# chhylp123/BitMapperBS

Hardware: AMD Instinct MI355X
Metric: M 150bp PE reads aligned/s (higher is better)
Workload: dtype u64

## Files before the change

### bitmapperbs_amd/csrc/bmbs_api.hip

```cpp
#include "bmbs_host.h"
#include "bmbs_kernels.hip"



int ensure(Lane* c, DevBuf& b, size_t bytes, bool zero)
{
    if (bytes == 0) bytes = 16;
    if (b.cap >= bytes) return BMBS_OK;
    size_t want = bytes + bytes / 8 + 256;
    if (c->kn.arena && want <= ((size_t)256 << 20)) {
        if (b.cap) want = std::min<size_t>(std::max(want, b.cap + b.cap / 2), (size_t)256 << 20);
        void* p = c->arena.alloc(want);
        if (!p) { c->err = "out of device memory (lane arena)"; return BMBS_ENOMEM; }
        if (b.p && !b.arena) (void)hipFree(b.p);
        b.p = p; b.cap = want; b.arena = true;
    } else {
        if (b.p && !b.arena) (void)hipFree(b.p);
        b.p = nullptr; b.cap = 0; b.arena = false;
        hipError_t e = hipMalloc(&b.p, want);
        if (e != hipSuccess) { c->err = std::string("hipMalloc: ") + hipGetErrorString(e); b.p = nullptr; return BMBS_ENOMEM; }
        b.cap = want;
    }
    if (zero && hipMemsetAsync(b.p, 0, want, c->stream) != hipSuccess) { c->err = "hipMemsetAsync failed"; return BMBS_ESTATE; }
    return BMBS_OK;
// ... 82 lines not shown
    }
    if (rep) for (int c = nc; c < 16; c++) rep[c] = rep[0];
    *n_classes = nc;
}

int map_calculation(const bmbs_params& P, unsigned second_best_diff, unsigned error_threshold, int best_score)
{
    const int unit = std::max(P.gap_open + P.gap_ext, P.mp_max);
    const int worst = -unit * (int)error_threshold;
    const double rank = (double)std::max(best_score - worst, 0) / (double)(-worst);
    const unsigned ediff = second_best_diff > error_threshold ? error_threshold + 1 : second_best_diff;
    if (ediff > error_threshold) {
        static const struct { double at; int q; } alone[] = {{0.8, 42}, {0.7, 40}, {0.6, 24}, {0.5, 23}, {0.4, 8}, {0.3, 3}};
        for (const auto& r : alone) if (rank >= r.at) return r.q;
        return 0;
    }
    const double rerr = (double)(int)ediff / (double)error_threshold;
    const bool perfect = best_score == 0;
    static const struct { double at; int zero; double hi_cut; int hi; double mid_cut; int mid; int lo; } rows[] = {
        {0.9, 39, 0.0, 33, 0.0, 33, 33}, {0.8, 38, 0.0, 27, 0.0, 27, 27}, {0.7, 37, 0.0, 26, 0.0, 26, 26}, {0.6, 36, 0.0, 22, 0.0, 22, 22},
        {0.5, 35, 0.84, 25, 0.68, 16, 5}, {0.4, 34, 0.84, 21, 0.68, 14, 4},
        {0.3, 32, 0.88, 18, 0.67, 15, 3}, {0.2, 31, 0.88, 17, 0.67, 11, 0}, {0.1, 30, 0.88, 12, 0.67, 7, 0},
    };
    for (const auto& r : rows)
        if (rerr >= r.at) return perfect ? r.zero : rank >= r.hi_cut ? r.hi : rank >= r.mid_cut ? r.mid : r.lo;
    return ediff == 0 ? (rank >= 0.67 ? 1 : 0) : (rank >= 0.67 ? 6 : 2);
}

int threshold_k(const bmbs_params& P, int L)
{
    u64 k = (u64)(P.e_f * L);
    if (k >= 31) k = 31;
    return (int)k;
}

int cigar_ops_bound(const bmbs_params& P, int L, int k)
{
    const long goe = (long)P.gap_open + P.gap_ext;
    const long worst = std::max<long>(std::max<long>(P.mp_max, P.np), goe);
    long gaps = (long)L + 2 * k;
    if (goe > 0) gaps = std::min<long>(gaps, (long)k * worst / goe);
    return (int)std::min<long>(2 * gaps + 8, 1 << 20);
}
#define BMBS_MAX_RECORD_OPS 254

int prepare_luts(Lane* c)
{
    if (c->luts_ready) return BMBS_OK;
    int unit = c->prm.gap_open + c->prm.gap_ext;
    if (unit < c->prm.mp_max) unit = c->prm.mp_max;
    c->mapq_unit = unit;
    std::vector<u32> off(64, 0);
    std::vector<u8> lut;
    for (int k = 0; k <= 62; k++) {
        const int range = unit * k;
        off[k] = (u32)lut.size();
        lut.resize(lut.size() + (size_t)(k + 2) * (range + 1));
        u8* t = lut.data() + off[k];
        for (int ed = 0; ed <= k + 1; ed++)
            for (int sd = 0; sd <= range; sd++)
                t[(size_t)ed * (range + 1) + sd] = (u8)map_calculation(c->prm, (unsigned)ed, (unsigned)k, sd - range);
    }
    std::vector<u8> kl(1002);
    for (int L = 0; L <= 1001; L++) kl[L] = (u8)threshold_k(c->prm, L);
    ENS(c, c->mapq_lut, lut.size()); ENS(c, c->mapq_off, off.size() * 4); ENS(c, c->klut, kl.size());
    HIPCHK(c, hipMemcpyAsync(c->mapq_lut.p, lut.data(), lut.size(), hipMemcpyHostToDevice, c->stream));
    HIPCHK(c, hipMemcpyAsync(c->mapq_off.p, off.data(), off.size() * 4, hipMemcpyHostToDevice, c->stream));
    HIPCHK(c, hipMemcpyAsync(c->klut.p, kl.data(), kl.size(), hipMemcpyHostToDevice, c->stream));
    HIPCHK(c, hipStreamSynchronize(c->stream));
    c->luts_ready = true;
    return BMBS_OK;
}

ReadGeom geom(Lane* c, int L, const u16* d_len)
{
    ReadGeom g;
    g.len = d_len; g.klut = c->klut.as<u8>(); g.L = L; g.k = threshold_k(c->prm, L);
    return g;
}

int per_read_workspace(Lane* c, u64 n)
{
    ENS(c, c->verdict, n); ENS(c, c->n_seeds, n); ENS(c, c->multi, n); ENS(c, c->mm_site, n * 2);
    ENS(c, c->exit_site, n * 8); ENS(c, c->seeds, n * BMBS_MAX_SEEDS * sizeof(SeedRec));
    ENS(c, c->n_cand, n * 4); ENS(c, c->cand_off, (n + 1) * 8); ENS(c, c->n_votes, n * 4);
    ENS(c, c->best_site, n * 8); ENS(c, c->best_end, n * 4); ENS(c, c->best_err, n * 4); ENS(c, c->sbd, n * 4);
    ENS(c, c->red_status, n); ENS(c, c->job_flag, n * 4); ENS(c, c->job_off, (n + 1) * 8);
    return BMBS_OK;
}

ReadState read_state(Lane* c)
{
    ReadState s;
    s.verdict = c->verdict.as<u8>(); s.n_seeds = c->n_seeds.as<u8>(); s.multi = c->multi.as<u8>();
    s.mm_site = c->mm_site.as<u16>(); s.exit_site = c->exit_site.as<u64>(); s.seeds = c->seeds.as<SeedRec>();
    s.n_cand = c->n_cand.as<u32>(); s.cand_off = c->cand_off.as<u64>(); s.n_votes = c->n_votes.as<u32>();
    s.best_site = c->best_site.as<u64>(); s.best_end = c->best_end.as<int32_t>(); s.best_err = c->best_err.as<u32>();
    s.sbd = c->sbd.as<u32>(); s.red_status = c->red_status.as<u8>(); s.job_flag = c->job_flag.as<u32>();
    s.job_off = c->job_off.as<u64>();
    return s;
}

inline u64 sw_trace_slots(u64 n_jobs) { const u64 t = (u64)nblk(n_jobs, 64) * 64; return t < (1ull << 20) ? t : (1ull << 20); }

inline size_t sw_window_lds(const ReadGeom& gm, int jobs_per_lane) { return (size_t)jobs_per_lane * ((gm.L + 2 * gm.k + 62) / 32 + 1) * 64 * 8; }

template <int KB>
void launch_sw(Lane* c, const char* d_seq, const char* d_qual, const char* d_qual2, const ReadGeom& gm, int stride, u64 n_jobs,
               const Jobs& jobs, u32 rev_from, u32* d_cigar_pool, int max_ops, const PackedRows& prw)
{
    const u64 slots = sw_trace_slots(n_jobs);
    const size_t lds = sw_window_lds(gm, 1);
    auto kern = gm.len ? k_align_sw<KB, false> : gm.k == KB ? k_align_sw<KB, true, true> : k_align_sw<KB, true, false>;
    for (u64 base = 0; base < n_jobs; base += slots)
        hipLaunchKernelGGL(kern, dim3((unsigned)(slots / 64)), dim3(64), lds, c->stream, c->ix, c->sp, c->pen_lut.as<int>(), d_seq,
                           d_qual, d_qual2, gm, stride, c->totals.as<u64>() + 2, c->sw_job.as<u32>(), jobs, rev_from, c->trace.as<u64>(),
                           slots, base, d_cigar_pool, max_ops, c->a_start.as<int>(), c->a_end.as<int>(), c->a_nm.as<u32>(),
                           c->a_score.as<int>(), c->a_nops.as<int>(), prw);
}

template <int KB>
void launch_sw2(Lane* c, const char* d_seq, const char* d_qual, const char* d_qual2, const ReadGeom& gm, int stride, u64 n_jobs,
                const Jobs& jobs, u32 rev_from, u32* d_cigar_pool, int max_ops, const PackedRows& prw)
{
    const u64 slots = sw_trace_slots((n_jobs + 1) / 2);
    auto kern = !prw.base ? k_align_sw2<KB, false, false> : gm.k == KB ? k_align_sw2<KB, true, true> : k_align_sw2<KB, false, true>;
    for (u64 base = 0; base < n_jobs; base += 2 * slots)
        hipLaunchKernelGGL(kern, dim3((unsigned)(slots / 64)), dim3(64), sw_window_lds(gm, 2), c->stream, c->ix, c->sp, c->pen_lut.as<int>(), d_seq,
                           d_qual, d_qual2, gm, stride, c->totals.as<u64>() + 2, c->sw_job.as<u32>(), jobs, rev_from, c->trace.as<u64>(),
                           slots, base, d_cigar_pool, max_ops, c->a_start.as<int>(), c->a_end.as<int>(), c->a_nm.as<u32>(),
                           c->a_score.as<int>(), c->a_nops.as<int>(), prw);
}

template <class F>
void with_band_bound(int k, F&& f)
{
    if (k <= 2) f(std::integral_constant<int, 2>());
    else if (k <= 4) f(std::integral_constant<int, 4>());
    else if (k <= 6) f(std::integral_constant<int, 6>());
    else if (k <= 8) f(std::integral_constant<int, 8>());
    else if (k <= 10) f(std::integral_constant<int, 10>());
    else if (k <= 12) f(std::integral_constant<int, 12>());
    else if (k <= 16) f(std::integral_constant<int, 16>());
    else if (k <= 20) f(std::integral_constant<int, 20>());
    else if (k <= 24) f(std::integral_constant<int, 24>());
    else f(std::integral_constant<int, 31>());
}

int run_align(Lane* c, const char* d_seq, const char* d_qual, const char* d_qual2, const ReadGeom& gm, int stride, u64 n_jobs, const Jobs& jobs,
              u32 rev_from, u32* d_cigar_pool, int max_ops, const PackedRows& pr, const u64* n_jobs_dev, u64 sw_bound)
{
    if (sw_bound > n_jobs) sw_bound = n_jobs;
    const int L = gm.L, k = gm.k;
    const u64 nj = n_jobs ? n_jobs : 1;
    const u64 nwk = (u64)((2 * k + 1 + 15) / 16);
    ENS(c, c->a_start, nj * 4); ENS(c, c->a_end, nj * 4); ENS(c, c->a_nm, nj * 4); ENS(c, c->a_score, nj * 4); ENS(c, c->a_nops, nj * 4);
    ENS(c, c->need_sw, nj * 4); ENS(c, c->sw_off, (nj + 1) * 8); ENS(c, c->sw_job, nj * 4);
    if (!n_jobs) return BMBS_OK;
    const int swm = c->kn.sw_form;
    const bool wave_form = swm == 3;
    int maxpen = std::max(std::max(c->prm.mp_max, c->prm.np), c->prm.gap_open + c->prm.gap_ext);
    const bool packed = !wave_form && swm != 1 && (k >= 5 || swm == 2) && !gm.len && c->prm.gap_ext < 256 && (L + 64) * maxpen < 12000 &&
                        c->prm.mp_min >= 0 && c->prm.gap_ext >= 0 && c->prm.gap_open >= 0 && c->prm.np >= 0;
    const bool reg_form = !wave_form;
    if (reg_form) {
        const u64 nwords = packed ? (u64)((2 * k + 1 + 7) / 8) : nwk;
        const u64 slots = packed ? sw_trace_slots((sw_bound + 1) / 2) : sw_trace_slots(sw_bound);
        ENS(c, c->trace, slots * (u64)L * nwords * 8);
    }
    unsigned long long* cnt = c->counters.as<unsigned long long>();
    prof_begin(c, "k_align_ungapped");
    if (pr.base)
        hipLaunchKernelGGL(k_align_ungapped_p, dim3(nblk(n_jobs, 256)), dim3(256), 0, c->stream, c->ix, c->sp, c->pen_lut.as<int>(), d_seq, pr,
                           d_qual, d_qual2, gm, stride, n_jobs, n_jobs_dev, jobs, rev_from, c->a_start.as<int>(), c->a_end.as<int>(), c->a_nm.as<u32>(),
                           c->a_score.as<int>(), c->a_nops.as<int>(), c->need_sw.as<u32>(), cnt);
    else
        hipLaunchKernelGGL(k_align_ungapped, dim3(nblk(n_jobs, 256)), dim3(256), 0, c->stream, c->ix, c->sp, c->pen_lut.as<int>(), d_seq,
                           d_qual, d_qual2, gm, stride, n_jobs, n_jobs_dev, jobs, rev_from, c->a_start.as<int>(), c->a_end.as<int>(), c->a_nm.as<u32>(),
                           c->a_score.as<int>(), c->a_nops.as<int>(), c->need_sw.as<u32>(), cnt);
    prof_end(c);
    prof_begin(c, "scan_sw");
    int rc = scan_u32(c, c->need_sw.as<u32>(), n_jobs, c->sw_off.as<u64>(), 2, c->sw_job.as<u32>(), 0, n_jobs_dev);
    if (rc) return rc;
    prof_end(c);
    if (n_jobs_dev && reg_form && sw_bound < n_jobs)
        hipLaunchKernelGGL(k_guard_count, dim3(1), dim3(1), 0, c->stream, c->totals.as<u64>() + 2, sw_bound, c->flags.as<u32>(), BMBS_FLAG_SW);
    prof_begin(c, "k_align_sw");
    if (!reg_form) {
        const size_t words = (size_t)sww_lds_words(L, k);
#define SWW_LAUNCH(LANES)                                                                                                             \
        hipLaunchKernelGGL((k_align_sw_wave<LANES>), dim3(nblk(n_jobs, 64 / LANES)), dim3(64), words * 4 * (64 / LANES), c->stream, c->ix, \
                           c->sp, c->pen_lut.as<int>(), d_seq, d_qual, d_qual2, gm, stride, c->totals.as<u64>() + 2, c->sw_job.as<u32>(),   \
                           jobs, rev_from, d_cigar_pool, max_ops, c->a_start.as<int>(), c->a_end.as<int>(), c->a_nm.as<u32>(),          \
                           c->a_score.as<int>(), c->a_nops.as<int>(), pr)
        if (k <= 7) SWW_LAUNCH(16);
        else if (k <= 15) SWW_LAUNCH(32);
        else SWW_LAUNCH(64);
#undef SWW_LAUNCH
        prof_end(c);
        return BMBS_OK;
    }
    with_band_bound(k, [&](auto kb) {
        if (packed) launch_sw2<decltype(kb)::value>(c, d_seq, d_qual, d_qual2, gm, stride, sw_bound, jobs, rev_from, d_cigar_pool, max_ops, pr);
        else launch_sw<decltype(kb)::value>(c, d_seq, d_qual, d_qual2, gm, stride, sw_bound, jobs, rev_from, d_cigar_pool, max_ops, pr);
    });
    prof_end(c);
    return BMBS_OK;
}

SeedCarry seed_carry(Lane* c)
{
    SeedCarry sc;
    sc.sp0 = c->sd_sp0.as<u64>(); sc.hits0 = c->sd_hits0.as<u32>(); sc.ml0 = c->sd_ml0.as<u16>(); sc.tm = c->sd_tm.as<u16>();
    sc.seed_id = c->sd_seed_id.as<u8>(); sc.clen = c->sd_clen.as<u32>(); sc.first_ml = c->sd_first_ml.as<u16>();
    sc.flag_c = c->sd_flag_c.as<u32>(); sc.flag_d = c->sd_flag_d.as<u32>(); sc.off_c = c->sd_off_c.as<u64>(); sc.off_d = c->sd_off_d.as<u64>();
    sc.list_c = c->sd_list_c.as<u32>(); sc.list_d = c->sd_list_d.as<u32>();
    return sc;
}

bool use_packed_rows(const Lane* c) { return !c->kn.rows_ascii; }
PackedRows packed_rows(const Lane* c, const ReadGeom& gm)
{
    if (!use_packed_rows(c)) return PackedRows{nullptr, nullptr, 0, 0};
    return PackedRows{c->prow.as<u64>(), c->prow_dirty.as<u8>(), pack_words(gm.L), pack_base_words(gm.L)};
}

bool occ3_build(Occ3Shared& o, u64 margin)
{
    const u64 rows = o.rows, nb = rows / 96 + 2, need = 27 * nb * 16;
    size_t free_b = 0, total_b = 0;
    (void)hipMemGetInfo(&free_b, &total_b);
    if (free_b <= need + margin) return false;
    const u64 n_chunks = (nb + OCC3_CHUNK - 1) / OCC3_CHUNK;
    void *t3 = nullptr, *c3 = nullptr, *sums = nullptr;
    hipStream_t st = nullptr;
    bool ok = hipMalloc(&t3, need) == hipSuccess && hipMalloc(&c3, 64 * 8) == hipSuccess && hipMalloc(&sums, 27 * n_chunks * 8 + 64) == hipSuccess &&
              hipStreamCreate(&st) == hipSuccess;
    if (ok) {
        u32* flag = reinterpret_cast<u32*>(c3) + 2 * 60;
        (void)hipMemsetAsync(c3, 0, 64 * 8, st);
        hipLaunchKernelGGL(k_occ3_planes, dim3(8192), dim3(256), 0, st, o.base, rows, nb, reinterpret_cast<uint4*>(t3));
        hipLaunchKernelGGL(k_occ3_chunk_sums, dim3(nblk(27 * n_chunks, 256)), dim3(256), 0, st, reinterpret_cast<uint4*>(t3), nb, n_chunks, reinterpret_cast<u64*>(sums));
        hipLaunchKernelGGL(k_occ3_chunk_scan, dim3(1), dim3(64), 0, st, reinterpret_cast<u64*>(sums), n_chunks, flag);
        hipLaunchKernelGGL(k_occ3_apply, dim3(nblk(27 * n_chunks, 256)), dim3(256), 0, st, reinterpret_cast<uint4*>(t3), nb, n_chunks, reinterpret_cast<u64*>(sums));
        hipLaunchKernelGGL(k_occ3_c3, dim3(1), dim3(64), 0, st, o.base, reinterpret_cast<u64*>(c3));
        DevIndex probe = o.base;
        probe.occ3 = reinterpret_cast<const uint4*>(t3); probe.c3 = reinterpret_cast<const u64*>(c3); probe.nb3 = nb;
        const u64 n_check = 1u << 20;
        hipLaunchKernelGGL(k_occ3_check, dim3(nblk(n_check, 256)), dim3(256), 0, st, probe, rows, n_check, flag + 1);
        u32 h[2] = {1, 1};
        ok = hipMemcpyAsync(h, flag, 8, hipMemcpyDeviceToHost, st) == hipSuccess && hipStreamSynchronize(st) == hipSuccess && h[0] == 0 && h[1] == 0;
        if (!ok && getenv("BMBS_VERBOSE")) fprintf(stderr, "[bmbs] trigram table not used: count overflow %u, differences from three single steps %u\n", h[0], h[1]);
    }
    if (st) (void)hipStreamDestroy(st);
    if (sums) (void)hipFree(sums);
    if (ok) { o.occ3 = t3; o.c3 = c3; o.nb3 = nb; }
    else { if (t3) (void)hipFree(t3); if (c3) (void)hipFree(c3); }
    return true;
}
void occ3_want(Lane* c, bool behind_a_call)
{
    if (c->ix.occ3 || !c->o3 || c->kn.kgram < 1 || !use_packed_rows(c)) return;
    const bool wants = c->kn.kgram >= 2 || c->lr_chain >= 3.0;
    std::lock_guard<std::mutex> l(c->o3->mu);
    if (!c->o3->occ3 && wants && !c->o3->tried) {
        (void)hipSetDevice(c->dev);
        const bool attempted = occ3_build(*c->o3, behind_a_call ? (8ull << 30) : (40ull << 30));
        if (attempted || ++c->o3->skipped >= 8) c->o3->tried = true;
    }
    if (c->o3->occ3) { c->ix.occ3 = reinterpret_cast<const uint4*>(c->o3->occ3); c->ix.c3 = reinterpret_cast<const u64*>(c->o3->c3); c->ix.nb3 = c->o3->nb3; }
}

int launch_seeding(Lane* c, const char* d_seq, const ReadGeom& gm, int stride, u64 n, int pe_mode, bool prepacked)
{
    ENS(c, c->sd_sp0, n * 8); ENS(c, c->sd_hits0, n * 4); ENS(c, c->sd_ml0, n * 2); ENS(c, c->sd_tm, n * 2); ENS(c, c->sd_seed_id, n);
    ENS(c, c->sd_clen, n * 4); ENS(c, c->sd_first_ml, n * 2); ENS(c, c->sd_flag_c, n * 4); ENS(c, c->sd_flag_d, n * 4);
    ENS(c, c->sd_off_c, (n + 1) * 8); ENS(c, c->sd_off_d, (n + 1) * 8); ENS(c, c->sd_list_c, n * 4); ENS(c, c->sd_list_d, n * 4);
    SeedCarry sc = seed_carry(c);
    ReadState st = read_state(c);
    unsigned long long* cnt = c->counters.as<unsigned long long>();
    const unsigned chunks = nblk(n, SEED_CHUNK);
    const unsigned chunks_min = nblk(n, SEED_CHUNK_MIN);
    const int target_waves = c->kn.seed_waves;
    const bool packed = use_packed_rows(c);
    if (packed && !prepacked) {
        const int pwords = pack_words(gm.L), W = pack_base_words(gm.L);
        { int rz_ = ensure(c, c->prow, n * (u64)pwords * 8 + 64, true); if (rz_) return rz_; } ENS(c, c->prow_dirty, n + 64);
        HIPCHK(c, hipMemsetAsync(c->prow_dirty.p, 0, n + 64, c->stream));
        prof_begin(c, "k_pack_rows");
        hipLaunchKernelGGL(k_pack_rows, dim3(nblk(n * (u64)(stride / 16), 256)), dim3(256), 0, c->stream, d_seq, gm, stride, (long)n,
                           c->prow.as<u64>(), pwords, W, c->prow_dirty.as<u32>());
        prof_end(c);
    }
    const PackedRows pr = packed_rows(c, gm);
    prof_begin(c, "k_seed_first");
    occ3_want(c, false);
    const bool kg = c->ix.occ3 && packed && (c->kn.kgram >= 2 || (c->kn.kgram == 1 && c->lr_chain >= 3.0));
    const int stage = c->kn.seed_stage;
    if (packed && kg && stage) hipLaunchKernelGGL((k_seed_first<true, true, true>), dim3(chunks), dim3(64), 0, c->stream, c->ix, d_seq, pr, gm, stride, (long)n, sc, cnt);
    else if (packed && kg) hipLaunchKernelGGL((k_seed_first<true, true>), dim3(chunks), dim3(64), 0, c->stream, c->ix, d_seq, pr, gm, stride, (long)n, sc, cnt);
    else if (packed && stage) hipLaunchKernelGGL((k_seed_first<true, false, true>), dim3(chunks), dim3(64), 0, c->stream, c->ix, d_seq, pr, gm, stride, (long)n, sc, cnt);
    else if (packed) hipLaunchKernelGGL(k_seed_first<true>, dim3(chunks), dim3(64), 0, c->stream, c->ix, d_seq, pr, gm, stride, (long)n, sc, cnt);
    else hipLaunchKernelGGL(k_seed_first<false>, dim3(chunks), dim3(64), 0, c->stream, c->ix, d_seq, pr, gm, stride, (long)n, sc, cnt);
    prof_end(c);
    prof_begin(c, "k_seed_decide");
    const bool lds_ok = (size_t)64 * (stride + 8) <= 48 * 1024;
    if (packed)
        hipLaunchKernelGGL(k_seed_decide_p, dim3(nblk(n, 64)), dim3(64), (size_t)64 * (pr.pwords + 1) * 8, c->stream, c->ix, d_seq, pr, gm, stride,
                           (long)n, c->prm.seed_len, pe_mode, (stage && !(pe_mode && c->prm.sensitive)) ? 1 : 0, st, sc, cnt);
    else if (lds_ok)
        hipLaunchKernelGGL((k_seed_decide<true, true>), dim3(nblk(n, 64)), dim3(64), (size_t)64 * (stride + 8), c->stream, c->ix, d_seq, gm,
                           stride, (long)n, c->prm.seed_len, pe_mode, st, sc, cnt);
    else
        hipLaunchKernelGGL((k_seed_decide<false, true>), dim3(nblk(n, 256)), dim3(256), 0, c->stream, c->ix, d_seq, gm, stride, (long)n,
                           c->prm.seed_len, pe_mode, st, sc, cnt);
    prof_end(c);
    prof_begin(c, "list_second");
    int rc = scan_u32(c, sc.flag_c, n, sc.off_c, 3, sc.list_c);
    if (rc) return rc;
    prof_end(c);
    prof_begin(c, "k_seed_second");
    if (packed && kg) hipLaunchKernelGGL((k_seed_second<true, true>), dim3(chunks_min), dim3(64), 0, c->stream, c->ix, d_seq, pr, gm, stride, c->totals.as<u64>() + 3, target_waves, pe_mode, st, sc, cnt);
    else if (packed) hipLaunchKernelGGL(k_seed_second<true>, dim3(chunks_min), dim3(64), 0, c->stream, c->ix, d_seq, pr, gm, stride, c->totals.as<u64>() + 3, target_waves, pe_mode, st, sc, cnt);
    else hipLaunchKernelGGL(k_seed_second<false>, dim3(chunks_min), dim3(64), 0, c->stream, c->ix, d_seq, pr, gm, stride, c->totals.as<u64>() + 3, target_waves, pe_mode, st, sc, cnt);
    prof_end(c);
    prof_begin(c, "list_extra");
    rc = scan_u32(c, sc.flag_d, n, sc.off_d, 4, sc.list_d);
    if (rc) return rc;
    prof_end(c);
    prof_begin(c, "k_seed_extra");
    {
        const size_t lds = 64 * (size_t)(stride + 16);
        const bool wide_ix = c->ix.sa64 != nullptr;
        const int rows_in_lds = lds <= 48 * 1024 && !wide_ix;
        const size_t plds = (size_t)64 * (pr.pwords + 1) * 8;
        if (packed && plds <= 16 * 1024 && kg)
            hipLaunchKernelGGL((k_seed_extra<false, true, true, true>), dim3(chunks_min), dim3(64), plds, c->stream, c->ix, d_seq, pr, gm, stride, c->totals.as<u64>() + 4,
                               target_waves, c->prm.seed_len, pe_mode, st, sc, cnt);
        else if (packed && plds <= 16 * 1024)
            hipLaunchKernelGGL((k_seed_extra<false, true, true>), dim3(chunks_min), dim3(64), plds, c->stream, c->ix, d_seq, pr, gm, stride, c->totals.as<u64>() + 4,
                               target_waves, c->prm.seed_len, pe_mode, st, sc, cnt);
        else if (packed)
            hipLaunchKernelGGL((k_seed_extra<false, true>), dim3(chunks_min), dim3(64), 0, c->stream, c->ix, d_seq, pr, gm, stride, c->totals.as<u64>() + 4,
                               target_waves, c->prm.seed_len, pe_mode, st, sc, cnt);
        else if (rows_in_lds)
            hipLaunchKernelGGL((k_seed_extra<true, false>), dim3(chunks_min), dim3(64), lds, c->stream, c->ix, d_seq, pr, gm, stride, c->totals.as<u64>() + 4,
                               target_waves, c->prm.seed_len, pe_mode, st, sc, cnt);
        else
            hipLaunchKernelGGL((k_seed_extra<false, false>), dim3(chunks_min), dim3(64), 0, c->stream, c->ix, d_seq, pr, gm, stride, c->totals.as<u64>() + 4,
                               target_waves, c->prm.seed_len, pe_mode, st, sc, cnt);
    }
    prof_end(c);
    return BMBS_OK;
}

int cand_total(Lane* c, const ReadState& st, u64 n, bool exact, u64* tot_out)
{
    if (exact) {
        u64 tot = 0;
        HIPCHK(c, hipMemcpyAsync(&tot, c->totals.as<u64>(), 8, hipMemcpyDeviceToHost, c->stream));
        HIPCHK(c, hipStreamSynchronize(c->stream));
        *tot_out = tot;
        return BMBS_OK;
    }
    const u64 cap = cap_from(c->lr_cand, n, n, c->kn.cap_scale);
    hipLaunchKernelGGL(k_guard_cand, dim3(nblk(n, 256)), dim3(256), 0, c->stream, c->totals.as<u64>(), cap, c->flags.as<u32>(), (long)n, st.verdict,
                       st.n_cand, st.cand_off);
    hipLaunchKernelGGL(k_guard_done, dim3(1), dim3(1), 0, c->stream, c->totals.as<u64>(), c->flags.as<u32>(), BMBS_FLAG_CAND);
    *tot_out = cap;
    return BMBS_OK;
}

int run_seed_stages(Lane* c, const char* d_seq, const ReadGeom& gm, int stride, u64 n, u64* total_cand, int pe_mode, bool exact, bool prepacked)
{
    ReadState st = read_state(c);
    int rc = launch_seeding(c, d_seq, gm, stride, n, pe_mode, prepacked);
    if (rc) return rc;
    prof_begin(c, "scan_cand");
    rc = scan_u32(c, st.n_cand, n, st.cand_off, 0);
    if (rc) return rc;
    prof_end(c);
    u64 tot = 0;
    rc = cand_total(c, st, n, exact, &tot);
    if (rc) return rc;
    *total_cand = tot;
    const u64 t1 = exact ? std::max<u64>(tot, cap_from((double)tot / (double)n, n, n)) : tot;
    ENS(c, c->cand, t1 * 8); ENS(c, c->votes, t1 * sizeof(bmbs_vote)); ENS(c, c->slot_read, t1 * 4);
    ENS(c, c->ferr, t1 * 4); ENS(c, c->fend, t1 * 4);
    ENS(c, c->long_flag, n * 4); ENS(c, c->long_off, (n + 1) * 8); ENS(c, c->long_list, n * 4); ENS(c, c->vote_list, n * 4);
    prof_begin(c, "k_vote_fused");
    HIPCHK(c, hipMemsetAsync(c->long_flag.p, 0, n * 4, c->stream));
    HIPCHK(c, hipMemsetAsync(st.n_votes, 0, n * 4, c->stream));
// ... 43 lines not shown
    if (n && stride == ds) { HIPCHK(c, hipMemcpyAsync(dst.p, src, n * (u64)ds, hipMemcpyHostToDevice, st)); return BMBS_OK; }
    HIPCHK(c, hipMemsetAsync(dst.p, 0, n * (u64)ds + 64, st));
    if (n) HIPCHK(c, hipMemcpy2DAsync(dst.p, ds, src, stride, L, n, hipMemcpyHostToDevice, st));
    return BMBS_OK;
}


extern "C" void bmbs_default_params(bmbs_params* p)
{
    p->e_f = 0.08; p->mp_max = 6; p->mp_min = 2; p->np = 1; p->gap_open = 5; p->gap_ext = 3; p->q_base = 33;
    p->seed_len = 30; p->min_ins = 0; p->max_ins = 500; p->sensitive = 0; p->ambiguous_out = 0;
}

void lane_destroy(Lane* c);

Lane* lane_create(int device_id, const bmbs_params& prm, const Knobs& kn, bool first)
{
    Lane* c = new Lane();
    c->dev = device_id;
    c->prm = prm; c->kn = kn;
    c->sp.mp_max = c->prm.mp_max; c->sp.mp_min = c->prm.mp_min; c->sp.np = c->prm.np;
    c->sp.gap_open = c->prm.gap_open; c->sp.gap_ext = c->prm.gap_ext; c->sp.q_base = c->prm.q_base;
    c->sp.seed_len = c->prm.seed_len;
    if (hipStreamCreate(&c->stream) != hipSuccess) { delete c; return nullptr; }
    (void)hipEventCreateWithFlags(&c->ev_up, hipEventDisableTiming);
    (void)hipEventCreateWithFlags(&c->ev_k, hipEventDisableTiming);
    int lut[256];
    for (int q = 0; q < 256; q++) lut[q] = mismatch_penalty(c->prm, q);
    {
        uint8_t class_of[256], rep[16]; int32_t penalty_of[16], nc = 0;
        qual_class_table(c->prm, class_of, penalty_of, &nc, rep);
        for (int k = 0; k < 8; k++) { c->qrep_lo |= (u64)rep[k] << (8 * k); c->qrep_hi |= (u64)rep[8 + k] << (8 * k); }
    }
    const size_t shard_bytes = BMBS_SHARDS * BMBS_SHARD_WORDS * 8;
    if (ensure(c, c->pen_lut, sizeof(lut)) || ensure(c, c->stats, shard_bytes) || ensure(c, c->call_stats, shard_bytes) || ensure(c, c->counters, shard_bytes) ||
        ensure(c, c->totals, 32 * 8) || ensure(c, c->flags, BMBS_FLAG_WORDS * 4) || ensure(c, c->tx_info, 64) ||
        hipHostMalloc((void**)&c->h_info, 128, hipHostMallocPortable) != hipSuccess ||
        hipHostMalloc((void**)&c->h_tot, 8 * 20 * 8, hipHostMallocPortable) != hipSuccess) { lane_destroy(c); return nullptr; }
    memset(c->h_tot, 0, 8 * 20 * 8);
    (void)hipMemcpy(c->pen_lut.p, lut, sizeof(lut), hipMemcpyHostToDevice);
    (void)hipMemset(c->stats.p, 0, shard_bytes);
    (void)hipMemset(c->call_stats.p, 0, shard_bytes);
    (void)hipMemset(c->counters.p, 0, shard_bytes);
    textpath_device_init(c);
    (void)hipMemset(c->totals.p, 0, 32 * 8);
    (void)hipMemset(c->flags.p, 0, BMBS_FLAG_WORDS * 4);
    if (first)
    if (const char* wl = getenv("BMBS_WAVELOG")) {
        const unsigned cap = 1u << 21;
        if (*wl && !ensure(c, c->wavelog_buf, (u64)cap * 32) && !ensure(c, c->wavelog_count, 64)) {
            (void)hipMemset(c->wavelog_count.p, 0, 64);
            WaveLogDev d = {c->wavelog_buf.as<unsigned long long>(), c->wavelog_count.as<unsigned int>(), cap};
            if (hipMemcpyToSymbol(HIP_SYMBOL(g_wavelog), &d, sizeof(d)) == hipSuccess) c->wavelog_path = wl;
        }
    }
    return c;
}

void lane_copy_streams(std::vector<Lane*>& lanes)
{
    for (Lane* c : lanes) (void)hipStreamCreateWithFlags(&c->up_stream, hipStreamNonBlocking);
    for (Lane* c : lanes) (void)hipStreamCreateWithFlags(&c->down_stream, hipStreamNonBlocking);
}
__attribute__((constructor)) static void bmbs_env_init() { setenv("GPU_MAX_HW_QUEUES", "8", 0); }

void lane_destroy(Lane* c)
{
    if (!c) return;
    (void)hipSetDevice(c->dev);
    if (c->stream) (void)hipStreamSynchronize(c->stream);
    if (!c->wavelog_path.empty()) {
        (void)hipDeviceSynchronize();
        unsigned cnt = 0;
        (void)hipMemcpy(&cnt, c->wavelog_count.p, 4, hipMemcpyDeviceToHost);
        if (cnt > (1u << 21)) cnt = 1u << 21;
        std::vector<unsigned long long> h((size_t)cnt * 4);
        if (cnt) (void)hipMemcpy(h.data(), c->wavelog_buf.p, (size_t)cnt * 32, hipMemcpyDeviceToHost);
        if (FILE* f = fopen(c->wavelog_path.c_str(), "wb")) { fwrite(h.data(), 32, cnt, f); fclose(f); }
        WaveLogDev d = {nullptr, nullptr, 0};
        (void)hipMemcpyToSymbol(HIP_SYMBOL(g_wavelog), &d, sizeof(d));
        release(c->wavelog_buf); release(c->wavelog_count);
    }
    DevBuf* all[] = {&c->occ, &c->hash, &c->sa, &c->gen2, &c->gen2p, &c->chrom_start, &c->t20, &c->pen_lut, &c->mapq_lut, &c->verdict,
                     &c->n_seeds, &c->multi, &c->mm_site, &c->exit_site, &c->seeds, &c->n_cand, &c->cand_off,
                     &c->n_votes, &c->best_site, &c->best_end, &c->best_err, &c->sbd, &c->red_status, &c->job_flag,
                     &c->job_off, &c->scan_tmp, &c->scan_ticket, &c->totals, &c->cand, &c->votes, &c->slot_read, &c->vote_off, &c->votes_dense, &c->dense_read, &c->ferr, &c->fend,
                     &c->job_read, &c->job_site, &c->job_end, &c->job_err, &c->need_sw, &c->sw_off, &c->sw_job, &c->trace, &c->a_start, &c->a_end, &c->a_nm, &c->a_score, &c->a_nops,
                     &c->in_seq, &c->in_qual, &c->out_res, &c->cig_pool, &c->in_a, &c->in_b, &c->in_c, &c->in_d,
                     &c->stats, &c->call_stats, &c->flags, &c->counters, &c->pe_seq, &c->pe_B, &c->pe_occ, &c->pe_len, &c->pe_cur,
                     &c->sd_sp0, &c->sd_hits0, &c->sd_ml0, &c->sd_tm, &c->sd_seed_id, &c->sd_clen, &c->sd_first_ml, &c->sd_flag_c, &c->sd_flag_d,
                     &c->sd_off_c, &c->sd_off_d, &c->sd_list_c, &c->sd_list_d, &c->pe_vround, &c->pe_dead, &c->pe_both, &c->pe_npair, &c->pe_sbd, &c->in_seq2, &c->in_qual2,
                     &c->pe_first, &c->pe_full, &c->pe_R, &c->pe_roff, &c->pe_rflag, &c->pe_rscan, &c->pe_rlist, &c->pe_rcnt, &c->pe_ritem_off, &c->pe_rcand, &c->long_flag, &c->long_off, &c->long_list, &c->vote_list,
                     &c->mapq_off, &c->klut, &c->in_len, &c->fq_text1, &c->fq_text2, &c->fq_idx, &c->pk_in1, &c->pk_in2, &c->pq_in1, &c->pq_in2, &c->pk_ascii, &c->prow, &c->prow_dirty, &c->pe_mid_flag, &c->pe_mid_list};
    for (DevBuf* b : all) release(*b);
    for (auto& set : c->profset) for (auto& p : set) { (void)hipEventDestroy(p.a); (void)hipEventDestroy(p.b); }
    c->arena.free_all();
    if (c->h_tot) (void)hipHostFree(c->h_tot);
    if (c->h_info) (void)hipHostFree(c->h_info);
    { DevBuf* tx[] = {&c->tx_tilecnt, &c->tx_tileoff, &c->tx_nl[0], &c->tx_nl[1], &c->tx_rec[0], &c->tx_rec[1], &c->tx_info, &c->sam_len, &c->sam_off, &c->sam_out, &c->chrom_chars, &c->chrom_off, &c->big_list,
                     &c->bam_raw, &c->bam_slots, &c->bam_slot_len, &c->bam_off, &c->stats_snap, &c->z_comp, &c->z_off, &c->z_text, &c->z_err, &c->z_nl, &c->z_comp2, &c->z_off2, &c->z_err2,
                     &c->bs_key, &c->bs_key2, &c->bs_idx, &c->bs_idx2, &c->bs_slen, &c->bs_soff, &c->bs_tmp, &c->bs_in, &c->bs_len, &c->bs_off, &c->bs_sorted, &c->bai_a, &c->bai_b, &c->bai_out,
                     &c->dp_in, &c->dp_len, &c->dp_off, &c->dp_sig, &c->dp_key, &c->dp_key2, &c->dp_idx, &c->dp_idx2, &c->dp_dup, &c->dp_tmpl,
                     &c->mt_in, &c->mt_len, &c->mt_off, &c->mt_clip, &c->mt_cnt, &c->mt_eoff, &c->mt_ev, &c->mt_work, &c->mt_acc, &c->mt_site, &c->mt_cl2};
      for (DevBuf* b : tx) release(*b); }
    if (c->ev_up) (void)hipEventDestroy(c->ev_up);
    if (c->ev_k) (void)hipEventDestroy(c->ev_k);
    if (c->ev_qx_a) (void)hipEventDestroy(c->ev_qx_a);
    if (c->ev_qx_b) (void)hipEventDestroy(c->ev_qx_b);
    if (c->up_stream) (void)hipStreamDestroy(c->up_stream);
    if (c->down_stream) (void)hipStreamDestroy(c->down_stream);
    if (c->stream) (void)hipStreamDestroy(c->stream);
    delete c;
}


extern "C" bmbs_ctx* bmbs_create(int device_id, const bmbs_params* params)
{
    int ndev = 0;
    if (hipGetDeviceCount(&ndev) != hipSuccess || ndev <= 0 || device_id < 0 || device_id >= ndev) return nullptr;
    if (hipSetDevice(device_id) != hipSuccess) return nullptr;
    bmbs_ctx* X = new bmbs_ctx();
    X->dev = device_id;
    if (params) X->prm = *params; else bmbs_default_params(&X->prm);
    X->kn.read();
    for (int i = 0; i < X->kn.host_lanes; i++) {
        Lane* c = lane_create(device_id, X->prm, X->kn, i == 0);
        if (!c) { bmbs_destroy(X); return nullptr; }
        X->lanes.push_back(c);
    }
    lane_copy_streams(X->lanes);
    return X;
}

extern "C" void bmbs_destroy(bmbs_ctx* X)
{
#ifdef VOTE_PROF
    {
        unsigned long long h[4][8];
        if (hipMemcpyFromSymbol(h, HIP_SYMBOL(g_vote_prof), sizeof h) == hipSuccess)
            for (int q = 0; q < 4; q++)
                fprintf(stderr, "[vote_prof] class %d: lists %llu candidates %llu sites %llu | Mcycles: locate+sort %.1f run-ends %.1f vote-order %.1f write %.1f | one-lane fallbacks %llu\n",
                        q, h[q][0], h[q][1], h[q][2], h[q][3] / 1e6, h[q][4] / 1e6, h[q][5] / 1e6, h[q][6] / 1e6, h[q][7]);
    }
#endif
    if (!X) return;
    (void)hipSetDevice(X->dev);
    for (size_t i = X->lanes.size(); i-- > 0;) lane_destroy(X->lanes[i]);
    delete X;
}

extern "C" int32_t bmbs_max_cigar_ops(const bmbs_params* params, int32_t L)
{
    if (L <= 0 || L > BMBS_MAX_READ) return -1;
    bmbs_params P;
    if (params) P = *params; else bmbs_default_params(&P);
    return cigar_ops_bound(P, L, threshold_k(P, L));
}

extern "C" int64_t bmbs_outcome_index(uint64_t bases, uint32_t not_acgt, int32_t len, int32_t bits, int32_t* depth)
{
    if (bits != 32 && bits != 33) return -2;
    static const std::vector<u16> tab = [] { std::vector<u16> t(256); for (int v = 0; v < 256; v++) t[v] = th_tab_entry(v); return t; }();
    int D = 0;
    u64 idx = 0;
    const bool ok = th_slot(bases, not_acgt, len, bits, tab.data(), idx, D);
    if (depth) *depth = D;
    return ok ? (int64_t)idx : -1;
}

extern "C" const char* bmbs_last_error(const bmbs_ctx* X) { return X ? X->err.c_str() : "no context (no HIP device?)"; }

static int lane_index_attach(Lane* c, const bmbs_index_view* v)
{
// ... 185 lines not shown
        if ((u64)P.cigar_cap < n_jobs * (u64)max_ops) { c->err = "cigar pool too small (it takes bmbs_max_cigar_ops() slots per read)"; return BMBS_ENOMEM; }
    } else {
        n_jobs_dev = c->totals.as<u64>() + 1;
        sw_bound = cap_from(c->lr_sw, reads, c->kn.cap_scale < 1.0 ? 64 : 16384, c->kn.cap_scale);
        if ((u64)P.cigar_cap < reads * (u64)max_ops) {
            hipLaunchKernelGGL(k_guard_jobs, dim3(nblk(reads, 256)), dim3(256), 0, c->stream, n_jobs_dev, (u64)max_ops, (u64)P.cigar_cap, c->flags.as<u32>(), (long)reads, st.job_flag);
            hipLaunchKernelGGL(k_guard_done, dim3(1), dim3(1), 0, c->stream, c->totals.as<u64>() + 1, c->flags.as<u32>(), BMBS_FLAG_CIGAR);
        }
    }
    c->last_n_jobs = n_jobs;
    const u64 nj = n_jobs ? n_jobs : 1;
    ENS(c, c->job_read, nj * 4); ENS(c, c->job_site, nj * 8); ENS(c, c->job_end, nj * 4); ENS(c, c->job_err, nj * 4);
    if (n_jobs) {
        prof_begin(c, "k_job_list");
        hipLaunchKernelGGL(k_job_list, dim3(nblk(reads, 256)), dim3(256), 0, c->stream, (long)reads, st, c->job_read.as<u32>(),
                           c->job_site.as<u64>(), c->job_end.as<int>(), c->job_err.as<u32>());
        prof_end(c);
    }
    const Jobs jobs = {c->job_read.as<u32>(), c->job_site.as<u64>(), c->job_end.as<int>(), c->job_err.as<u32>()};
    return run_align(c, seq, qual1, qual2, gm, P.stride, n_jobs, jobs, rev_from, reinterpret_cast<u32*>(P.d_cigar_pool), max_ops, packed_rows(c, gm),
                     n_jobs_dev, sw_bound);
}

int se_filter_reduce(Lane* c, const ReadGeom& gm, const ReadState& st, const char* d_seq, int stride, u64 n, u64 tot, bool exact)
{
    ENS(c, c->vote_off, (n + 1) * 8);
    {
        const u64 t1 = exact ? std::max<u64>(tot, cap_from((double)tot / (double)n, n, n)) : (tot ? tot : 1);
        ENS(c, c->votes_dense, t1 * sizeof(bmbs_vote)); ENS(c, c->dense_read, t1 * 4);
    }
    prof_begin(c, "vote_compact");
    int rc = scan_u32(c, st.n_votes, n, c->vote_off.as<u64>(), 5);
    if (rc) return rc;
    if (tot)
        hipLaunchKernelGGL(k_vote_compact, dim3(nblk(tot, 256)), dim3(256), 0, c->stream, tot, exact ? (const u64*)nullptr : c->totals.as<u64>(), st,
                           c->vote_off.as<u64>(), c->slot_read.as<u32>(), c->votes.as<bmbs_vote>(), c->votes_dense.as<bmbs_vote>(), c->dense_read.as<u32>());
    prof_end(c);
    if (tot) {
        prof_begin(c, "k_filter");
        hipLaunchKernelGGL(k_filter, dim3(nblk(tot, 256)), dim3(256), 0, c->stream, c->ix, d_seq, packed_rows(c, gm), gm, stride, c->totals.as<u64>() + 5,
                           c->dense_read.as<u32>(), c->votes_dense.as<bmbs_vote>(), c->ferr.as<u32>(), c->fend.as<int>(), c->counters.as<unsigned long long>());
        prof_end(c);
    }
    prof_begin(c, "k_reduce");
    HIPCHK(c, hipMemsetAsync(st.job_flag, 0, n * 4, c->stream));
    HIPCHK(c, hipMemsetAsync(st.red_status, 0, n, c->stream));
    hipLaunchKernelGGL(k_reduce, dim3(nblk(n, 256)), dim3(256), 0, c->stream, (long)n, c->prm.ambiguous_out, st, c->vote_off.as<u64>(),
                       c->votes_dense.as<bmbs_vote>(), c->ferr.as<u32>(), c->fend.as<int>(), c->totals.as<u64>() + 10, c->vote_list.as<u32>());
    prof_end(c);
    return BMBS_OK;
}

int map_se_dev(Lane* c, const Pending& P)
{
    ReadGeom gm = {};
    int max_ops = 0;
    int rc = call_open(c, P, (u64)P.n, &gm, &max_ops);
    if (rc || P.n == 0) return rc;
    const u64 n = (u64)P.n;
    const char* d_seq = reinterpret_cast<const char*>(P.a[0]);
    const char* d_qual = reinterpret_cast<const char*>(P.a[1]);
    if (P.packed_hw) {
        ENS(c, c->pk_ascii, n * (u64)P.stride + 64);
        { int rz_ = ensure(c, c->prow, n * (u64)pack_words(gm.L) * 8 + 64, true); if (rz_) return rz_; } ENS(c, c->prow_dirty, n + 64);
        HIPCHK(c, hipMemsetAsync(c->prow_dirty.p, 0, n + 64, c->stream));
        prof_begin(c, "k_rows_from_packed");
        rows_from_packed(c, reinterpret_cast<const u64*>(P.a[0]), P.packed_hw, gm, 0, n, false, c->pk_ascii.as<char>(), P.stride);
        prof_end(c);
        d_seq = c->pk_ascii.as<char>();
    }
    const ReadState st = read_state(c);
    u64 tot = 0;
    rc = run_seed_stages(c, d_seq, gm, P.stride, n, &tot, 0, P.exact, P.packed_hw > 0);
    if (rc) return rc;
    c->last_total_cand = tot;
    rc = se_filter_reduce(c, gm, st, d_seq, P.stride, n, tot, P.exact);
    if (rc) return rc;
    rc = align_jobs(c, P, gm, st, d_seq, d_qual, nullptr, n, 0xffffffffu, max_ops);
    if (rc) return rc;
    prof_begin(c, "k_finalize");
    hipLaunchKernelGGL(k_finalize, dim3(nblk(n, 256)), dim3(256), 0, c->stream, c->ix, c->sp, c->pen_lut.as<int>(),
                       c->mapq_lut.as<u8>(), c->mapq_off.as<u32>(), c->mapq_unit, d_seq, d_qual, gm, P.stride, (long)n, st, c->a_start.as<int>(),
                       c->a_end.as<int>(), c->a_nm.as<u32>(), c->a_score.as<int>(), c->a_nops.as<int>(), max_ops, P.cigar_base,
                       c->prm.ambiguous_out, c->sd_sp0.as<u64>(), c->sd_hits0.as<u32>(),
                       reinterpret_cast<bmbs_result_dev*>(P.d_results), c->call_stats.as<unsigned long long>());
    prof_end(c);
    return call_end(c, P.slot);
}

struct PeCall {
    Lane* c; ReadGeom gm; PeIns pi; ReadState st; PeState ps; PeCand *A, *B; char* seq_all; u64 n, n2; int stride; bool exact; u64 tot;
    bool prepacked;
    int rows(const Pending& P);
    int seed();
    int votes();
    int verify_round(int round, u64 cap, const char* name_f, const char* name_c);
    int verify_fast();
    int verify_sensitive();
};

int PeCall::rows(const Pending& P)
{
    prepacked = false;
    if (P.packed_hw) {
        { int rz_ = ensure(c, c->prow, n2 * (u64)pack_words(gm.L) * 8 + 64, true); if (rz_) return rz_; } ENS(c, c->prow_dirty, n2 + 64);
        HIPCHK(c, hipMemsetAsync(c->prow_dirty.p, 0, n2 + 64, c->stream));
        prof_begin(c, "k_rows_from_packed");
        rows_from_packed(c, reinterpret_cast<const u64*>(P.a[0]), P.packed_hw, gm, 0, n, false, seq_all, stride);
        rows_from_packed(c, reinterpret_cast<const u64*>(P.a[2]), P.packed_hw, gm, n, n, true, seq_all, stride);
        prof_end(c);
        prepacked = true;
    } else if (!P.prepared) {
        u64* prow = nullptr; u32* pdirty = nullptr;
        const int pwords = pack_words(gm.L), W = pack_base_words(gm.L);
        if (use_packed_rows(c)) {
            { int rz_ = ensure(c, c->prow, n2 * (u64)pwords * 8 + 64, true); if (rz_) return rz_; } ENS(c, c->prow_dirty, n2 + 64);
            HIPCHK(c, hipMemsetAsync(c->prow_dirty.p, 0, n2 + 64, c->stream));
            prow = c->prow.as<u64>(); pdirty = c->prow_dirty.as<u32>(); prepacked = true;
        }
        const int sparse = prow != nullptr;
        const char* seq1 = reinterpret_cast<const char*>(P.a[0]);
        const char* seq2 = reinterpret_cast<const char*>(P.a[2]);
        prof_begin(c, "k_pe_prepare");
        const int ppr = stride / 16;
        if (sparse && ppr <= 256) {
            const int rpb = 256 / ppr;
            hipLaunchKernelGGL(k_pe_prepare_p, dim3(std::min<u64>(nblk(n, rpb), 2048)), dim3(256), (size_t)rpb * (ppr + 1) * 16, c->stream,
                               seq1, seq2, gm, stride, (long)n, seq_all, prow, pwords, W, pdirty);
        } else
        hipLaunchKernelGGL(k_pe_prepare, dim3(nblk(n * (stride / 16), 256)), dim3(256), 0, c->stream, seq1, seq2, gm, stride, (long)n, seq_all,
                           prow, pwords, W, pdirty, sparse);
        prof_end(c);
    }
    return BMBS_OK;
}

int PeCall::seed()
{
    ps.occ = c->pe_occ.as<int>(); ps.len = c->pe_len.as<u32>(); ps.cur = c->pe_cur.as<u8>(); ps.vround = c->pe_vround.as<u8>();
    ps.dead = c->pe_dead.as<u8>(); ps.both = c->pe_both.as<u8>(); ps.npair = c->pe_npair.as<int>(); ps.sbd = c->pe_sbd.as<u32>();
    if (c->prm.sensitive) {
        ENS(c, c->pe_first, n); ENS(c, c->pe_full, n2); ENS(c, c->pe_roff, n2 * 8); ENS(c, c->pe_rflag, n * 4); ENS(c, c->pe_rscan, (n + 1) * 8);
        ENS(c, c->pe_rlist, n * 4); ENS(c, c->pe_rcnt, n * 4); ENS(c, c->pe_ritem_off, (n + 1) * 8);
    }
    ps.first = c->pe_first.as<u8>(); ps.full = c->pe_full.as<u8>(); ps.R = c->pe_R.as<PeCand>(); ps.roff = c->pe_roff.as<u64>();
    c->last_reseeded = 0; c->last_reseed_cand = 0;
    int rc = launch_seeding(c, seq_all, gm, stride, n2, 1, prepacked);
    if (rc) return rc;
    prof_begin(c, "scan_cand");
    rc = scan_u32(c, st.n_cand, n2, st.cand_off, 0);
    if (rc) return rc;
    prof_end(c);
    rc = cand_total(c, st, n2, exact, &tot);
    if (rc) return rc;
    c->last_total_cand = tot;
    const u64 t1 = exact ? std::max<u64>(tot, cap_from((double)tot / (double)n2, n2, n2)) : (tot ? tot : 1);
    ENS(c, c->cand, t1 * 8); ENS(c, c->votes, t1 * sizeof(PeCand)); ENS(c, c->pe_B, t1 * sizeof(PeCand)); ENS(c, c->slot_read, t1 * 4);
    ENS(c, c->dense_read, t1 * 4); ENS(c, c->ferr, t1 * 4);
    A = c->votes.as<PeCand>();
    B = c->pe_B.as<PeCand>();
    return BMBS_OK;
}

int PeCall::votes()
{
    unsigned long long* cnt = c->counters.as<unsigned long long>();
    ENS(c, c->long_flag, n2 * 4); ENS(c, c->long_off, (n2 + 1) * 8); ENS(c, c->long_list, n2 * 4);
// ... 1033 lines not shown
```

### bitmapperbs_amd/csrc/bmbs_dev.h

```cpp
#ifndef BMBS_DEV_H
#define BMBS_DEV_H
#include <stdint.h>
#include <hip/hip_runtime.h>

typedef uint64_t u64; typedef uint32_t u32; typedef uint16_t u16; typedef uint8_t u8;

struct DevIndex {
    const uint4* occ;
    const u64*   hash;
    const u32*   sa;
    const u64*   sa64;
    int          sup_shift;
    u64          supT[4], supA[4];
    const u64*   gen2;
    const u64*   gen2p;
    const u64*   t20;
    int          t_e;
    int          t_b;
    const uint4* occ3;
    const u64*   c3;
    u64          nb3;
    const u64*   chrom_start;
    u64 G;
    u64 total;
    u64 shapline;
    u64 C[3];
    int n_chrom;
};

struct SeedRec { u64 sp; u32 hits; u16 len; u16 off; };
#define BMBS_MAX_SEEDS 28

struct ReadState {
    u8*   verdict;
    u8*   n_seeds;
    u8*   multi;
    u16*  mm_site;
    u64*  exit_site;
    SeedRec* seeds;
    u32*  n_cand;
    u64*  cand_off;
    u32*  n_votes;
    u64*  best_site;
    int32_t* best_end;
    u32*  best_err;
    u32*  sbd;
    u8*   red_status;
    u32*  job_flag;
    u64*  job_off;
};

struct ReadGeom {
    const u16* len; const u8* klut; int L; int k;
    __device__ __forceinline__ int rl(long r) const { return len ? (int)len[r] : L; }
    __device__ __forceinline__ int rk(int Lr) const { return len ? (int)klut[Lr] : k; }
};

struct ScoreParams {
    int mp_max, mp_min, np, gap_open, gap_ext, q_base;
    int seed_len;
};
struct bmbs_result_dev {
    u64 pos; u32 cigar_off; int32_t chrom; u16 flag; u16 nm; int16_t score; u8 status; u8 mapq; u8 n_cigar; u8 path; u16 n_cand; u32 tlen;
};

#define BMBS_SHARDS 64
#define BMBS_SHARD_WORDS 32
#endif
```

### bitmapperbs_amd/csrc/bmbs_host.h

```cpp
#ifndef BMBS_HOST_H
#define BMBS_HOST_H
#include "../../include/bmbs.h"
#include "bmbs_dev.h"
#include <algorithm>
#include <atomic>
#include <cmath>
#include <cstdio>
#include <cstring>
#include <ctime>
#include <sys/syscall.h>
#include <unistd.h>
#include <deque>
#include <memory>
#include <mutex>
#include <string>
#include <thread>
#include <vector>


struct DevBuf {
    void* p = nullptr; size_t cap = 0;
    bool arena = false;
    template <class T> T* as() const { return reinterpret_cast<T*>(p); }
};
// ... 33 lines not shown
    long split_min = 250000;
    int up_turns = 1;
    int scan_chain = 0;
    int prefilter = 1;
    int pef_long = 1;
    int vote_dense = 1;
    int kgram = 1;
    int seed_stage = 1;
    double cap_scale = 1.0;
    static const bool copy_streams = true, copy_lock = true, arena = true;
    void read()
    {
        auto is = [](const char* e, const char* v) { return e && !strcmp(e, v); };
        const char* e = getenv("BMBS_SW");
        sw_form = is(e, "reg") ? 1 : is(e, "reg2") ? 2 : is(e, "wave") ? 3 : 0;
        rows_ascii = is(getenv("BMBS_LEGACY"), "1");
        if ((e = getenv("BMBS_SEED_WAVES"))) seed_waves = atoi(e);
        exact = is(getenv("BMBS_EXACT"), "1");
        if ((e = getenv("BMBS_LANES"))) lanes = atoi(e);
        if (lanes < 1) lanes = 1;
        if (lanes > 8) lanes = 8;
        if ((e = getenv("BMBS_HOST_LANES"))) host_lanes = atoi(e);
        if (host_lanes < lanes) host_lanes = lanes;
        if (host_lanes > 8) host_lanes = 8;
        if ((e = getenv("BMBS_KGRAM"))) kgram = atoi(e);
        if ((e = getenv("BMBS_CHUNK"))) chunk = atol(e);
        if ((e = getenv("BMBS_SPLIT_MIN"))) split_min = atol(e);
        if (split_min < 1) split_min = 1;
        if ((e = getenv("BMBS_CAP_SCALE"))) cap_scale = atof(e);
        if ((e = getenv("BMBS_PEF_LONG"))) pef_long = atoi(e);
        if ((e = getenv("BMBS_PREFILTER"))) prefilter = atoi(e);
        if ((e = getenv("BMBS_VOTE_DENSE"))) vote_dense = atoi(e);
        if ((e = getenv("BMBS_UP_TURNS"))) up_turns = atoi(e);
        if ((e = getenv("BMBS_SCAN_CHAIN"))) scan_chain = atoi(e);
        if ((e = getenv("BMBS_SEED_STAGE"))) seed_stage = atoi(e) == 0 ? 0 : 1;
    }
};

struct Pending {
    bool pe = false, exact = false;
    int slot = 0;
    uint64_t a[4] = {0, 0, 0, 0};
    const u16* d_len = nullptr;
    int32_t L = 0, stride = 0;
    int64_t n = 0;
    uint64_t d_results = 0, d_cigar_pool = 0;
    int64_t cigar_cap = 0;
    u32 cigar_base = 0;
    bool prepared = false;
    int packed_hw = 0;
    bool staged = false;
};

struct Occ3Shared {
    std::mutex mu;
    bool tried = false;
    int skipped = 0;
    int dev = 0;
    DevIndex base;
    u64 rows = 0;
    void* occ3 = nullptr; void* c3 = nullptr; u64 nb3 = 0;
    ~Occ3Shared() { if (occ3 || c3) { (void)hipSetDevice(dev); if (occ3) (void)hipFree(occ3); if (c3) (void)hipFree(c3); } }
};

struct Lane {
    int dev = 0;
    hipStream_t stream = nullptr;
    hipStream_t up_stream = nullptr, down_stream = nullptr;
    hipEvent_t ev_up = nullptr, ev_k = nullptr;
    bmbs_params prm;
    ScoreParams sp;
    Knobs kn;
    Arena arena;
    std::string err;
    bool attached = false;
    DevIndex ix;
    u64 rows = 0;
    DevBuf occ, hash, sa, gen2, gen2p, chrom_start, t20;
    std::shared_ptr<Occ3Shared> o3;
    DevBuf pen_lut, mapq_lut;
    bool luts_ready = false;
    int mapq_unit = 0;
    DevBuf mapq_off, klut;
    DevBuf verdict, n_seeds, multi, mm_site, exit_site, seeds, n_cand, cand_off, n_votes, best_site,
        best_end, best_err, sbd, red_status, job_flag, job_off, scan_tmp, totals;
    DevBuf scan_ticket;
    u32 scan_ticket_base = 0, scan_epoch = 0;
    DevBuf vote_list;
    DevBuf cand, votes, slot_read, vote_off, votes_dense, dense_read, ferr, fend, job_read, job_site, job_end, job_err, need_sw, sw_off, sw_job, trace,
        a_start, a_end, a_nm, a_score, a_nops;
    DevBuf in_seq, in_qual, out_res, cig_pool, in_a, in_b, in_c, in_d, in_len;
    DevBuf pe_mid_flag, pe_mid_list;
    DevBuf big_list;
    DevBuf wavelog_buf, wavelog_count; std::string wavelog_path;
    DevBuf prow, prow_dirty;
    double link_up_s = 0, link_down_s = 0, text_call_s = 0; u64 text_calls = 0;
    DevBuf pk_in1, pk_in2, pk_ascii;
    DevBuf pq_in1, pq_in2;
    u64 qrep_lo = 0, qrep_hi = 0;
    hipEvent_t ev_qx_a = nullptr, ev_qx_b = nullptr;
    bool qx_timed = false;
    DevBuf fq_text1, fq_text2, fq_idx;
    DevBuf tx_tilecnt, tx_tileoff, tx_nl[2], tx_rec[2], tx_info, sam_len, sam_off, sam_out, chrom_chars, chrom_off;
    DevBuf bam_raw, bam_slots, bam_slot_len, bam_off, stats_snap;
    DevBuf bs_key, bs_key2, bs_idx, bs_idx2, bs_slen, bs_soff, bs_tmp, bs_in, bs_len, bs_off, bs_sorted;
    int64_t bs_n = -1;
    DevBuf bai_a, bai_b, bai_out;
    int64_t bai_n = -1;
    u64 bai_bytes = 0, bai_z = 0, bai_cnt[4] = {0, 0, 0, 0}, bai_at[3] = {0, 0, 0};
    u32 bai_ref_max = 0;
    bool bai_done = false;
    DevBuf dp_in, dp_len, dp_off, dp_sig, dp_key, dp_key2, dp_idx, dp_idx2, dp_dup, dp_tmpl;
    int64_t dup_n2 = -1;
    bool dup_pe = false, dup_done = false;
    DevBuf mt_in, mt_len, mt_off, mt_clip, mt_cnt, mt_eoff, mt_ev, mt_work, mt_acc, mt_site, mt_cl2;
    std::vector<std::pair<u64, u64>> mt_slice;
    int64_t ms_n = -1, mt_sites = -1;
    u64 ms_bytes = 0;
    DevBuf z_comp, z_off, z_text, z_err, z_nl, z_comp2, z_off2, z_err2;
    struct OpenText { bool valid = false, pe = false; u64 bytes1 = 0, bytes2 = 0; int64_t n = 0; } open_text;
    u32* h_info = nullptr;
    int n_refs = 0, max_ref_len = 0;
    DevBuf sd_sp0, sd_hits0, sd_ml0, sd_tm, sd_seed_id, sd_clen, sd_first_ml, sd_flag_c, sd_flag_d, sd_off_c, sd_off_d, sd_list_c, sd_list_d;
    DevBuf pe_seq, pe_B, pe_occ, pe_len, pe_cur, pe_vround, pe_dead, pe_both, pe_npair, pe_sbd, in_seq2, in_qual2;
    DevBuf pe_first, pe_full, pe_R, pe_roff, pe_rflag, pe_rscan, pe_rlist, pe_rcnt, pe_ritem_off, pe_rcand;
    u64 last_reseeded = 0, last_reseed_cand = 0;
    DevBuf stats, call_stats, flags, counters, long_flag, long_off, long_list;
    std::vector<Prof> profset[8];
    int prof_used[8] = {0, 0, 0, 0, 0, 0, 0, 0};
    int cur_slot = 0;
    struct ProfSum { const char* name; double ms; };
    std::vector<ProfSum> last, acc;
    u64 acc_calls = 0;
    u64 last_total_cand = 0, last_n_jobs = 0;
    int last_max_ops = 0;
    double lr_chain = 0;
    u64 h_counters[8] = {0, 0, 0, 0, 0, 0, 0, 0};
    double lr_cand = 0, lr_sw = 0, lr_rcand = 0, lr_long = 0;
    u64* h_tot = nullptr;
    std::deque<Pending> inflight;
    int next_slot = 0;
    u64 n_retries = 0;
};


struct bmbs_ctx {
    int dev = 0;
    bmbs_params prm;
    Knobs kn;
    std::string err;
    std::vector<Lane*> lanes;
    int used_lanes = 1;
    int next_lane = 0;
};

#define HIPCHK(c, call)                                                                                   \
    do {                                                                                                  \
        hipError_t e_ = (call);                                                                           \
        if (e_ != hipSuccess) {                                                                           \
            (c)->err = std::string(#call) + ": " + hipGetErrorString(e_);                                 \
            return BMBS_ENODEV;                                                                           \
        }                                                                                                 \
    } while (0)
#define ENS(c, buf, bytes) do { int rc_ = ensure((c), (buf), (bytes)); if (rc_) return rc_; } while (0)

int ensure(Lane* c, DevBuf& b, size_t bytes, bool zero = false);
void release(DevBuf& b);
inline unsigned nblk(u64 n, unsigned bs) { return (unsigned)((n + bs - 1) / bs); }
void prof_begin(Lane* c, const char* name);
void prof_end(Lane* c);
int scan_u32(Lane* c, const u32* in, u64 n, u64* out, int slot, u32* list = nullptr, int nz = 0, const u64* n_dev = nullptr);
int threshold_k(const bmbs_params& P, int L);
int cigar_ops_bound(const bmbs_params& P, int L, int k);
int lane_settle(Lane* c);
int lane_enqueue(Lane* c, Pending P, bool staged);
int settle_all(bmbs_ctx* X);
inline Lane* lane0(bmbs_ctx* X) { return X && !X->lanes.empty() ? X->lanes[0] : nullptr; }
inline int fin(bmbs_ctx* X, Lane* c, int rc) { if (rc && X && c) X->err = c->err; return rc; }
#define ON_LANE0(call) Lane* c = lane0(X); if (!c) return BMBS_EINVAL; { const int rs_ = settle_all(X); if (rs_) return rs_; } X->used_lanes = 1; return fin(X, c, call)
extern std::mutex g_h2d_mu[16], g_d2h_mu[16];
void textpath_device_init(Lane* c);
#endif
```

### bitmapperbs_amd/csrc/k_finalize.hip

```cpp
DEVI u16 sat16(u32 v) { return v > 0xffffu ? (u16)0xffffu : (u16)v; }

__global__ void __launch_bounds__(256)
k_finalize(DevIndex ix, ScoreParams sp, const int* __restrict__ pen_lut, const u8* __restrict__ mapq_lut,
           const u32* __restrict__ mapq_off, int unit, const char* __restrict__ seq, const char* __restrict__ qual, ReadGeom gm,
           int stride, long n, ReadState st, const int* __restrict__ a_start, const int* __restrict__ a_end,
           const u32* __restrict__ a_nm, const int* __restrict__ a_score, const int* __restrict__ a_nops,
           int max_ops, u32 cigar_base, int ambiguous_out, const u64* __restrict__ sp0, const u32* __restrict__ hits0,
           bmbs_result_dev* __restrict__ res, unsigned long long* __restrict__ stats)
{
    __shared__ unsigned long long sh[5];
    __shared__ u64 s_cs[BMBS_CS_LDS];
    if (threadIdx.x < 5) sh[threadIdx.x] = 0;
    const u64* cs = chrom_table(ix, s_cs);
    __syncthreads();
    const long r = (long)blockIdx.x * blockDim.x + threadIdx.x;
    u32 s0 = 0, s1 = 0, s2 = 0, s3 = 0, s4 = 0;
    if (r < n) {
        bmbs_result_dev o;
        o.pos = 0; o.cigar_off = 0; o.chrom = -1; o.status = 0; o.mapq = 0; o.flag = 0; o.nm = 0; o.score = 0;
        o.n_cigar = 0; o.path = 0; o.n_cand = sat16(st.n_cand[r]); o.tlen = 0;
        const int verdict = st.verdict[r];
        const int L = gm.rl(r), k = gm.rk(L);
        const int range = unit * k;
        mapq_lut += mapq_off[k];
        bool have = false, amb = false;
        u64 site = 0; long long start_site = 0, end_site = 0;
        u32 nm = 0; int score = 0; u32 sbd = 0; int mapq = 0;
        if (verdict == 1) { have = true; site = st.exit_site[r]; start_site = 0; end_site = L - 1; nm = 0; score = 0; mapq = 42; o.path = 1; }
        else if (verdict == 2) {
            have = true; site = st.exit_site[r]; start_site = 0; end_site = L - 1; nm = 1; o.path = 2;
            const int mv = st.mm_site[r], ms = mv & 0x7fff;
            score = (mv & 0x8000) ? -sp.np : -pen_lut[(unsigned char)qual[(size_t)r * stride + ms]];
            sbd = 0xffffffffu;
        } else if (verdict == 4) {
            o.status = 2; o.path = 4;
            if (ambiguous_out) {
                const u64 sp_ = sp0[r];
                u32 nh = hits0[r]; if (nh > 1000u) nh = 1000u;
                o.status = 3;
                for (u32 i = 0; i < nh; i++) {
                    const u64 s_ = ix.total - sa_at(ix, sp_ + i) - (u64)L;
                    u64 loc = s_; int flag;
                    if (loc >= ix.G) { loc = ix.G * 2 - (loc + (u64)(L - 1)) - 1; flag = 16; } else flag = 0;
                    int c = 0;
                    c = chrom_of(cs, ix.n_chrom, loc);
                    if (c >= ix.n_chrom) continue;
                    const u64 pos = loc + 1 - cs[c];
                    if (pos + (u64)(L - 1) > cs[c + 1] - cs[c]) continue;
                    o.pos = pos; o.chrom = c; o.flag = (u16)flag; o.mapq = 1; o.status = 2;
                    break;
                }
            }
        }
        else if (verdict == 3) {
            o.path = 3;
            const int rs = st.red_status[r];
            if (rs == 1 || (rs == 2 && ambiguous_out)) {
                amb = rs == 2;
                have = true; site = st.best_site[r]; sbd = st.sbd[r];
                if (st.job_flag[r]) {
                    const u64 jb = st.job_off[r];
                    start_site = a_start[jb]; end_site = a_end[jb]; nm = a_nm[jb]; score = a_score[jb];
                    const int no = a_nops[jb];
                    o.cigar_off = cigar_base + (u32)(jb * (u64)max_ops);
                    o.n_cigar = no < 0 ? 255 : (u8)no;
                } else { end_site = st.best_end[r]; start_site = end_site - L + 1; nm = 0; score = 0; }
            } else if (rs == 2) o.status = 2;
        }
        if (have) {
            if (verdict != 1) {
                int sd = score + range; if (sd < 0) sd = 0; if (sd > range) sd = range;
                const u32 ed = sbd > (u32)k ? (u32)k + 1 : sbd;
                mapq = mapq_lut[(size_t)ed * (range + 1) + sd];
            }
            u64 loc = site; int flag;
            if (loc >= ix.G) { loc = loc + (u64)end_site; loc = ix.G * 2 - loc - 1; flag = 16; }
            else { loc = loc + (u64)start_site; flag = 0; }
            int c = 0;
            c = chrom_of(cs, ix.n_chrom, loc);
            bool ok = c < ix.n_chrom;
            u64 pos = 0;
            if (ok) {
                pos = loc + 1 - cs[c];
                const u64 clen = cs[c + 1] - cs[c];
                if (pos + (u64)end_site - (u64)start_site > clen) ok = false;
            }
            o.pos = pos; o.chrom = c < ix.n_chrom ? c : -1; o.flag = (u16)flag; o.mapq = (u8)mapq;
            o.nm = (u16)nm; o.score = (int16_t)score;
            o.status = ok ? (amb ? 2 : 1) : 3;
        }
        res[r] = o;
        s0 = 1;
        if (o.status == 1) { s1 = 1; s3 = (u32)L; s4 = (u32)nm; }
        else if (o.status == 2) s2 = 1;
    }
    wave_stats_add(sh, s0, s1, s2, s3, s4);
    __syncthreads();
    if (threadIdx.x < 5 && sh[threadIdx.x]) atomicAdd(&SHARD(stats)[threadIdx.x], sh[threadIdx.x]);
}
```

### bitmapperbs_amd/csrc/k_pe_fast.hip

```cpp
struct PeCand { u64 site; u32 err; int32_t end; };

struct PeIns { int min_ins, max_ins; };
DEVI void pe_bounds(const ReadGeom& gm, const PeIns& pi, long p, long n, long long& maxd, long long& mind, int& large_k)
{
    const int L1 = gm.rl(p), L2 = gm.rl(p + n);
    const int k1 = gm.rk(L1), k2 = gm.rk(L2);
    large_k = k1 > k2 ? k1 : k2;
    maxd = (long long)pi.max_ins + 2LL * large_k;
    mind = (long long)pi.min_ins - 2LL * large_k - (L1 > L2 ? L1 : L2);
}

struct PeState {
    int*  occ;
    u32*  len;
    u8*   cur;
    u8*   vround;
    u8*   dead;
    u8*   both;
    int*  npair;
    u32*  sbd;
    u8*   first;
    u8*   full;
    PeCand* R;
    u64*  roff;
// ... 86 lines not shown
            const size_t i16 = (size_t)r * ppr + piece;
            const int L1 = gm.rl(r);
            L2 = gm.rl(n + r);
            u32 b1, m1, b2, m2;
            pack_piece(v1, L1 - piece * 16, b1, m1);
            pack_piece(v2, L2 - piece * 16, b2, m2);
            lb[rl * (ppr + 1) + piece] = b2; lm[rl * (ppr + 1) + piece] = m2;
            if (piece == 0) { lb[rl * (ppr + 1) + ppr] = 0; lm[rl * (ppr + 1) + ppr] = 0; }
            if (piece * 16 < ((L1 + 63) & ~63)) {
                u64* row = prow + (size_t)r * pwords;
                if (piece * 16 < ((L1 + 31) & ~31)) reinterpret_cast<u32*>(row)[piece] = b1;
                reinterpret_cast<u16*>(row + W)[piece] = (u16)m1;
                if (m1) { atomicOr(&dirty32[r >> 2], 1u << (8 * (int)(r & 3))); reinterpret_cast<uint4*>(seq_all)[i16] = v1; }
            }
        }
        __syncthreads();
        if (on && piece * 16 < ((L2 + 63) & ~63)) {
            const int j0 = piece * 16, lo = L2 - 16 - j0;
            const u32* fb = lb + rl * (ppr + 1); const u32* fm = lm + rl * (ppr + 1);
            u32 win, bad, inr;
            if (lo >= 0) {
                const int idx = lo >> 4, sh = lo & 15;
                win = sh ? (fb[idx] >> (2 * sh)) | (fb[idx + 1] << (32 - 2 * sh)) : fb[idx];
                bad = ((fm[idx] | (fm[idx + 1] << 16)) >> sh) & 0xffffu;
                inr = 0xffffu;
            } else if (lo > -16) {
                win = fb[0] << (2 * -lo);
                bad = (fm[0] << -lo) & 0xffffu;
                inr = (0xffffu << -lo) & 0xffffu;
            } else { win = 0; bad = 0; inr = 0; }
            u32 x = inr & ~bad;
            x = (x | (x << 8)) & 0x00ff00ffu; x = (x | (x << 4)) & 0x0f0f0f0fu; x = (x | (x << 2)) & 0x33333333u; x = (x | (x << 1)) & 0x55555555u;
            win ^= x | (x << 1);
            u32 rv = __brev(win);
            rv = ((rv >> 1) & 0x55555555u) | ((rv & 0x55555555u) << 1);
            const u32 om = __brev(bad & inr) >> 16;
            const long row_id = n + r;
            u64* row = prow + (size_t)row_id * pwords;
            if (j0 < ((L2 + 31) & ~31)) reinterpret_cast<u32*>(row)[piece] = rv;
            reinterpret_cast<u16*>(row + W)[piece] = (u16)om;
            if (om) {
                atomicOr(&dirty32[row_id >> 2], 1u << (8 * (int)(row_id & 3)));
                const char* src = s2raw + r * stride;
                unsigned char o[16];
#pragma unroll
                for (int t = 0; t < 16; t++) {
                    const int j = j0 + t;
                    char c = 0;
                    if (j < L2) { const char a = src[L2 - 1 - j]; c = a == 'A' ? 'T' : a == 'T' ? 'A' : a == 'C' ? 'G' : a == 'G' ? 'C' : a; }
                    o[t] = (unsigned char)c;
                }
                uint4 v;
                v.x = o[0] | (o[1] << 8) | (o[2] << 16) | ((u32)o[3] << 24);
                v.y = o[4] | (o[5] << 8) | (o[6] << 16) | ((u32)o[7] << 24);
                v.z = o[8] | (o[9] << 8) | (o[10] << 16) | ((u32)o[11] << 24);
                v.w = o[12] | (o[13] << 8) | (o[14] << 16) | ((u32)o[15] << 24);
                reinterpret_cast<uint4*>(seq_all + total)[(size_t)r * ppr + piece] = v;
            }
        }
        r = rn; on = onn; v1 = n1; v2 = n2;
    }
}


DEVI bool vote_pe_light(long r, const ReadGeom& gm, const ReadState& st, const PeState& ps, PeCand* __restrict__ A, u32* __restrict__ long_flag)
{
    const int v = st.verdict[r];
    ps.cur[r] = 0; ps.vround[r] = 0;
    if (v == 3 || v == 4) return true;
    long_flag[r] = 0;
    if (v == 1 || v == 2) {
        const u64 off = st.cand_off[r];
        A[off].site = st.exit_site[r]; A[off].err = v == 1 ? 0u : 1u; A[off].end = gm.rl(r) - 1;
        ps.occ[r] = 1; ps.len[r] = 1;
    } else { ps.occ[r] = 0; ps.len[r] = 0; }
    return false;
}
DEVI void vote_pe_heavy(const DevIndex& ix, long r, const ReadGeom& gm, const ReadState& st, const PeState& ps, PeCand* __restrict__ A,
                        u32* __restrict__ long_flag, u32* __restrict__ mid_flag)
{
    const int L = gm.rl(r), k = gm.rk(L);
    const int v = st.verdict[r];
    const long nc = (long)st.n_cand[r];
    const SeedRec* my = st.seeds + (size_t)r * BMBS_MAX_SEEDS;
    const int ns = st.n_seeds[r];
    PeCand* o = A + st.cand_off[r];
    if (nc <= VOTE_REG) {
        u64 c[VOTE_REG];
        int sidx = 0; u32 h = 0;
        u64 sp = 0, adj = 0; u32 hits = 0;
        if (ns > 0) { sp = my[0].sp; adj = (u64)my[0].len + (u64)my[0].off; hits = my[0].hits; }
#pragma unroll
        for (int j = 0; j < VOTE_REG; j++) {
            c[j] = ~0ull;
            if (j < nc) {
                while (h == hits && sidx + 1 < ns) { sidx++; h = 0; sp = my[sidx].sp; adj = (u64)my[sidx].len + (u64)my[sidx].off; hits = my[sidx].hits; }
                c[j] = ix.total - ((sp >> 63) ? (sp & ~(1ull << 63)) : sa_at(ix, sp + h)) - adj;
                h++;
            }
        }
#define CE(a, b) { const u64 x_ = c[a], y_ = c[b]; c[a] = x_ < y_ ? x_ : y_; c[b] = x_ < y_ ? y_ : x_; }
        CE(0,1) CE(2,3) CE(4,5) CE(6,7) CE(8,9) CE(10,11) CE(12,13) CE(14,15)
        CE(0,2) CE(1,3) CE(4,6) CE(5,7) CE(8,10) CE(9,11) CE(12,14) CE(13,15)
        CE(1,2) CE(5,6) CE(9,10) CE(13,14)
        CE(0,4) CE(1,5) CE(2,6) CE(3,7) CE(8,12) CE(9,13) CE(10,14) CE(11,15)
        CE(2,4) CE(3,5) CE(10,12) CE(11,13)
        CE(1,2) CE(3,4) CE(5,6) CE(9,10) CE(11,12) CE(13,14)
        CE(0,8) CE(1,9) CE(2,10) CE(3,11) CE(4,12) CE(5,13) CE(6,14) CE(7,15)
        CE(4,8) CE(5,9) CE(6,10) CE(7,11)
        CE(2,4) CE(3,5) CE(6,8) CE(7,9) CE(10,12) CE(11,13)
        CE(1,2) CE(3,4) CE(5,6) CE(7,8) CE(9,10) CE(11,12) CE(13,14)
#undef CE
        int nv = 0;
#pragma unroll
        for (int i = 0; i < VOTE_REG; i++) {
            if (i < nc) {
                if (v == 4) { o[i].site = c[i]; o[i].err = 0; o[i].end = L - 1; }
                else if (i + 1 >= nc || (i + 1 < VOTE_REG && c[i + 1] != c[i])) {
                    o[nv].site = c[i] < (u64)k ? 0 : c[i] - (u64)k; o[nv].err = 0; o[nv].end = 0; nv++;
                }
            }
        }
        if (v == 4) { ps.occ[r] = (int)nc; ps.len[r] = (u32)nc; }
        else { ps.occ[r] = -1; ps.len[r] = (u32)nv; }
        long_flag[r] = 0;
        return;
    }
    if (mid_flag && nc <= VOTE_MID) { mid_flag[r] = 1; long_flag[r] = 0; return; }
    long_flag[r] = 1;
}

__global__ void __launch_bounds__(64)
k_vote_pe_fused(DevIndex ix, long n2, ReadGeom gm, ReadState st, PeState ps, PeCand* __restrict__ A, u32* __restrict__ long_flag,
                u32* __restrict__ mid_flag)
{
    const long r = (long)blockIdx.x * blockDim.x + threadIdx.x;
    if (r >= n2) return;
    if (vote_pe_light(r, gm, st, ps, A, long_flag)) vote_pe_heavy(ix, r, gm, st, ps, A, long_flag, mid_flag);
}

#define VOTE_DENSE_BLOCK 256
__global__ void __launch_bounds__(VOTE_DENSE_BLOCK)
k_vote_pe_dense(DevIndex ix, long n2, ReadGeom gm, ReadState st, PeState ps, PeCand* __restrict__ A, u32* __restrict__ long_flag,
                u32* __restrict__ mid_flag)
{
    constexpr int BLOCK = VOTE_DENSE_BLOCK, NW = BLOCK / 64;
    __shared__ u16 sh_idx[BLOCK];
    __shared__ int sh_tot[NW];
    const int tid = (int)threadIdx.x, lane = tid & 63, w = tid >> 6;
    const long row0 = (long)blockIdx.x * BLOCK;
    const long r = row0 + tid;
    const bool heavy = r < n2 && vote_pe_light(r, gm, st, ps, A, long_flag);
    const unsigned long long m = __ballot(heavy);
    if (heavy) sh_idx[w * 64 + __popcll(m & ((1ull << lane) - 1))] = (u16)tid;
    if (lane == 0) sh_tot[w] = __popcll(m);
    __syncthreads();
    int base = 0, src = -1;
#pragma unroll
    for (int q = 0; q < NW; q++) {
        const int t = sh_tot[q];
        if (src < 0 && tid < base + t) src = q * 64 + tid - base;
        base += t;
    }
    if (src < 0) return;
    vote_pe_heavy(ix, row0 + sh_idx[src], gm, st, ps, A, long_flag, mid_flag);
}

__global__ void __launch_bounds__(64)
k_vote_pe_mid(DevIndex ix, ReadGeom gm, ReadState st, PeState ps, const u64* __restrict__ count_ptr, const u32* __restrict__ list,
              PeCand* __restrict__ A, unsigned long long* __restrict__ counters)
{
    const long it = (long)blockIdx.x * blockDim.x + threadIdx.x;
    const bool act = it < (long)*count_ptr;
    const long r = act ? (long)list[it] : 0;
    const long nc = act ? (long)st.n_cand[r] : 0;
    wave_count_add(counters, CNT_CAND_MID, (u32)nc);
    if (!act) return;
    const int L = gm.rl(r), k = gm.rk(L);
    const int v = st.verdict[r];
    const SeedRec* my = st.seeds + (size_t)r * BMBS_MAX_SEEDS;
    const int ns = st.n_seeds[r];
    PeCand* o = A + st.cand_off[r];
    u64 c[VOTE_MID];
    {
        int sidx = 0; u32 h = 0;
        u64 sp = 0, adj = 0; u32 hits = 0;
        if (ns > 0) { sp = my[0].sp; adj = (u64)my[0].len + (u64)my[0].off; hits = my[0].hits; }
#pragma unroll
        for (int j = 0; j < VOTE_MID; j++) {
            c[j] = ~0ull;
            if (j < nc) {
                while (h == hits && sidx + 1 < ns) { sidx++; h = 0; sp = my[sidx].sp; adj = (u64)my[sidx].len + (u64)my[sidx].off; hits = my[sidx].hits; }
                c[j] = ix.total - ((sp >> 63) ? (sp & ~(1ull << 63)) : sa_at(ix, sp + h)) - adj;
                h++;
            }
        }
    }
#pragma unroll
    for (int size = 2; size <= VOTE_MID; size <<= 1) {
#pragma unroll
        for (int stride = size >> 1; stride > 0; stride >>= 1) {
#pragma unroll
            for (int t = 0; t < VOTE_MID / 2; t++) {
                const int i = 2 * t - (t & (stride - 1)), j = i + stride;
                const bool asc = (i & size) == 0;
                const u64 x_ = c[i], y_ = c[j];
                const bool sw = asc ? x_ > y_ : x_ < y_;
                c[i] = sw ? y_ : x_; c[j] = sw ? x_ : y_;
            }
        }
    }
    if (v == 4) {
#pragma unroll
        for (int i = 0; i < VOTE_MID; i++) if (i < nc) { PeCand e; e.site = c[i]; e.err = 0; e.end = L - 1; o[i] = e; }
        ps.occ[r] = (int)nc; ps.len[r] = (u32)nc;
    } else {
        int nv = 0;
#pragma unroll
        for (int i = 0; i < VOTE_MID; i++) {
            if (i < nc && (i + 1 >= nc || (i + 1 < VOTE_MID && c[i + 1] != c[i]))) {
                PeCand e; e.site = c[i] < (u64)k ? 0 : c[i] - (u64)k; e.err = 0; e.end = 0;
                o[nv++] = e;
            }
        }
        ps.occ[r] = -1; ps.len[r] = (u32)nv;
    }
}

DEVI long pe_lower_bound_u64(const u64* v, long n, u64 key)
{
    long lo = 0, hi = n;
    while (lo < hi) { const long mid = (lo + hi) >> 1; if (v[mid] < key) lo = mid + 1; else hi = mid; }
    return lo;
}
#define PREF_STAGE 256
template <int EMAX>
DEVI int pe_prefilter(u64* keys, int cnt, int k, const PeCand* mate, long nm, u64 maxd, u64* sh_mate, int* sh_w)
{
    const int T = (int)blockDim.x, tid = (int)threadIdx.x, lane = tid & 63, w = tid >> 6;
    const int E = (cnt + T - 1) / T;
    for (int i = tid; i < (int)nm; i += T) sh_mate[i] = mate[i].site;
    __syncthreads();
    u64 mine[EMAX];
    u32 keep = 0;
    bool wrapped = false;
    int kept = 0;
#pragma unroll
    for (int e = 0; e < EMAX; e++) {
        const int idx = tid * E + e;
        if (e < E && idx < cnt) {
            const u64 c = keys[idx];
            mine[e] = c;
            wrapped |= (c >> 63) != 0;
            const u64 x = c < (u64)k ? 0 : c - (u64)k;
            const u64 lo = x > maxd ? x - maxd : 0;
            const long j = pe_lower_bound_u64(sh_mate, nm, lo);
            const bool ok = j < nm && (sh_mate[j] <= x || sh_mate[j] - x <= maxd);
            if (ok) { keep |= 1u << e; kept++; }
        }
    }
    if (__syncthreads_or(wrapped ? 1 : 0)) return -1;
    int incl = kept;
    for (int o = 1; o < 64; o <<= 1) { const int v = __shfl_up(incl, o, 64); if (lane >= o) incl += v; }
    if (lane == 63) sh_w[w] = incl;
    __syncthreads();
    int base = incl - kept, total = 0;
    for (int q = 0; q < (T + 63) / 64; q++) { const int x = sh_w[q]; if (q < w) base += x; total += x; }
#pragma unroll
    for (int e = 0; e < EMAX; e++) if (keep & (1u << e)) keys[base++] = mine[e];
    __syncthreads();
    return total;
}

template <int CAP, int BLOCK, int LO>
__global__ void __launch_bounds__(BLOCK)
k_vote_pe_long(DevIndex ix, ReadGeom gm, ReadState st, PeState ps, const u64* __restrict__ count_ptr, const u32* __restrict__ list,
               PeCand* __restrict__ A, u32* __restrict__ big_list, unsigned long long* __restrict__ big_count, u64* __restrict__ cand,
               unsigned long long* __restrict__ counters, long n_pairs, PeIns pi, int prefilter, const u32* __restrict__ long_flag)
{
    __shared__ u64 keys[CAP];
    __shared__ u16 endpos[CAP];
    __shared__ u32 sh_pref[BMBS_MAX_SEEDS + 1];
    __shared__ int sh_w[2 * (BLOCK / 64) + 1];
    __shared__ u64 sh_mate[PREF_STAGE];
    constexpr int EMAX = (CAP + BLOCK - 1) / BLOCK;
    auto in_class = [](long nc) { return nc > LO && (CAP == VL_CAP || nc <= CAP); };
    auto listed = [&](long x) { return long_flag[x] != 0; };
    const long total_items = (long)*count_ptr;
    for (long item = blockIdx.x; item < total_items; item += gridDim.x) {
        const long r0 = list[item];
        const long nc0 = (long)st.n_cand[r0];
        if (big_list && nc0 > CAP) { if (threadIdx.x == 0) big_list[atomicAdd(big_count, 1ull)] = (u32)r0; continue; }
        if (!in_class(nc0)) continue;
        const long m0 = r0 < n_pairs ? r0 + n_pairs : r0 - n_pairs;
        const bool mate_here = prefilter && listed(m0) && in_class((long)st.n_cand[m0]);
        if (mate_here) {
            const long ncm = (long)st.n_cand[m0];
            if (ncm < nc0 || (ncm == nc0 && m0 < r0)) continue;
        }
        for (int turn = 0; turn < (mate_here ? 2 : 1); turn++) {
            const long r = turn ? m0 : r0;
            const long m = turn ? r0 : m0;
            const long nc = (long)st.n_cand[r];
            if (counters && threadIdx.x == 0) {
                atomicAdd(&SHARD(counters)[CAP == VM_CAP ? CNT_CAND_LONG : CNT_CAND_BIG], (unsigned long long)nc);
                atomicAdd(&SHARD(counters)[CNT_LISTS_LONG], 1ull);
            }
            const int L = gm.rl(r), k = gm.rk(L);
            const int v = st.verdict[r];
            PeCand* o = A + st.cand_off[r];
            if (nc > CAP) {
                u64* c = cand + st.cand_off[r];
                vl_sort_huge<CAP, BLOCK>(ix, st.seeds + (size_t)r * BMBS_MAX_SEEDS, st.n_seeds[r], nc, keys, sh_pref, reinterpret_cast<u64*>(o), c);
                if (v == 4) {
                    for (long i = threadIdx.x; i < nc; i += BLOCK) { PeCand e; e.site = c[i]; e.err = 0; e.end = L - 1; o[i] = e; }
                    if (threadIdx.x == 0) { ps.occ[r] = (int)nc; ps.len[r] = (u32)nc; }
                } else {
                    int running = 0;
                    for (long base = 0; base < nc; base += BLOCK) {
                        const long i = base + (long)threadIdx.x;
                        bool keep = false;
                        u64 key = 0;
                        if (i < nc) { key = c[i]; keep = i == nc - 1 || c[i + 1] != key; }
                        int tot;
                        const int pre = vl_prefix(keep, sh_w, tot);
                        if (keep) { PeCand e; e.site = key < (u64)k ? 0 : key - (u64)k; e.err = 0; e.end = 0; o[running + pre] = e; }
                        running += tot;
                    }
                    if (threadIdx.x == 0) { ps.occ[r] = -1; ps.len[r] = (u32)running; }
                }
                if (mate_here && turn == 0) __threadfence();
                __syncthreads();
                continue;
            }
            vl_locate_range(ix, st.seeds + (size_t)r * BMBS_MAX_SEEDS, st.n_seeds[r], 0, (int)nc, keys, sh_pref, true);
            int cnt = (int)nc;
            if (prefilter && v == 3) {
                const bool earlier = !listed(m) || (long)st.n_cand[m] <= LO;
                const bool mate_final = (turn == 1 || earlier) && ps.len[m] <= PREF_STAGE;
                long long maxd, mind; int large_k;
                pe_bounds(gm, pi, r < n_pairs ? r : r - n_pairs, n_pairs, maxd, mind, large_k);
                if (mate_final && mind <= 0 && maxd >= 0) {
                    const int occm = ps.occ[m];
                    const long nm = occm == 0 ? 0 : (long)ps.len[m];
                    const PeCand* ml = A + st.cand_off[m];
                    if (nm == 0) cnt = 0;
                    else if (!(ml[nm - 1].site >> 63)) {
                        const int kept = pe_prefilter<EMAX>(keys, cnt, k, ml, nm, (u64)maxd, sh_mate, sh_w);
                        if (kept >= 0) cnt = kept;
                    }
                    if (cnt < (int)nc && counters && threadIdx.x == 0) atomicAdd(&SHARD(counters)[CNT_PREFILTER_DROP], (unsigned long long)(nc - cnt));
                }
            }
            if (cnt == 0) {
                if (threadIdx.x == 0) { ps.occ[r] = -1; ps.len[r] = 0; }
                __syncthreads();
                continue;
            }
            vl_sort_keys<EMAX>(keys, cnt);
            if (v == 4) {
                for (long i = threadIdx.x; i < cnt; i += BLOCK) { PeCand e; e.site = keys[i]; e.err = 0; e.end = L - 1; o[i] = e; }
                if (threadIdx.x == 0) { ps.occ[r] = (int)cnt; ps.len[r] = (u32)cnt; }
            } else {
                const int nv = vl_run_ends(keys, cnt, endpos, sh_w);
                for (int e2 = threadIdx.x; e2 < nv; e2 += BLOCK) {
                    const u64 site = keys[endpos[e2]];
                    PeCand e; e.site = site < (u64)k ? 0 : site - (u64)k; e.err = 0; e.end = 0;
                    o[e2] = e;
                }
                if (threadIdx.x == 0) { ps.occ[r] = -1; ps.len[r] = (u32)nv; }
            }
            if (mate_here && turn == 0) __threadfence();
            __syncthreads();
        }
    }
}

DEVI PeCand* pe_list(const PeState& ps, const ReadState& st, PeCand* A, PeCand* B, long r)
{
    const int cur = ps.cur[r];
    return cur == 2 ? ps.R + ps.roff[r] : (cur ? B : A) + st.cand_off[r];
}

DEVI void pe_filter_decide(const PeState& ps, long p, long r1, long r2, int occ1, int occ2, long la, long lb)
{
    ps.cur[r1] = 1; ps.cur[r2] = 1;
    ps.len[r1] = (u32)la; ps.len[r2] = (u32)lb;
    if (la == 0 || lb == 0) { ps.dead[p] = 1; return; }
    if (occ1 == -1 && occ2 == -1) {
        ps.both[p] = 1;
        if (la <= lb) { ps.vround[r1] = 1; ps.vround[r2] = 2; } else { ps.vround[r2] = 1; ps.vround[r1] = 2; }
    } else if (occ1 != -1) {
        if (la < occ1) ps.occ[r1] = (int)la;
        ps.vround[r2] = 1;
    } else {
        if (lb < occ2) ps.occ[r2] = (int)lb;
        ps.vround[r1] = 1;
    }
}
DEVI void pe_filter_serial(const PeCand* a, long na, const PeCand* b, long nb, long long maxd, long long mind, PeCand* ra, PeCand* rb, long& la_out, long& lb_out)
{
    long la = 0, lb = 0, first = 0;
    for (long i = 0; i < na; i++) {
        for (long j = first; j < nb; j++) {
            bool hit = false;
            if (a[i].site > b[j].site) {
                const long long d = (long long)(a[i].site - b[j].site);
                if (d > maxd) first = j + 1;
                else if (d >= mind) hit = true;
            } else {
                const long long d = (long long)(b[j].site - a[i].site);
                if (d > maxd) break;
                if (d >= mind) hit = true;
            }
            if (hit) {
                if (la == 0 || a[i].site > ra[la - 1].site) ra[la++] = a[i];
                if (lb == 0 || b[j].site > rb[lb - 1].site) rb[lb++] = b[j];
            }
// ... 236 lines not shown
```

### bitmapperbs_amd/csrc/k_pe_sensitive.hip

```cpp

DEVI bool pes_suit(const PeCand* mate, int mate_occ, int& next_start, u64 site, long long maxd, long long mind)
{
    for (int i = next_start; i < mate_occ; i++) {
        const u64 ms = mate[i].site;
        if (ms > site) {
            const long long d = (long long)(ms - site);
            if (d > maxd) return false;
            if (d >= mind) return true;
        } else {
            const long long d = (long long)(site - ms);
            if (d > maxd) next_start = i + 1;
            else if (d >= mind) return true;
        }
    }
    return false;
}

__global__ void __launch_bounds__(256)
k_pes_order(long n, ReadState st, SeedCarry sc, PeState ps)
{
    const long p = (long)blockIdx.x * blockDim.x + threadIdx.x;
    if (p >= n) return;
    ps.dead[p] = 0; ps.both[p] = 0; ps.npair[p] = 0; ps.sbd[p] = 0;
    u32 c[2];
    for (int m = 0; m < 2; m++) {
        const long r = p + m * n;
        const int v = st.verdict[r], ns = st.n_seeds[r];
        const SeedRec* my = st.seeds + (size_t)r * BMBS_MAX_SEEDS;
        c[m] = (v == 1 || v == 4) ? 0u : (ns >= 1 && my[0].off == 0 ? my[0].hits : 0u);
        ps.full[r] = (u8)((sc.flag_c[r] && !sc.flag_d[r]) ? 1 : ns);
        ps.roff[r] = 0;
    }
    const int f = c[0] <= c[1] ? 0 : 1;
    ps.first[p] = (u8)f;
    const long rF = p + (long)f * n;
    const int vF = st.verdict[rF];
    if (vF == 0) ps.dead[p] = 1;
    else if (vF == 3) ps.vround[rF] = 1;
}

DEVI bool pes_suit_any(const PeCand* a, int na, u64 s, long long maxd, long long mind)
{
    if (na == 0 || maxd < 0) return false;
    const u64 mn = mind > 0 ? (u64)mind : 0;
    if (mn > (u64)maxd) return false;
    long j = pe_lower_bound(a, na, s + mn);
    if (j < na && a[j].site - s <= (u64)maxd) return true;
    if (s < mn) return false;
    j = pe_lower_bound(a, na, s > (u64)maxd ? s - (u64)maxd : 0);
    return j < na && a[j].site <= s - mn;
}
__global__ void __launch_bounds__(64)
k_pes_second(long n, ReadGeom gm, PeIns pi, ReadState st, PeState ps, PeCand* __restrict__ A, PeCand* __restrict__ B)
{
    const long p = (long)blockIdx.x * blockDim.x + threadIdx.x;
    const int lane = threadIdx.x & 63;
    bool act = p < n && !ps.dead[p];
    long long maxd = 0, mind = 0; int large_k;
    long rF = 0, rS = 0;
    int occF = 0;
    if (act) {
        pe_bounds(gm, pi, p, n, maxd, mind, large_k);
        const int f = ps.first[p];
        rF = p + (long)f * n; rS = p + (long)(1 - f) * n;
        occF = ps.occ[rF];
        if (occF == 0) { ps.dead[p] = 1; act = false; }
        else if (st.verdict[rS] != 3) act = false;
    }
    const long nb = act ? (long)ps.len[rS] : 0;
    const bool coop = act && nb + occF > 64;
    if (act && !coop) {
        const PeCand* a = pe_list(ps, st, A, B, rF);
        PeCand* b = pe_list(ps, st, A, B, rS);
        long kept = 0;
        int next_start = 0;
        for (long j = 0; j < nb; j++) {
            const PeCand cj = b[j];
            if (pes_suit(a, occF, next_start, cj.site, maxd, mind)) b[kept++] = cj;
        }
        ps.len[rS] = (u32)kept;
        ps.vround[rS] = 2;
    }
    unsigned long long todo = __ballot(coop);
    while (todo) {
        const int src = __ffsll((long long)todo) - 1;
        todo &= todo - 1;
        const long pp = (long)__shfl((long long)p, src, 64);
        long long mxd, mnd; int lk;
        pe_bounds(gm, pi, pp, n, mxd, mnd, lk);
        const int f = ps.first[pp];
        const long rF2 = pp + (long)f * n, rS2 = pp + (long)(1 - f) * n;
        const int na = ps.occ[rF2];
        const long nb2 = (long)ps.len[rS2];
        const PeCand* a = pe_list(ps, st, A, B, rF2);
        PeCand* b = pe_list(ps, st, A, B, rS2);
        if ((a[na - 1].site >> 63) || (nb2 && (b[nb2 - 1].site >> 63))) {
            if (lane == src) {
                long kept = 0;
                int next_start = 0;
                for (long j = 0; j < nb2; j++) {
                    const PeCand cj = b[j];
                    if (pes_suit(a, na, next_start, cj.site, mxd, mnd)) b[kept++] = cj;
                }
                ps.len[rS2] = (u32)kept; ps.vround[rS2] = 2;
            }
            continue;
        }
        long kept = 0;
        for (long base = 0; base < nb2; base += 64) {
            const long j = base + lane;
            PeCand cj; cj.site = 0; cj.err = 0; cj.end = 0;
            bool keep = false;
            if (j < nb2) { cj = b[j]; keep = pes_suit_any(a, na, cj.site, mxd, mnd); }
            const unsigned long long kb = __ballot(keep);
            if (keep) b[kept + __popcll(kb & ((1ull << lane) - 1))] = cj;
            kept += __popcll(kb);
        }
        if (lane == src) { ps.len[rS2] = (u32)kept; ps.vround[rS2] = 2; }
    }
}

__global__ void __launch_bounds__(256)
k_pes_reseed_flag(long n, PeState ps, u32* __restrict__ flag)
{
    const long p = (long)blockIdx.x * blockDim.x + threadIdx.x;
    if (p >= n) return;
    const long rS = p + (long)(1 - ps.first[p]) * n;
    flag[p] = (!ps.dead[p] && ps.occ[rS] == 0) ? 1u : 0u;
}

template <bool PACKED, bool KG = false>
__global__ void __launch_bounds__(64)
k_pes_reseed(DevIndex ix, const char* __restrict__ seq, PackedRows pr, ReadGeom gm, int stride, long n, const u64* __restrict__ count_ptr,
             const u32* __restrict__ plist, ReadState st, PeState ps, u32* __restrict__ rcnt, unsigned long long* __restrict__ counters)
{
    __shared__ u64 s_c3[KG ? 27 : 1];
    th_tab_fill(ix);
    const u64* c3 = KG ? kgram_c3(ix, s_c3) : nullptr;
    const long it = (long)blockIdx.x * blockDim.x + threadIdx.x;
    LaneCounters lc = {0, 0, 0, 0, 0};
    if (it < (long)*count_ptr) {
        const long p = plist[it];
        const long r = p + (long)(1 - ps.first[p]) * n;
        const char* rd = seq + (size_t)r * stride;
        const u64* prow = PACKED ? pr.base + (size_t)r * pr.pwords : nullptr;
        const bool dirty = PACKED ? pr.dirty[r] != 0 : false;
        const int L = gm.rl(r);
        SeedRec* my = st.seeds + (size_t)r * BMBS_MAX_SEEDS;
        const int full = ps.full[r];
        int rs[3], rl[3], rn = 0;
        int s0 = 0, s1 = 0;
        if (full >= 1) s0 = my[0].off;
        if (full >= 2) {
            s1 = my[1].off;
            rn = 2;
            rs[0] = s0; rl[0] = s1 - s0;
            rs[1] = (int)my[full - 2].off + (int)my[full - 2].len; rl[1] = L - rs[1];
        } else if (full == 1) {
            rn = 2;
            rs[0] = s0; rl[0] = L / 2;
            rs[1] = rs[0] + rl[0]; rl[1] = L - rs[1];
        }
        const int last = full >= 1 ? (int)my[full - 1].off + (int)my[full - 1].len : 0;
        if (last < L) { rs[rn] = last; rl[rn] = L - last; rn++; }
        const int max_seed = L / 10 == 0 ? 25 : (L / 10 - 1 > 25 ? 25 : L / 10 - 1);
        const u64 max_hits = 1000, avail = 20;
        int ns = 0, seed_id = 0;
        u64 ncand = 0;
        typename std::conditional<PACKED, SearchP, Search>::type S; SeedHit h;
        while (seed_id < rn) {
            const int tm = rs[seed_id], ml = rl[seed_id];
            if constexpr (PACKED) {
                if (search_begin_p<true>(ix, prow, pr.W, dirty, tm + ml, tm, S, h, lc.n_hash))
                    while (!search_step_p<true, KG>(ix, tm + ml, S, h, lc.n_ext, c3, &lc.n_jump)) {}
            } else {
                if (search_begin<true>(ix, rd, tm + ml, tm, S, h, lc.n_hash))
                    while (!search_step<true>(ix, rd, tm + ml, S, h, lc.n_ext)) {}
            }
            if (h.hits == 1) seed_record(my, ns, ncand, h.sp, 1, (u64)ml, (u64)tm);
            else if ((u64)ml >= avail && h.hits <= max_hits) { if (h.hits != 0) seed_record(my, ns, ncand, h.sp, h.hits, (u64)ml, (u64)tm); }
            else if (L - tm == ml) break;
            seed_id++;
        }
        int tm = full > 1 ? (s0 + s1) / 2 : 4;
        while (seed_id < max_seed && tm < L) {
            if constexpr (PACKED) {
                if (search_begin_p<false>(ix, prow, pr.W, dirty, L, tm, S, h, lc.n_hash))
                    while (!search_step_p<false, KG>(ix, L, S, h, lc.n_ext, c3, &lc.n_jump)) {}
            } else {
                if (search_begin<false>(ix, rd, L, tm, S, h, lc.n_hash))
                    while (!search_step<false>(ix, rd, L, S, h, lc.n_ext)) {}
            }
            if (h.hits == 1) seed_record(my, ns, ncand, h.sp, 1, h.ml, (u64)tm);
            else if (h.ml >= avail && h.hits <= max_hits) { if (h.hits != 0) seed_record(my, ns, ncand, h.sp, h.hits, h.ml, (u64)tm); }
            else if ((u64)(L - tm) == h.ml) break;
            tm += 8;
            seed_id++;
        }
        st.n_seeds[r] = (u8)ns;
        rcnt[it] = (u32)ncand;
    }
    flush_counters(counters, lc, 2);
}

#define PESV_LONG 32
__global__ void __launch_bounds__(64)
k_pes_vote(DevIndex ix, long n, ReadGeom gm, PeIns pi, const u64* __restrict__ count_ptr, const u32* __restrict__ plist,
           const u64* __restrict__ roff, ReadState st, PeState ps, u64* __restrict__ rcand, PeCand* __restrict__ A, PeCand* __restrict__ B,
           u32* __restrict__ long_flag, unsigned long long* __restrict__ counters)
{
    const long it = (long)blockIdx.x * blockDim.x + threadIdx.x;
    const bool act_ = it < (long)*count_ptr;
    wave_count_add(counters, CNT_CAND_RESEED, act_ ? (u32)(roff[it + 1] - roff[it]) : 0u);
    if (!act_) return;
    if (long_flag) long_flag[it] = 0;
    const long p = plist[it];
    const int f = ps.first[p];
    const long rF = p + (long)f * n, r = p + (long)(1 - f) * n;
    const int k = gm.rk(gm.rl(r));
    long long maxd, mind; int large_k;
    pe_bounds(gm, pi, p, n, maxd, mind, large_k);
    const u64 o0 = roff[it], o1 = roff[it + 1];
    ps.roff[r] = o0;
    const long nc = (long)(o1 - o0);
    if (nc == 0) { ps.len[r] = 0; ps.vround[r] = 0; return; }
    if (long_flag && nc > PESV_LONG) { long_flag[it] = 1; return; }
    const SeedRec* my = st.seeds + (size_t)r * BMBS_MAX_SEEDS;
    const int ns = st.n_seeds[r];
    u64* c = rcand + o0;
    long o = 0;
    for (int s = 0; s < ns; s++) {
        const u64 sp = my[s].sp, adj = (u64)my[s].len + (u64)my[s].off;
        for (u32 j = 0; j < my[s].hits; j++) c[o++] = ix.total - ((sp >> 63) ? (sp & ~(1ull << 63)) : sa_at(ix, sp + j)) - adj;
    }
    sort_u64_asc(c, nc);
    const PeCand* a = pe_list(ps, st, A, B, rF);
    const int occF = ps.occ[rF];
    PeCand* out = ps.R + o0;
    long nv = 0;
    int next_start = 0;
    u64 pre = c[0];
    for (long i = 1; i <= nc; i++) {
        if (i < nc && c[i] == pre) continue;
        const u64 site = (i < nc) ? (pre < (u64)k ? 0 : pre - (u64)k) : (pre >= (u64)k ? pre - (u64)k : 0);
        if (pes_suit(a, occF, next_start, site, maxd, mind)) { out[nv].site = site; out[nv].err = 0; out[nv].end = 0; nv++; }
        if (i < nc) pre = c[i];
    }
    ps.cur[r] = 2; ps.len[r] = (u32)nv; ps.vround[r] = 3;
}

template <int CAP, int BLOCK, int LO>
__global__ void __launch_bounds__(BLOCK)
k_pes_vote_long(DevIndex ix, long n, ReadGeom gm, PeIns pi, const u64* __restrict__ count_ptr, const u32* __restrict__ items,
                const u32* __restrict__ plist, const u64* __restrict__ roff, ReadState st, PeState ps, u64* __restrict__ rcand,
                PeCand* __restrict__ A, PeCand* __restrict__ B)
{
    __shared__ u64 keys[CAP];
    __shared__ u16 endpos[CAP];
    __shared__ u32 sh_pref[BMBS_MAX_SEEDS + 1];
    __shared__ int sh_w[2 * (BLOCK / 64) + 1];
    const long total = (long)*count_ptr;
    for (long item = blockIdx.x; item < total; item += gridDim.x) {
        const long it = items[item];
        const u64 o0 = roff[it], o1 = roff[it + 1];
        const long nc = (long)(o1 - o0);
        if (nc <= LO || (CAP != VL_CAP && nc > CAP)) continue;
        const long p = plist[it];
        const int f = ps.first[p];
        const long rF = p + (long)f * n, r = p + (long)(1 - f) * n;
        const int k = gm.rk(gm.rl(r));
        long long maxd, mind; int large_k;
        pe_bounds(gm, pi, p, n, maxd, mind, large_k);
        const SeedRec* my = st.seeds + (size_t)r * BMBS_MAX_SEEDS;
        const int ns = st.n_seeds[r];
        const PeCand* a = pe_list(ps, st, A, B, rF);
        const int occF = ps.occ[rF];
        PeCand* out = ps.R + o0;
        if (nc > CAP) {
            u64* c = rcand + o0;
            vl_sort_huge<CAP, BLOCK>(ix, my, ns, nc, keys, sh_pref, reinterpret_cast<u64*>(out), c);
            if ((occF > 0 && (a[occF - 1].site >> 63)) || (c[nc - 1] >> 63)) {
                if (threadIdx.x == 0) {
                    long nv = 0;
                    int next_start = 0;
                    u64 pre = c[0];
                    for (long i = 1; i <= nc; i++) {
                        if (i < nc && c[i] == pre) continue;
                        const u64 site = pre < (u64)k ? 0 : pre - (u64)k;
                        if (pes_suit(a, occF, next_start, site, maxd, mind)) { out[nv].site = site; out[nv].err = 0; out[nv].end = 0; nv++; }
                        if (i < nc) pre = c[i];
                    }
                    ps.cur[r] = 2; ps.len[r] = (u32)nv; ps.vround[r] = 3;
                }
                __syncthreads();
                continue;
            }
            int running = 0;
            for (long base = 0; base < nc; base += BLOCK) {
                const long i = base + (long)threadIdx.x;
                bool keep = false;
                u64 site = 0;
                if (i < nc) {
                    const u64 key = c[i];
                    if (i == nc - 1 || c[i + 1] != key) { site = key < (u64)k ? 0 : key - (u64)k; keep = pes_suit_any(a, occF, site, maxd, mind); }
                }
                int tot;
                const int pre = vl_prefix(keep, sh_w, tot);
                if (keep) { PeCand c2; c2.site = site; c2.err = 0; c2.end = 0; out[running + pre] = c2; }
                running += tot;
            }
            if (threadIdx.x == 0) { ps.cur[r] = 2; ps.len[r] = (u32)running; ps.vround[r] = 3; }
            __syncthreads();
            continue;
        }
        bool serial = occF > 0 && (a[occF - 1].site >> 63);
        if (!serial) {
            vl_locate_sort<(CAP + BLOCK - 1) / BLOCK>(ix, my, ns, (int)nc, keys, sh_pref);
            serial = (keys[nc - 1] >> 63) != 0;
        }
        if (serial) {
            if (threadIdx.x == 0) {
                u64* c = rcand + o0;
                long o = 0;
                for (int s2 = 0; s2 < ns; s2++) {
                    const u64 sp = my[s2].sp, adj = (u64)my[s2].len + (u64)my[s2].off;
                    for (u32 j = 0; j < my[s2].hits; j++) c[o++] = ix.total - ((sp >> 63) ? (sp & ~(1ull << 63)) : sa_at(ix, sp + j)) - adj;
                }
                sort_u64_asc(c, nc);
                long nv = 0;
                int next_start = 0;
                u64 pre = c[0];
                for (long i = 1; i <= nc; i++) {
                    if (i < nc && c[i] == pre) continue;
                    const u64 site = pre < (u64)k ? 0 : pre - (u64)k;
                    if (pes_suit(a, occF, next_start, site, maxd, mind)) { out[nv].site = site; out[nv].err = 0; out[nv].end = 0; nv++; }
                    if (i < nc) pre = c[i];
                }
                ps.cur[r] = 2; ps.len[r] = (u32)nv; ps.vround[r] = 3;
            }
            __syncthreads();
            continue;
        }
        const int nd = vl_run_ends(keys, (int)nc, endpos, sh_w);
        int running = 0;
        for (int base = 0; base < nd; base += BLOCK) {
            const int e = base + (int)threadIdx.x;
            bool keep = false;
            u64 site = 0;
            if (e < nd) {
                const u64 key = keys[endpos[e]];
                site = key < (u64)k ? 0 : key - (u64)k;
                keep = pes_suit_any(a, occF, site, maxd, mind);
            }
            int tot;
            const int pre = vl_prefix(keep, sh_w, tot);
            if (keep) { PeCand c2; c2.site = site; c2.err = 0; c2.end = 0; out[running + pre] = c2; }
// ... 232 lines not shown
```

### bitmapperbs_amd/csrc/k_seed.hip

```cpp
struct SeedHit { u64 hits, sp, ml; };

struct Search { u64 top, bot, ptop, pbot; int s, steps, tm; ReadCur cur; };

DEVI void swar_code3(u64 w, u64& digits, u64& bad)
{
    const u64 K01 = 0x0101010101010101ull;
    digits = 0x0202020202020202ull - ((w >> 1) & K01) - ((w >> 2) & K01);
    const u64 isT = (w >> 2) & ~(w >> 1) & K01;
    bad = w ^ (0x4141414141414141ull | (w & 0x0606060606060606ull)) ^ (isT | (isT << 4));
}
DEVI u32 base3_of4(u32 x) { return (x * 0x0103091Bu) >> 24; }

template <bool FIXED, class SearchT>
DEVI int th_outcome(u64 v, int D, int len, SearchT& S, SeedHit& out, u32& n_hash)
{
    const int tag = (int)(v >> 60);
    if (tag == 14) return 0;
    n_hash++;
    const u64 row = v & ((1ull << 36) - 1), hits = (v >> 36) & ((1ull << 20) - 1);
    const int s = (int)(v >> 56) & 15, E = D - 16;
    if (tag == 15) return 1;
    if (FIXED) {
        if (tag == 2) return 1;
        if (tag != 0) { S.top = row | (1ull << 63); S.bot = S.top + 1; S.s = tag == 3 ? E : s; return 3; }
// ... 210 lines not shown
            if (!FIXED) { out.ml = 16 + S.s; out.sp = ptop; out.hits = pbot - ptop; } else { out.hits = 0; out.sp = 0; }
            return true;
        }
    }
    const u64 lt = ptop - (ptop > ix.shapline ? 1 : 0), lb = pbot - (pbot > ix.shapline ? 1 : 0);
    const u32 it = jump ? (u32)(ptop >> 5) / 3u : (u32)(lt >> 5), ib = jump ? (u32)(pbot >> 5) / 3u : (u32)(lb >> 5);
    const u32 rt = jump ? (u32)(ptop - (u64)it * 96) : (u32)lt & 31u, rb = jump ? (u32)(pbot - (u64)ib * 96) : (u32)lb & 31u;
    const uint4* base = jump ? ix.occ3 + (u64)g * ix.nb3 : ix.occ;
    const uint4 ht = base[it];
    uint4 hb = ht;
    if (ib != it) hb = base[ib];
    if (jump) {
        const u64 c3g = c3[g];
        const u64 t2 = c3g + occ3_in_block(ht, rt), b2 = c3g + occ3_in_block(hb, rb);
        if (b2 > t2 && b2 - t2 >= 2) {
            S.top = t2; S.bot = b2; S.s += 3; n_ext += 3;
            if (n_jump) (*n_jump)++;
            S.cur.buf >>= 6; S.cur.have -= 3; S.cur.pos += 3;
            if (S.s == S.steps) { out.ml = (u64)len; out.sp = S.top; out.hits = S.bot - S.top; return true; }
            return false;
        }
        S.kg = -(1 << 20);
        return false;
    }
    {
        const u32 mt = rt ? (~0u << (32 - rt)) : 0u, mb = rb ? (~0u << (32 - rb)) : 0u;
        u64 tT = (u64)ht.x + __popc(ht.z & mt), tA = (u64)ht.y + __popc(ht.w & mt);
        u64 bT = (u64)hb.x + __popc(hb.z & mb), bA = (u64)hb.y + __popc(hb.w & mb);
        if (ix.sup_shift) { super_add(ix, lt, tT, tA); super_add(ix, lb, bT, bA); }
        const u64 ct = d == 1 ? tT : (d == 2 ? tA : lt - tT - tA);
        const u64 cb = d == 1 ? bT : (d == 2 ? bA : lb - bT - bA);
        S.top = ix.C[d] + ct; S.bot = ix.C[d] + cb;
    }
    n_ext++;
    if (S.bot <= S.top) {
        if (!FIXED) { out.ml = 16 + S.s; out.sp = ptop; out.hits = pbot - ptop; } else { out.hits = 0; out.sp = S.top; }
        return true;
    }
    if (KG) S.kg = 2 * (S.bot - S.top) > before ? S.kg + 1 : (S.kg < 0 ? S.kg : 0);
    S.s++;
    if (S.s == S.steps) { out.ml = (u64)len; out.sp = S.top; out.hits = S.bot - S.top; return true; }
    return false;
}

DEVI bool rest_matches_3l(const DevIndex& ix, const u64* row, int W, bool dirty, int L, int tm, int start, u64 site)
{
    for (int q = start & ~31; q < L; q += 32) {
        const u64 rb = row[q >> 5];
        const u64 d = site + (u64)(q - tm);
        u64 mm;
        if (d + 32 <= ix.total) mm = mism_3l(rb, gen_bases32(ix, d));
        else {
            mm = 0;
            for (int j = 0; j < 32; j++) {
                const u64 dj = d + (u64)j;
                const int rc = (int)((rb >> (2 * j)) & 3);
                bool eq = false;
                if (dj < ix.total) { const int g = gbase(ix, dj); eq = (rc == g) || ((rc & 1) && (g & 1)); }
                if (!eq) mm |= 1ull << (2 * j);
            }
        }
        if (dirty) mm |= spread32((u32)((row[W + (q >> 6)] >> (q & 63)) & 0xffffffffull));
        if (mm & field_range(start - q, L - q)) return false;
    }
    return true;
}

DEVI int seed_offset_unmatch(int L, int pre, const char* rd, int step)
{
    if (L - pre < 18 || L - pre < step) return L;
    const int ret = pre + step;
    for (int i = 0; i < step; i++, pre++) if (rd[pre] == 'N') return pre + 1;
    return ret;
}
DEVI int seed_offset_unmatch_p(int L, int pre, const char* rd, int step, const u64* mask)
{
    if (L - pre < 18 || L - pre < step) return L;
    const int ret = pre + step;
    for (int i = 0; i < step; i++, pre++) if (((mask[pre >> 6] >> (pre & 63)) & 1) && rd[pre] == 'N') return pre + 1;
    return ret;
}

struct SeedCarry {
    u64* sp0; u32* hits0; u16* ml0;
    u16* tm; u8* seed_id; u32* clen; u16* first_ml;
    u32* flag_c; u32* flag_d;
    u64* off_c; u64* off_d;
    u32* list_c; u32* list_d;
};

DEVI void seed_record(SeedRec* my, int& ns, u64& ncand, u64 sp, u64 hits, u64 len, u64 off)
{
    my[ns].sp = sp; my[ns].hits = (u32)hits; my[ns].len = (u16)len; my[ns].off = (u16)off; ns++;
    ncand += hits;
}

DEVI void seed_finish(const ReadState& st, long r, int verdict, int ns, u64 ncand, int pe_mode)
{
    st.verdict[r] = (u8)verdict;
    st.n_seeds[r] = (u8)ns;
    st.n_cand[r] = verdict == 3 ? (u32)ncand : (pe_mode ? (verdict == 4 ? (u32)ncand : (verdict == 1 || verdict == 2) ? 1u : 0u) : 0u);
}

#define SEED_BATCH 16
#define SEED_CHUNK 256
#define SEED_CHUNK_MIN 64
DEVI long seed_chunk(long total, int target_waves)
{
    long c = (total + target_waves - 1) / target_waves;
    return c < SEED_CHUNK_MIN ? SEED_CHUNK_MIN : (c > SEED_CHUNK ? SEED_CHUNK : c);
}

struct LaneCounters { u32 n_hash, n_ext, n_sa, n_ung, n_jump; };
DEVI void flush_counters(unsigned long long* counters, const LaneCounters& c, int kid)
{
    u32 a = c.n_hash, b = c.n_ext, d = c.n_sa, e = c.n_ung, j = c.n_jump;
    for (int o = 32; o > 0; o >>= 1) { a += __shfl_down(a, o); b += __shfl_down(b, o); d += __shfl_down(d, o); e += __shfl_down(e, o); j += __shfl_down(j, o); }
    if ((threadIdx.x & 63) == 0 && counters) {
        counters = SHARD(counters);
        if (j) atomicAdd(&counters[8], (unsigned long long)j);
        unsigned long long* k = counters + 16 + 4 * kid;
        if (a) { atomicAdd(&counters[0], (unsigned long long)a); atomicAdd(&k[0], (unsigned long long)a); }
        if (b) { atomicAdd(&counters[1], (unsigned long long)b); atomicAdd(&k[1], (unsigned long long)b); }
        if (d) { atomicAdd(&counters[2], (unsigned long long)d); atomicAdd(&k[2], (unsigned long long)d); }
        if (e) { atomicAdd(&counters[5], (unsigned long long)e); atomicAdd(&k[3], (unsigned long long)e); }
    }
}

DEVI void wave_stats_add(unsigned long long* sh, u32 v0, u32 v1, u32 v2, u32 v3, u32 v4)
{
    for (int o = 32; o > 0; o >>= 1) { v0 += __shfl_down(v0, o); v1 += __shfl_down(v1, o); v2 += __shfl_down(v2, o); v3 += __shfl_down(v3, o); v4 += __shfl_down(v4, o); }
    if ((threadIdx.x & 63) == 0) {
        if (v0) atomicAdd(&sh[0], (unsigned long long)v0);
        if (v1) atomicAdd(&sh[1], (unsigned long long)v1);
        if (v2) atomicAdd(&sh[2], (unsigned long long)v2);
        if (v3) atomicAdd(&sh[3], (unsigned long long)v3);
        if (v4) atomicAdd(&sh[4], (unsigned long long)v4);
    }
}

template <bool PACKED, bool KG = false, bool STAGE = false>
__global__ void __launch_bounds__(64)
k_seed_first(DevIndex ix, const char* __restrict__ seq, PackedRows pr, ReadGeom gm, int stride, long n, SeedCarry sc,
             unsigned long long* __restrict__ counters)
{
    __shared__ u64 s_c3[KG ? 27 : 1];
    __shared__ u64 s_sp0[STAGE ? SEED_CHUNK : 1];
    __shared__ u32 s_hits0[STAGE ? SEED_CHUNK : 1];
    __shared__ u16 s_ml0[STAGE ? SEED_CHUNK : 1];
    th_tab_fill(ix);
    const u64* c3 = KG ? kgram_c3(ix, s_c3) : nullptr;
    const WaveLogT wl_t = wavelog_begin();
    int L = gm.L;
    const long chunk_begin = (long)blockIdx.x * SEED_CHUNK;
    const long chunk_end = chunk_begin + SEED_CHUNK < n ? chunk_begin + SEED_CHUNK : n;
    long next = chunk_begin;
    LaneCounters lc = {0, 0, 0, 0, 0};
    bool active = false;
    long r = 0;
    const char* rd = seq;
    typename std::conditional<PACKED, SearchP, Search>::type S; SeedHit h;
    bool pending = true, have = false;
    for (;;) {
        const unsigned long long pm = __ballot(pending);
        if (__popcll(pm) >= SEED_BATCH || !__any(active)) {
            if (pm == 0) break;
            const int rank = __popcll(pm & ((1ull << (threadIdx.x & 63)) - 1));
            const long it = next + rank;
            next += __popcll(pm);
            if (pending) {
                if (have) {
                    if (STAGE) { const int q = (int)(r - chunk_begin); s_sp0[q] = h.sp; s_hits0[q] = (u32)h.hits; s_ml0[q] = (u16)h.ml; }
                    else { sc.sp0[r] = h.sp; sc.hits0[r] = (u32)h.hits; sc.ml0[r] = (u16)h.ml; }
                    have = false;
                }
                if (it < chunk_end) {
                    r = it; have = true; L = gm.rl(r);
                    bool go;
                    if constexpr (PACKED) go = search_begin_p<false>(ix, pr.base + (size_t)r * pr.pwords, pr.W, pr.dirty[r] != 0, L, 0, S, h, lc.n_hash);
                    else { rd = seq + (size_t)r * stride; go = search_begin<false>(ix, rd, L, 0, S, h, lc.n_hash); }
                    if (go) { active = true; pending = false; }
                } else pending = false;
            }
            if (!__any(active) && !__any(pending)) break;
            continue;
        }
#ifdef BMBS_UTIL
        if ((threadIdx.x & 63) == 0) atomicAdd(&counters[8], 1ull);
        if (active) atomicAdd(&counters[9], 1ull);
#endif
        if (active) {
            bool fin;
            if constexpr (PACKED) fin = search_step_p<false, KG>(ix, L, S, h, lc.n_ext, c3, &lc.n_jump); else fin = search_step<false>(ix, rd, L, S, h, lc.n_ext);
            if (fin) { active = false; pending = true; }
        }
    }
    if (STAGE) {
        __syncthreads();
        const int cnt = (int)(chunk_end - chunk_begin);
        for (int q = threadIdx.x & 63; q < cnt; q += 64) { sc.sp0[chunk_begin + q] = s_sp0[q]; sc.hits0[chunk_begin + q] = s_hits0[q]; sc.ml0[chunk_begin + q] = s_ml0[q]; }
    }
    flush_counters(counters, lc, 0);
    wavelog_end(wl_t, 3);
}

template <bool USE_LDS, bool VEC8>
__global__ void
k_seed_decide(DevIndex ix, const char* __restrict__ seq, ReadGeom gm, int stride, long n, int seed_len, int pe_mode, ReadState st,
              SeedCarry sc, unsigned long long* __restrict__ counters)
{
    __shared__ unsigned int shc[2];
    if (threadIdx.x < 2) shc[threadIdx.x] = 0;
    __syncthreads();
    const long r = (long)blockIdx.x * blockDim.x + threadIdx.x;
    u32 n_sa = 0, n_ung = 0;
    extern __shared__ __align__(16) char lds_rows[];
    const int lstride = stride + 8;
    if (USE_LDS) {
        const long row0 = (long)blockIdx.x * blockDim.x;
        const long rows = n - row0 < (long)blockDim.x ? n - row0 : (long)blockDim.x;
        const int per_row = stride / 16;
        const int total16 = (int)rows * per_row;
        const uint4* src = reinterpret_cast<const uint4*>(seq + (size_t)row0 * stride);
        const int dq = (int)blockDim.x / per_row, dr = (int)blockDim.x - dq * per_row;
        int rr = (int)threadIdx.x / per_row, cc = (int)threadIdx.x - rr * per_row;
        for (int q = threadIdx.x; q < total16; q += blockDim.x) {
            const uint4 v = src[q];
            u64* dst = reinterpret_cast<u64*>(lds_rows + rr * lstride + cc * 16);
            dst[0] = ((u64)v.y << 32) | v.x;
            dst[1] = ((u64)v.w << 32) | v.z;
            rr += dq; cc += dr;
            if (cc >= per_row) { cc -= per_row; rr++; }
        }
    }
    __syncthreads();
    if (r < n) {
        const char* rd = USE_LDS ? lds_rows + (size_t)threadIdx.x * lstride : seq + (size_t)r * stride;
        const int L = gm.rl(r);
        int firstC = L;
        for (int i = 0; i < L; i += 8) {
            const u64 x = *reinterpret_cast<const u64*>(rd + i) ^ 0x4343434343434343ull;
            const u64 z = (x - 0x0101010101010101ull) & ~x & 0x8080808080808080ull;
            if (z) { const int j = i + (__ffsll((long long)z) - 1) / 8; if (j < L) firstC = j; break; }
        }
        SeedRec* my = st.seeds + (size_t)r * BMBS_MAX_SEEDS;
        int ns = 0;
        u64 ncand = 0, clen = 0;
        const int max_seed = L / 10 == 0 ? 25 : (L / 10 - 1 > 25 ? 25 : L / 10 - 1);
        int verdict = 0, multi = 0, get_error = -1, tm = 0, seed_id = 0;
        u64 mm_site = 0, c0 = 0, first_ml = 0;
        const u64 max_hits = 1000;
        bool done = false;
        u32 fc = 0, fd = 0;
        if (seed_id < max_seed && tm < L) {
            const u64 hits = sc.hits0[r], sp = sc.sp0[r];
            u64 ml = sc.ml0[r];
            first_ml = ml;
            if (hits == 1) {
                u64 p;
                if (sp >> 63) p = sp & ~(1ull << 63);
                else { p = sa_at(ix, sp); n_sa++; }
                const u64 loc = ix.total - p - ml;
                seed_record(my, ns, ncand, sp, 1, ml, 0);
                c0 = loc; clen = 1;
                int error = 0;
                if (ml > (u64)firstC) ml = (u64)firstC;
                if (ml != (u64)L) {
                    const int need = L - (int)ml;
                    const u64 start = loc + ml;
                    n_ung++;
                    if (VEC8) {
                        if (!window_valid(ix, start, (u64)need, loc < ix.G)) {
                            error = need >= 2 ? 2 : 1;
                        } else {
                            const int ml0 = (int)ml;
                            const uint4* g4 = reinterpret_cast<const uint4*>(ix.gen2);
                            u64 gidx = (loc + (u64)(ml0 & ~15)) >> 6;
                            uint4 cb = g4[gidx], nb = g4[gidx + 1];
                            for (int p = ml0 & ~15; p < L && error < 2; p += 16) {
                                const u64 r0 = *reinterpret_cast<const u64*>(rd + p), r1 = *reinterpret_cast<const u64*>(rd + p + 8);
                                const u64 d = loc + (u64)p;
                                if ((d >> 6) != gidx) { gidx = d >> 6; cb = nb; nb = g4[gidx + 1]; }
                                const int o = (int)(d & 63) * 2;
                                const u64 c0 = ((u64)cb.y << 32) | cb.x, c1 = ((u64)cb.w << 32) | cb.z, n0 = ((u64)nb.y << 32) | nb.x;
                                const u64 lo64 = o < 64 ? c0 : c1, hi64 = o < 64 ? c1 : n0;
                                const int sh = o & 63;
                                u64 w = lo64 >> sh;
                                if (sh > 32) w |= hi64 << (64 - sh);
                                const u32 w32 = (u32)w;
                                u64 m0 = mism8(r0, w32 & 0xffffu), m1 = mism8(r1, w32 >> 16);
                                if (p < ml0) {
                                    const int lo = ml0 - p;
                                    if (lo >= 8) { m0 = 0; m1 &= ~((1ull << (8 * (lo - 8))) - 1); } else m0 &= ~((1ull << (8 * lo)) - 1);
                                }
                                if (p + 16 > L) {
                                    const int hi = L - p;
                                    if (hi <= 8) { m1 = 0; if (hi < 8) m0 &= (1ull << (8 * hi)) - 1; } else m1 &= (1ull << (8 * (hi - 8))) - 1;
                                }
                                if (m0 | m1) {
                                    const int cnt = __popcll(m0) + __popcll(m1);
                                    if (error == 0) {
                                        ml = (u64)(m0 ? p + (__ffsll((long long)m0) - 1) / 8 : p + 8 + (__ffsll((long long)m1) - 1) / 8);
                                        error = cnt >= 2 ? 2 : 1;
                                    } else error = 2;
                                }
                            }
                        }
                    } else {
                        WinReader wr; wr.init(ix, start, window_valid(ix, start, (u64)need, loc < ix.G));
                        int read_i = (int)ml;
                        ReadCur rc; rc.seek(rd, read_i, L);
                        for (int i = 0; i < need; i++) {
                            const char a = rc.next();
                            const int b = wr.next();
                            if (!(code4(a) == b || (a == 'T' && b == 1))) { error++; if (error == 1) ml = (u64)read_i; else break; }
                            read_i++;
                        }
                    }
                }
                get_error = error;
                if (error == 0) { verdict = 1; st.exit_site[r] = loc; done = true; }
            }
            if (!done) {
                mm_site = ml;
                if (!pe_mode) {
                    if (ml == (u64)L && hits > 1) {
                        multi = 1;
                        if (firstC == L) { verdict = 4; done = true; }
                    }
                } else if (ml == (u64)L && hits > 1 && hits <= 10000) {
                    multi = 1;
                    if (firstC == L) { seed_record(my, ns, ncand, sp, hits, ml, 0); verdict = 4; done = true; }
                }
            }
            if (!done) {
                if (hits == 1) {  }
                else if (ml >= (u64)seed_len && hits <= max_hits) { if (hits != 0) { seed_record(my, ns, ncand, sp, hits, ml, (u64)tm); clen += hits; } }
                if (ml == 0) tm = seed_offset_unmatch(L, tm, rd, 8); else tm = tm + (int)(ml / 2);
                seed_id++;
            }
        }
        st.multi[r] = (u8)multi;
        st.mm_site[r] = (u16)(mm_site | ((mm_site < (u64)L && rd[mm_site] == 'N') ? 0x8000u : 0u));
        if (done) seed_finish(st, r, verdict, ns, ncand, pe_mode);
        else {
            st.exit_site[r] = c0;
            st.n_seeds[r] = (u8)ns; st.n_cand[r] = (u32)ncand;
            sc.tm[r] = (u16)tm; sc.seed_id[r] = (u8)seed_id; sc.clen[r] = (u32)clen; sc.first_ml[r] = (u16)first_ml;
            if (get_error == 1 && L - (int)first_ml >= 17) fc = 1; else fd = 1;
        }
        sc.flag_c[r] = fc; sc.flag_d[r] = fd;
    }
    if (counters) {
        atomicAdd(&shc[0], n_sa); atomicAdd(&shc[1], n_ung);
        __syncthreads();
        if (threadIdx.x == 0) { unsigned long long* cs = SHARD(counters); atomicAdd(&cs[2], (unsigned long long)shc[0]); atomicAdd(&cs[5], (unsigned long long)shc[1]); }
    }
}

__global__ void __launch_bounds__(64)
k_seed_decide_p(DevIndex ix, const char* __restrict__ seq, PackedRows pr, ReadGeom gm, int stride, long n, int seed_len, int pe_mode,
                int skip_v1, ReadState st, SeedCarry sc, unsigned long long* __restrict__ counters)
{
    __shared__ unsigned int shc[2];
    if (threadIdx.x < 2) shc[threadIdx.x] = 0;
    extern __shared__ __align__(16) char lds_prows[];
    const int lw = pr.pwords + 1;
    u64* lrows = reinterpret_cast<u64*>(lds_prows);
    const long row0 = (long)blockIdx.x * blockDim.x;
    const long rows = n - row0 < (long)blockDim.x ? n - row0 : (long)blockDim.x;
    {
        const u64* src = pr.base + (size_t)row0 * pr.pwords;
        const int total = (int)rows * pr.pwords;
        for (int q = threadIdx.x; q < total; q += blockDim.x) { const int rr = q / pr.pwords, cc = q - rr * pr.pwords; lrows[rr * lw + cc] = src[q]; }
    }
    __syncthreads();
    const long r = row0 + threadIdx.x;
    u32 n_sa = 0, n_ung = 0;
    if (r < n) {
        const u64* row = lrows + (size_t)threadIdx.x * lw;
        const int W = pr.W;
        const bool dirty = pr.dirty[r] != 0;
        const int L = gm.rl(r);
        int firstC = L;
        for (int w = 0; w * 32 < L; w++) {
            const u64 x = row[w];
            const u64 z = x & ~(x >> 1) & PK_EVEN;
            if (z) { const int j = w * 32 + (__ffsll((long long)z) - 1) / 2; if (j < L) firstC = j; break; }
        }
        SeedRec* my = st.seeds + (size_t)r * BMBS_MAX_SEEDS;
        int ns = 0;
        u64 ncand = 0, clen = 0;
        const int max_seed = L / 10 == 0 ? 25 : (L / 10 - 1 > 25 ? 25 : L / 10 - 1);
        int verdict = 0, multi = 0, get_error = -1, tm = 0, seed_id = 0;
        u64 mm_site = 0, c0 = 0, first_ml = 0;
        const u64 max_hits = 1000;
        bool done = false;
        u32 fc = 0, fd = 0;
        if (seed_id < max_seed && tm < L) {
            const u64 hits = sc.hits0[r], sp = sc.sp0[r];
            u64 ml = sc.ml0[r];
            first_ml = ml;
            if (hits == 1) {
                u64 p;
                if (sp >> 63) p = sp & ~(1ull << 63);
                else { p = sa_at(ix, sp); n_sa++; }
                const u64 loc = ix.total - p - ml;
                if (!skip_v1) seed_record(my, ns, ncand, sp, 1, ml, 0);
                c0 = loc; clen = 1;
                int error = 0;
                if (ml > (u64)firstC) ml = (u64)firstC;
                if (ml != (u64)L) {
                    const int need = L - (int)ml;
                    n_ung++;
                    if (!window_valid(ix, loc + ml, (u64)need, loc < ix.G)) {
                        error = need >= 2 ? 2 : 1;
                    } else {
                        const int ml0 = (int)ml;
                        GenStream gs; gs.init(ix, loc + (u64)(ml0 & ~31));
                        for (int q = ml0 & ~31; q < L && error < 2; q += 32) {
                            u64 mm = mism_bs(row[q >> 5], gs.next32());
                            if (dirty) mm |= spread32((u32)((row[W + (q >> 6)] >> (q & 63)) & 0xffffffffull));
                            mm &= field_range(ml0 - q, L - q);
                            if (mm) {
                                const int cnt = __popcll(mm);
                                if (error == 0) { ml = (u64)(q + (__ffsll((long long)mm) - 1) / 2); error = cnt >= 2 ? 2 : 1; }
                                else error = 2;
                            }
                        }
                    }
                }
                get_error = error;
                if (error == 0) { verdict = 1; st.exit_site[r] = loc; done = true; }
                if (skip_v1) { if (error == 0) { ns = 1; ncand = 1; } else seed_record(my, ns, ncand, sp, 1, first_ml, 0); }
            }
            if (!done) {
                mm_site = ml;
                if (!pe_mode) {
                    if (ml == (u64)L && hits > 1) {
                        multi = 1;
                        if (firstC == L) { verdict = 4; done = true; }
                    }
                } else if (ml == (u64)L && hits > 1 && hits <= 10000) {
                    multi = 1;
                    if (firstC == L) { seed_record(my, ns, ncand, sp, hits, ml, 0); verdict = 4; done = true; }
                }
            }
            if (!done) {
                if (hits == 1) {  }
                else if (ml >= (u64)seed_len && hits <= max_hits) { if (hits != 0) { seed_record(my, ns, ncand, sp, hits, ml, (u64)tm); clen += hits; } }
                if (ml == 0) {
                    if (!dirty) tm = (L - tm < 18) ? L : tm + 8;
                    else tm = seed_offset_unmatch_p(L, tm, seq + (size_t)r * stride, 8, row + W);
                } else tm = tm + (int)(ml / 2);
                seed_id++;
            }
        }
        st.multi[r] = (u8)multi;
        bool isN = false;
        if (dirty && mm_site < (u64)L && ((row[W + (mm_site >> 6)] >> (mm_site & 63)) & 1)) isN = seq[(size_t)r * stride + mm_site] == 'N';
        st.mm_site[r] = (u16)(mm_site | (isN ? 0x8000u : 0u));
        if (done) seed_finish(st, r, verdict, ns, ncand, pe_mode);
        else {
            st.exit_site[r] = c0;
            st.n_seeds[r] = (u8)ns; st.n_cand[r] = (u32)ncand;
            sc.tm[r] = (u16)tm; sc.seed_id[r] = (u8)seed_id; sc.clen[r] = (u32)clen; sc.first_ml[r] = (u16)first_ml;
            if (get_error == 1 && L - (int)first_ml >= 17) fc = 1; else fd = 1;
        }
        sc.flag_c[r] = fc; sc.flag_d[r] = fd;
    }
    if (counters) {
        atomicAdd(&shc[0], n_sa); atomicAdd(&shc[1], n_ung);
        __syncthreads();
        if (threadIdx.x == 0) { unsigned long long* cs = SHARD(counters); atomicAdd(&cs[2], (unsigned long long)shc[0]); atomicAdd(&cs[5], (unsigned long long)shc[1]); }
    }
}

template <bool PACKED, bool KG = false>
__global__ void __launch_bounds__(64)
k_seed_second(DevIndex ix, const char* __restrict__ seq, PackedRows pr, ReadGeom gm, int stride, const u64* __restrict__ count_ptr, int target_waves,
              int pe_mode, ReadState st, SeedCarry sc, unsigned long long* __restrict__ counters)
{
    int L = gm.L;
    const long total = (long)*count_ptr;
    const long chunk = seed_chunk(total, target_waves);
    const long chunk_begin = (long)blockIdx.x * chunk;
    if (chunk_begin >= total) return;
    __shared__ u64 s_c3[KG ? 27 : 1];
    th_tab_fill(ix);
    const u64* c3 = KG ? kgram_c3(ix, s_c3) : nullptr;
    const WaveLogT wl_t = wavelog_begin();
    const long chunk_end = chunk_begin + chunk < total ? chunk_begin + chunk : total;
    long next = chunk_begin;
    LaneCounters lc = {0, 0, 0, 0, 0};
    bool active = false;
    long r = 0;
    const char* rd = seq;
    const u64* prow = nullptr;
    bool dirty = false;
    typename std::conditional<PACKED, SearchP, Search>::type S; SeedHit h;
    const u64 max_hits = 1000;
    bool verify = false;
    auto finish = [&]() {
        SeedRec* my = st.seeds + (size_t)r * BMBS_MAX_SEEDS;
        int ns = st.n_seeds[r];
        u64 ncand = st.n_cand[r], clen = sc.clen[r];
        const u64 first_ml = sc.first_ml[r];
        const u64 second_len = (u64)L - first_ml;
        const u64 c0 = st.exit_site[r];
        u64 c1 = 0;
        int extra = 1;
        if (verify) {
            verify = false;
            u64 p;
            if (S.top >> 63) p = S.top & ~(1ull << 63);
            else { p = sa_at(ix, S.top); lc.n_sa++; }
            const int done_chars = 16 + S.s;
            const int tm = S.tm;
            const u64 site = ix.total - p - (u64)done_chars;
            bool ok = true;
            const int start = tm + done_chars;
            if constexpr (PACKED) ok = rest_matches_3l(ix, prow, pr.W, dirty, L, tm, start, site);
            else {
            Win32Cur wc; wc.init(ix, site + (u64)((start & ~15) - tm));
            for (int q = start & ~15; q < L && ok; q += 16) {
                const uint4 v = *reinterpret_cast<const uint4*>(rd + q);
                const u64 rw[2] = {((u64)v.y << 32) | v.x, ((u64)v.w << 32) | v.z};
                const u64 d = site + (u64)(q - tm);
                u64 m[2];
                if (d + 16 <= ix.total) {
                    const u32 w32 = wc.at(d);
                    m[0] = mism8_3letter(rw[0], w32 & 0xffffu); m[1] = mism8_3letter(rw[1], w32 >> 16);
                } else {
                    for (int hf = 0; hf < 2; hf++) {
                        m[hf] = 0;
                        for (int j = 0; j < 8; j++) {
                            const u64 dj = d + (u64)(8 * hf + j);
                            const char a = (char)((rw[hf] >> (8 * j)) & 0xff);
                            const bool eq = dj < ix.total && code3(a) <= 2 && code3(a) == code3("ACGT"[gbase(ix, dj)]);
                            if (!eq) m[hf] |= 0x80ull << (8 * j);
                        }
                    }
                }
                if (q < start) {
                    const int lo = start - q;
                    if (lo >= 8) { m[0] = 0; m[1] &= ~((1ull << (8 * (lo - 8))) - 1); } else m[0] &= ~((1ull << (8 * lo)) - 1);
                }
                if (q + 16 > L) {
                    const int hi = L - q;
                    if (hi <= 8) { m[1] = 0; if (hi < 8) m[0] &= (1ull << (8 * hi)) - 1; } else m[1] &= (1ull << (8 * (hi - 8))) - 1;
                }
                if (m[0] | m[1]) ok = false;
            }
            }
            if (ok) { h.hits = 1; h.sp = (p - (u64)(S.steps - S.s)) | (1ull << 63); }
            else { h.hits = 0; h.sp = 0; }
        }
        if (h.hits == 1) {
            u64 p;
            if (h.sp >> 63) p = h.sp & ~(1ull << 63);
            else { p = sa_at(ix, h.sp); lc.n_sa++; }
            c1 = ix.total - p - second_len - first_ml;
            seed_record(my, ns, ncand, h.sp, 1, second_len, first_ml);
            clen += 1; extra = 0;
        } else if (h.hits <= max_hits) {
            if (h.hits != 0) { seed_record(my, ns, ncand, h.sp, h.hits, second_len, first_ml); clen += h.hits; }
            extra = 0;
        }
        if (extra == 0) {
            int verdict = 0;
            if (clen == 1 || (clen == 2 && c0 == c1)) verdict = 2;
            else if (clen != 0) verdict = 3;
            seed_finish(st, r, verdict, ns, ncand, pe_mode);
            sc.flag_d[r] = 0;
        } else {
            st.n_seeds[r] = (u8)ns; st.n_cand[r] = (u32)ncand; sc.clen[r] = (u32)clen;
            sc.flag_d[r] = 1;
        }
    };
    bool pending = true, have = false;
    for (;;) {
        const unsigned long long pm = __ballot(pending);
        if (__popcll(pm) >= SEED_BATCH || !__any(active)) {
            if (pm == 0) break;
            const int rank = __popcll(pm & ((1ull << (threadIdx.x & 63)) - 1));
            const long it = next + rank;
            next += __popcll(pm);
            if (pending) {
// ... 41 lines not shown
    const long chunk = seed_chunk(total, target_waves);
    const long chunk_begin = (long)blockIdx.x * chunk;
    if (chunk_begin >= total) return;
    __shared__ u64 s_c3[KG ? 27 : 1];
    th_tab_fill(ix);
    const u64* c3 = KG ? kgram_c3(ix, s_c3) : nullptr;
    const WaveLogT wl_t = wavelog_begin();
    const long chunk_end = chunk_begin + chunk < total ? chunk_begin + chunk : total;
    long next = chunk_begin;
    LaneCounters lc = {0, 0, 0, 0, 0};
    bool active = false, have = false;
    long r = 0;
    extern __shared__ __align__(16) char lds_rows[];
    __shared__ u32 take_row[64];
    __shared__ u8 take_lane[64];
    const int lstride = stride + 16;
    const char* rd = ROWS_LDS ? lds_rows + (size_t)(threadIdx.x & 63) * lstride : seq;
    const int plw = pr.pwords + 1;
    const u64* prow = PLDS ? reinterpret_cast<const u64*>(lds_rows) + (size_t)(threadIdx.x & 63) * plw : nullptr;
    bool dirty = false;
    typename std::conditional<PACKED, SearchP, Search>::type S; SeedHit h = {0, 0, 0};
    SeedRec* my = nullptr;
    int ns = 0, tm = 0, seed_id = 0, max_seed = 0;
    u64 ncand = 0, clen = 0;
    const u64 max_hits = 1000;
    auto after_seed = [&]() -> bool {
        const int cur_len = L - tm;
        const u64 ml = h.ml;
        auto rec = [&](u64 hits) { if (exp_nostore) { ns++; ncand += hits; } else seed_record(my, ns, ncand, h.sp, hits, ml, (u64)tm); };
        if (h.hits == 1) { rec(1); clen += 1; }
        else if (ml >= (u64)seed_len && h.hits <= max_hits) { if (h.hits != 0) { rec(h.hits); clen += h.hits; } }
        else if ((u64)cur_len == ml) return false;
        if (ml == 0) {
            if (PACKED && !dirty) tm = (L - tm < 18) ? L : tm + 8;
            else if constexpr (PACKED) tm = seed_offset_unmatch_p(L, tm, seq + (size_t)r * stride, 8, prow + pr.W);
            else tm = seed_offset_unmatch(L, tm, rd, 8);
        } else tm = tm + (int)(ml / 2);
        seed_id++;
        return true;
    };
    bool pending = true, seed_done = false;
    for (;;) {
        const unsigned long long pm = __ballot(pending);
        if (__popcll(pm) >= SEED_BATCH || !__any(active)) {
            if (pm == 0) break;
            if (pending && have && seed_done) {
                seed_done = false;
                if (!after_seed()) { seed_finish(st, r, clen != 0 ? 3 : 0, ns, ncand, pe_mode); have = false; }
            }
            if (pending && have && !(seed_id < max_seed && tm < L)) { seed_finish(st, r, clen != 0 ? 3 : 0, ns, ncand, pe_mode); have = false; }
            const unsigned long long want = __ballot(pending && !have);
            const int rank = __popcll(want & ((1ull << (threadIdx.x & 63)) - 1));
            const long it = next + rank;
            const long avail = chunk_end - next;
            const int n_take = (long)__popcll(want) < avail ? __popcll(want) : (int)(avail > 0 ? avail : 0);
            next += __popcll(want);
            if ((ROWS_LDS || PLDS) && n_take > 0) {
                if (pending && !have && it < chunk_end) { take_row[rank] = sc.list_d[it]; take_lane[rank] = (u8)(threadIdx.x & 63); }
                __syncthreads();
                if constexpr (PLDS) {
                    const int per_row = pr.pwords / 2, pieces = n_take * per_row;
                    u64* lr = reinterpret_cast<u64*>(lds_rows);
                    for (int t = threadIdx.x & 63; t < pieces; t += 64) {
                        const int w = t / per_row, cc = t - w * per_row;
                        u64 a, b; load2(pr.base + (size_t)take_row[w] * pr.pwords + 2 * cc, a, b);
                        u64* d = lr + (size_t)take_lane[w] * plw + 2 * cc;
                        d[0] = a; d[1] = b;
                    }
                } else {
                    const int per_row = stride / 16, pieces = n_take * per_row;
                    for (int t = threadIdx.x & 63; t < pieces; t += 64) {
                        const int w = t / per_row, cc = t - w * per_row;
                        const uint4 v = *reinterpret_cast<const uint4*>(seq + (size_t)take_row[w] * stride + (size_t)cc * 16);
                        *reinterpret_cast<uint4*>(lds_rows + (size_t)take_lane[w] * lstride + cc * 16) = v;
                    }
                }
                __syncthreads();
            }
            if (pending && !have) {
                if (it < chunk_end) {
                    r = sc.list_d[it]; L = gm.rl(r);
                    if (!ROWS_LDS) rd = seq + (size_t)r * stride;
                    if constexpr (PACKED) { if constexpr (!PLDS) prow = pr.base + (size_t)r * pr.pwords; dirty = pr.dirty[r] != 0; }
                    my = st.seeds + (size_t)r * BMBS_MAX_SEEDS;
                    ns = st.n_seeds[r]; ncand = st.n_cand[r]; clen = sc.clen[r]; tm = sc.tm[r]; seed_id = sc.seed_id[r];
                    max_seed = L / 10 == 0 ? 25 : (L / 10 - 1 > 25 ? 25 : L / 10 - 1);
                    have = true;
                    if (!(seed_id < max_seed && tm < L)) { seed_finish(st, r, clen != 0 ? 3 : 0, ns, ncand, pe_mode); have = false; }
                } else pending = false;
            }
            if (pending && have) {
                bool go;
                if constexpr (PACKED) go = search_begin_p<false>(ix, prow, pr.W, dirty, L, tm, S, h, lc.n_hash); else go = search_begin<false>(ix, rd, L, tm, S, h, lc.n_hash);
                if (go) { active = true; pending = false; }
                else seed_done = true;
            }
            if (!__any(active) && !__any(pending)) break;
            continue;
        }
#ifdef BMBS_UTIL
        if ((threadIdx.x & 63) == 0) atomicAdd(&counters[12], 1ull);
        if (active) atomicAdd(&counters[13], 1ull);
#endif
        if (active) {
            bool fin;
            if constexpr (PACKED) fin = search_step_p<false, KG>(ix, L, S, h, lc.n_ext, c3, &lc.n_jump); else fin = search_step<false>(ix, rd, L, S, h, lc.n_ext);
            if (fin) { active = false; pending = true; seed_done = true; }
        }
    }
    flush_counters(counters, lc, 2);
    wavelog_end(wl_t, 5);
}
```

### bitmapperbs_amd/csrc/k_vote.hip

```cpp
#define VOTE_REG 16
#define VOTE_MID 32
__global__ void __launch_bounds__(64)
k_vote_fused(DevIndex ix, long n, ReadGeom gm, ReadState st, u64* __restrict__ cand, bmbs_vote* __restrict__ votes,
             u32* __restrict__ slot_read, u32* __restrict__ long_flag, const u64* __restrict__ count_ptr, const u32* __restrict__ list,
             u32* __restrict__ mid_flag)
{
    const long it = (long)blockIdx.x * blockDim.x + threadIdx.x;
    long r = it;
    if (list) { if (it >= (long)*count_ptr) return; r = list[it]; }
    else {
        if (r >= n) return;
        if (long_flag) long_flag[r] = 0;
    }
    if (st.verdict[r] != 3) { st.n_votes[r] = 0; return; }
    const int k = gm.rk(gm.rl(r));
    const u64 off = st.cand_off[r];
    const long nc = (long)st.n_cand[r];
    const SeedRec* my = st.seeds + (size_t)r * BMBS_MAX_SEEDS;
    const int ns = st.n_seeds[r];
    bmbs_vote* v = votes + off;
    if (nc <= VOTE_REG) {
        u64 c[VOTE_REG];
        int sidx = 0; u32 h = 0;
        u64 sp = 0, adj = 0; u32 hits = 0;
        if (ns > 0) { sp = my[0].sp; adj = (u64)my[0].len + (u64)my[0].off; hits = my[0].hits; }
#pragma unroll
        for (int j = 0; j < VOTE_REG; j++) {
            c[j] = ~0ull;
            if (j < nc) {
                while (h == hits && sidx + 1 < ns) { sidx++; h = 0; sp = my[sidx].sp; adj = (u64)my[sidx].len + (u64)my[sidx].off; hits = my[sidx].hits; }
                c[j] = ix.total - ((sp >> 63) ? (sp & ~(1ull << 63)) : sa_at(ix, sp + h)) - adj;
                h++;
            }
        }
#define CE(a, b) { const u64 x_ = c[a], y_ = c[b]; c[a] = x_ < y_ ? x_ : y_; c[b] = x_ < y_ ? y_ : x_; }
        CE(0,1) CE(2,3) CE(4,5) CE(6,7) CE(8,9) CE(10,11) CE(12,13) CE(14,15)
        CE(0,2) CE(1,3) CE(4,6) CE(5,7) CE(8,10) CE(9,11) CE(12,14) CE(13,15)
        CE(1,2) CE(5,6) CE(9,10) CE(13,14)
        CE(0,4) CE(1,5) CE(2,6) CE(3,7) CE(8,12) CE(9,13) CE(10,14) CE(11,15)
        CE(2,4) CE(3,5) CE(10,12) CE(11,13)
        CE(1,2) CE(3,4) CE(5,6) CE(9,10) CE(11,12) CE(13,14)
        CE(0,8) CE(1,9) CE(2,10) CE(3,11) CE(4,12) CE(5,13) CE(6,14) CE(7,15)
        CE(4,8) CE(5,9) CE(6,10) CE(7,11)
        CE(2,4) CE(3,5) CE(6,8) CE(7,9) CE(10,12) CE(11,13)
        CE(1,2) CE(3,4) CE(5,6) CE(7,8) CE(9,10) CE(11,12) CE(13,14)
#undef CE
        u32 vote[VOTE_REG];
        bool last[VOTE_REG];
        u32 run = 0;
        int nv = 0;
#pragma unroll
        for (int i = 0; i < VOTE_REG; i++) {
            run = (i > 0 && c[i] == c[i - 1]) ? run + 1 : 1;
            vote[i] = run;
            last[i] = i < nc && (i + 1 >= nc || (i + 1 < VOTE_REG && c[i + 1] != c[i]));
            nv += last[i] ? 1 : 0;
        }
#pragma unroll
        for (int i = 0; i < VOTE_REG; i++) {
            if (last[i]) {
                int rank = 0;
#pragma unroll
                for (int j = 0; j < VOTE_REG; j++) rank += (last[j] && (vote[j] > vote[i] || (vote[j] == vote[i] && j < i))) ? 1 : 0;
                bmbs_vote o;
                o.site = c[i] < (u64)k ? 0 : c[i] - (u64)k; o.vote = vote[i]; o.pad = 0;
                v[rank] = o;
            }
        }
        st.n_votes[r] = (u32)nv;
        for (long i = 0; i < nc; i++) slot_read[off + i] = i < nv ? (u32)r : 0xffffffffu;
        return;
    }
    if (mid_flag && nc <= VOTE_MID) { mid_flag[r] = 1; st.n_votes[r] = 0; return; }
    if (long_flag) { long_flag[r] = 1; st.n_votes[r] = 0; return; }
    u64* c = cand + off;
    {
        u64 o = 0;
        for (int s2 = 0; s2 < ns && o < (u64)nc; s2++) {
            const u64 sp = my[s2].sp, adj = (u64)my[s2].len + (u64)my[s2].off;
            const u32 hh = my[s2].hits;
            for (u32 j = 0; j < hh && o < (u64)nc; j++) c[o++] = ix.total - ((sp >> 63) ? (sp & ~(1ull << 63)) : sa_at(ix, sp + j)) - adj;
        }
    }
    sort_u64_asc(c, nc);
    long nv = 0;
    u64 pre = c[0];
    u32 vote = 1;
    for (long i = 1; i < nc; i++) {
        if (c[i] == pre) vote++;
        else { v[nv].site = pre < (u64)k ? 0 : pre - (u64)k; v[nv].vote = vote; v[nv].pad = 0; nv++; vote = 1; pre = c[i]; }
    }
    v[nv].site = pre >= (u64)k ? pre - (u64)k : 0; v[nv].vote = vote; v[nv].pad = 0; nv++;
    intro_sort_desc(v, nv);
    st.n_votes[r] = (u32)nv;
    for (long i = 0; i < nc; i++) slot_read[off + i] = i < nv ? (u32)r : 0xffffffffu;
}

__global__ void __launch_bounds__(64)
k_vote_mid(DevIndex ix, ReadGeom gm, ReadState st, const u64* __restrict__ count_ptr, const u32* __restrict__ list,
           u64* __restrict__ cand, bmbs_vote* __restrict__ votes, u32* __restrict__ slot_read, unsigned long long* __restrict__ counters)
{
    const long it = (long)blockIdx.x * blockDim.x + threadIdx.x;
    const bool act = it < (long)*count_ptr;
    const long r = act ? (long)list[it] : 0;
    const long nc = act ? (long)st.n_cand[r] : 0;
    wave_count_add(counters, CNT_CAND_MID, (u32)nc);
    if (!act) return;
    const int k = gm.rk(gm.rl(r));
    const u64 off = st.cand_off[r];
    const SeedRec* my = st.seeds + (size_t)r * BMBS_MAX_SEEDS;
    const int ns = st.n_seeds[r];
    bmbs_vote* v = votes + off;
    u64 c[VOTE_MID];
    {
        int sidx = 0; u32 h = 0;
        u64 sp = 0, adj = 0; u32 hits = 0;
        if (ns > 0) { sp = my[0].sp; adj = (u64)my[0].len + (u64)my[0].off; hits = my[0].hits; }
#pragma unroll
        for (int j = 0; j < VOTE_MID; j++) {
            c[j] = ~0ull;
            if (j < nc) {
                while (h == hits && sidx + 1 < ns) { sidx++; h = 0; sp = my[sidx].sp; adj = (u64)my[sidx].len + (u64)my[sidx].off; hits = my[sidx].hits; }
                c[j] = ix.total - ((sp >> 63) ? (sp & ~(1ull << 63)) : sa_at(ix, sp + h)) - adj;
                h++;
            }
        }
    }
#pragma unroll
    for (int size = 2; size <= VOTE_MID; size <<= 1) {
#pragma unroll
        for (int stride = size >> 1; stride > 0; stride >>= 1) {
#pragma unroll
            for (int t = 0; t < VOTE_MID / 2; t++) {
                const int i = 2 * t - (t & (stride - 1)), j = i + stride;
                const bool asc = (i & size) == 0;
                const u64 x_ = c[i], y_ = c[j];
                const bool sw = asc ? x_ > y_ : x_ < y_;
                c[i] = sw ? y_ : x_; c[j] = sw ? x_ : y_;
            }
        }
    }
    u32 vote[VOTE_MID];
    bool last[VOTE_MID];
    u32 run = 0;
    int nv = 0;
#pragma unroll
    for (int i = 0; i < VOTE_MID; i++) {
        run = (i > 0 && c[i] == c[i - 1]) ? run + 1 : 1;
        vote[i] = run;
        last[i] = i < nc && (i + 1 >= nc || (i + 1 < VOTE_MID && c[i + 1] != c[i]));
        nv += last[i] ? 1 : 0;
    }
    if (nv <= 16) {
#pragma unroll
        for (int i = 0; i < VOTE_MID; i++) {
            if (last[i]) {
                int rank = 0;
#pragma unroll
                for (int j = 0; j < VOTE_MID; j++) rank += (last[j] && (vote[j] > vote[i] || (vote[j] == vote[i] && j < i))) ? 1 : 0;
                bmbs_vote o;
                o.site = c[i] < (u64)k ? 0 : c[i] - (u64)k; o.vote = vote[i]; o.pad = 0;
                v[rank] = o;
            }
        }
    } else {
        bmbs_vk items[VOTE_MID];
        u64* park = cand + off;
        int e = 0;
#pragma unroll
        for (int i = 0; i < VOTE_MID; i++) {
            if (last[i]) { park[e] = c[i]; items[e].x = (vote[i] << 24) | (u32)e; e++; }
        }
        intro_sort_desc(items, (long)nv);
        for (int j = 0; j < nv; j++) {
            const u32 x = items[j].x;
            const u64 site = park[x & 0xffffffu];
            bmbs_vote o;
            o.site = site < (u64)k ? 0 : site - (u64)k; o.vote = x >> 24; o.pad = 0;
            v[j] = o;
        }
    }
    st.n_votes[r] = (u32)nv;
    for (long i = 0; i < nc; i++) slot_read[off + i] = i < nv ? (u32)r : 0xffffffffu;
}

#define VL_CAP 4096
#define VL_BLOCK 256
#define VM_CAP 256
#define VM_BLOCK 64
DEVI int vl_prefix(bool flag, int* sh_w, int& total)
{
    const int lane = threadIdx.x & 63, w = threadIdx.x >> 6;
    const unsigned long long m = __ballot(flag);
    if (lane == 0) sh_w[w] = __popcll(m);
    __syncthreads();
    int add = 0, tot = 0;
    for (int i = 0; i < (int)(blockDim.x >> 6); i++) { const int x = sh_w[i]; if (i < w) add += x; tot += x; }
    __syncthreads();
    total = tot;
    return add + __popcll(m & ((1ull << lane) - 1));
}
template <int EMAX>
DEVI void vl_radix_sort(u64* keys, int nc)
{
    __shared__ u64 sh_scan[18];
    const int T = (int)blockDim.x, tid = (int)threadIdx.x, lane = tid & 63, w = tid >> 6, nw = T >> 6;
    const int E = (nc + T - 1) / T;
    u64 mine[EMAX];
    u64 diff = 0;
    const u64 k0 = keys[0];
    for (int i = tid; i < nc; i += T) diff |= keys[i] ^ k0;
    for (int o = 32; o > 0; o >>= 1) diff |= __shfl_xor(diff, o, 64);
    if (lane == 0) sh_scan[w] = diff;
    __syncthreads();
    diff = 0;
    for (int i = 0; i < nw; i++) diff |= sh_scan[i];
    __syncthreads();
    const int nbits = diff ? 64 - __builtin_clzll(diff) : 0;
    for (int b = 0; b < nbits; b += 2) {
        u64 cnt = 0;
#pragma unroll
        for (int e = 0; e < EMAX; e++) {
            const int idx = tid * E + e;
            if (e < E && idx < nc) { mine[e] = keys[idx]; cnt += 1ull << (16 * (int)((mine[e] >> b) & 3)); }
        }
        u64 incl = cnt;
        for (int o = 1; o < 64; o <<= 1) { const u64 v = __shfl_up(incl, o, 64); if (lane >= o) incl += v; }
        if (lane == 63) sh_scan[w] = incl;
        __syncthreads();
        u64 wbase = 0, total = 0;
        for (int i = 0; i < nw; i++) { const u64 x = sh_scan[i]; if (i < w) wbase += x; total += x; }
        const u64 excl = wbase + incl - cnt;
        const u32 t0 = (u32)(total & 0xffff), t1 = (u32)((total >> 16) & 0xffff), t2 = (u32)((total >> 32) & 0xffff);
        u32 r0 = (u32)(excl & 0xffff), r1 = t0 + (u32)((excl >> 16) & 0xffff), r2 = t0 + t1 + (u32)((excl >> 32) & 0xffff),
            r3 = t0 + t1 + t2 + (u32)((excl >> 48) & 0xffff);
        __syncthreads();
#pragma unroll
        for (int e = 0; e < EMAX; e++) {
            const int idx = tid * E + e;
            if (e < E && idx < nc) {
                const int d = (int)((mine[e] >> b) & 3);
                const u32 r = d == 0 ? r0++ : d == 1 ? r1++ : d == 2 ? r2++ : r3++;
                keys[r] = mine[e];
            }
        }
        __syncthreads();
    }
}
DEVI void vl_locate_range(const DevIndex& ix, const SeedRec* my, int ns, long j0, int cnt, u64* keys, u32* sh_pref, bool build_pref)
{
    if (build_pref && threadIdx.x == 0) { u32 a = 0; for (int s2 = 0; s2 < ns; s2++) { sh_pref[s2] = a; a += my[s2].hits; } sh_pref[ns] = a; }
    __syncthreads();
    for (int j = threadIdx.x; j < cnt; j += blockDim.x) {
        const u32 g = (u32)(j0 + j);
        int s2 = 0;
        while (s2 + 1 < ns && sh_pref[s2 + 1] <= g) s2++;
        const u64 sp = my[s2].sp, adj = (u64)my[s2].len + (u64)my[s2].off;
        keys[j] = ix.total - ((sp >> 63) ? (sp & ~(1ull << 63)) : sa_at(ix, sp + (g - sh_pref[s2]))) - adj;
    }
    __syncthreads();
}
template <int EMAX>
DEVI int vl_sort_keys(u64* keys, int cnt)
{
    int np2 = 32;
    while (np2 < cnt) np2 <<= 1;
    for (int j = cnt + (int)threadIdx.x; j < np2; j += blockDim.x) keys[j] = ~0ull;
    __syncthreads();
    if (np2 > 512 && blockDim.x >= 128) { vl_radix_sort<EMAX>(keys, cnt); return np2; }
    for (int size = 2; size <= np2; size <<= 1)
        for (int stride = size >> 1; stride > 0; stride >>= 1) {
            for (int t = threadIdx.x; t < np2 / 2; t += blockDim.x) {
                const int i = 2 * t - (t & (stride - 1)), j = i + stride;
                const bool asc = (i & size) == 0;
                const u64 a = keys[i], b = keys[j];
                if ((a > b) == asc) { keys[i] = b; keys[j] = a; }
            }
            __syncthreads();
        }
    return np2;
}
template <int EMAX>
DEVI int vl_locate_sort_range(const DevIndex& ix, const SeedRec* my, int ns, long j0, int cnt, u64* keys, u32* sh_pref, bool build_pref)
{
    vl_locate_range(ix, my, ns, j0, cnt, keys, sh_pref, build_pref);
    return vl_sort_keys<EMAX>(keys, cnt);
}
template <int EMAX>
DEVI int vl_locate_sort(const DevIndex& ix, const SeedRec* my, int ns, int nc, u64* keys, u32* sh_pref)
{
    return vl_locate_sort_range<EMAX>(ix, my, ns, 0, nc, keys, sh_pref, true);
}
template <int CAP, int BLOCK>
DEVI void vl_sort_huge(const DevIndex& ix, const SeedRec* my, int ns, long nc, u64* keys, u32* sh_pref, u64* tmp, u64* c)
{
    const int T = (int)((nc + CAP - 1) / CAP);
    for (int t = 0; t < T; t++) {
        const long j0 = (long)t * CAP;
        const int cnt = (int)(nc - j0 < CAP ? nc - j0 : CAP);
        vl_locate_sort_range<(CAP + BLOCK - 1) / BLOCK>(ix, my, ns, j0, cnt, keys, sh_pref, t == 0);
        for (int j = threadIdx.x; j < cnt; j += BLOCK) tmp[j0 + j] = keys[j];
        __syncthreads();
    }
    for (long g = threadIdx.x; g < nc; g += BLOCK) {
        const int t = (int)(g / CAP);
        const u64 x = tmp[g];
        long rank = g - (long)t * CAP;
        for (int u = 0; u < T; u++) {
            if (u == t) continue;
            const u64* tu = tmp + (long)u * CAP;
            const long len = nc - (long)u * CAP < CAP ? nc - (long)u * CAP : CAP;
            long lo = 0, hi = len;
            while (lo < hi) { const long mid = (lo + hi) >> 1; const u64 y = tu[mid]; if (u < t ? y <= x : y < x) lo = mid + 1; else hi = mid; }
            rank += lo;
        }
        c[rank] = x;
    }
    __syncthreads();
}
DEVI int vl_run_ends(const u64* keys, int nc, u16* endpos, int* sh_w)
{
    int running = 0;
    for (int base = 0; base < nc; base += blockDim.x) {
        const int i = base + (int)threadIdx.x;
        const bool flag = i < nc && (i == nc - 1 || keys[i + 1] != keys[i]);
        int total;
        const int pre = vl_prefix(flag, sh_w, total);
        if (flag) endpos[running + pre] = (u16)i;
        running += total;
    }
    __syncthreads();
    return running;
}

struct VlRange { u16 f, l; int d; };
DEVI void vl_prefix2(bool f0, bool f1, int* sh_w, int& p0, int& p1, int& t0, int& t1)
{
    const int lane = threadIdx.x & 63, w = threadIdx.x >> 6, nw = (int)(blockDim.x >> 6);
    const unsigned long long m0 = __ballot(f0), m1 = __ballot(f1);
    if (lane == 0) { sh_w[w] = __popcll(m0); sh_w[nw + w] = __popcll(m1); }
    __syncthreads();
    int a0 = 0, a1 = 0, s0 = 0, s1 = 0;
    for (int i = 0; i < nw; i++) { const int x = sh_w[i], y = sh_w[nw + i]; if (i < w) { a0 += x; a1 += y; } s0 += x; s1 += y; }
    __syncthreads();
    t0 = s0; t1 = s1;
    const unsigned long long below = (1ull << lane) - 1;
    p0 = a0 + __popcll(m0 & below); p1 = a1 + __popcll(m1 & below);
}
DEVI int vl_partition(bmbs_vk* items, int first, int last, u16* Lpos, u16* Rpos, int* sh_w)
{
    if (threadIdx.x == 0) {
        using namespace bmbs_sort_detail;
        move_median_to_first(items, (long)first, (long)first + 1, (long)first + (last - first) / 2, (long)last - 1);
    }
    __syncthreads();
    const u32 pv = items[first].x >> 24;
    const int n = last - first - 1;
    int nL = 0, nR = 0;
    for (int base = 0; base < n; base += (int)blockDim.x) {
        const int j = base + (int)threadIdx.x;
        const int iL = first + 1 + j, iR = last - 1 - j;
        const bool fl = j < n && (items[iL].x >> 24) <= pv;
        const bool fr = j < n && (items[iR].x >> 24) >= pv;
        int pl, pr, tl, tr;
        vl_prefix2(fl, fr, sh_w, pl, pr, tl, tr);
        if (fl) Lpos[nL + pl] = (u16)iL;
        if (fr) Rpos[nR + pr] = (u16)iR;
        nL += tl; nR += tr;
    }
    __syncthreads();
    const int m = nL < nR ? nL : nR;
    int T = 0;
    for (int base = 0; base < m; base += (int)blockDim.x) {
        const int t = base + (int)threadIdx.x;
        const bool c = t < m && Lpos[t] < Rpos[t];
        int tot;
        vl_prefix(c, sh_w, tot);
// ... 77 lines not shown
    }
}
template <int CAP, int SMALL, int EMAX>
DEVI bool vl_sort_votes(bmbs_vk* items, int nv, void* scratch, int* sh_w, int* ctl)
{
    u16* Lpos = (u16*)scratch;
    u16* Rpos = Lpos + CAP;
    VlRange* big = (VlRange*)(Rpos + CAP);
    VlRange* small = big + 64;
    if (nv > 16) {
        if (threadIdx.x == 0) {
            int lg = 0;
            for (int t = nv; t > 1; t >>= 1) lg++;
            VlRange rg; rg.f = 0; rg.l = (u16)nv; rg.d = 2 * lg;
            ctl[0] = 0; ctl[1] = 0; ctl[2] = 0;
            if (nv > SMALL) { big[0] = rg; ctl[0] = 1; } else { small[0] = rg; ctl[1] = 1; }
        }
        __syncthreads();
        while (true) {
            const int nb = ctl[0];
            if (nb == 0 || ctl[2]) break;
            const VlRange rg = big[nb - 1];
            __syncthreads();
            if (threadIdx.x == 0) ctl[0] = nb - 1;
            int first = rg.f, last = rg.l, depth = rg.d;
            while (last - first > SMALL) {
                if (depth == 0) { if (threadIdx.x == 0) ctl[2] = 1; break; }
                --depth;
                const int cut = vl_partition(items, first, last, Lpos, Rpos, sh_w);
                if (threadIdx.x == 0) {
                    VlRange q; q.f = (u16)cut; q.l = (u16)last; q.d = depth;
                    if (last - cut > SMALL) big[ctl[0]++] = q;
                    else if (last - cut > 16) small[ctl[1]++] = q;
                }
                last = cut;
            }
            if (threadIdx.x == 0 && last - first > 16 && last - first <= SMALL) {
                VlRange q; q.f = (u16)first; q.l = (u16)last; q.d = depth;
                small[ctl[1]++] = q;
            }
            __syncthreads();
        }
        if (ctl[2]) return false;
        const int n_small = ctl[1];
        for (int s2 = threadIdx.x; s2 < n_small; s2 += (int)blockDim.x) vl_intro_small(items, small[s2].f, small[s2].l, small[s2].d);
        __syncthreads();
    }
    vl_stable_by_vote_desc<EMAX>(items, nv);
    return true;
}

#ifdef VOTE_PROF
__device__ unsigned long long g_vote_prof[4][8];
#define VP_T(v) const unsigned long long v = __builtin_readcyclecounter()
#define VP_ADD(cls, slot, val) do { if (threadIdx.x == 0) atomicAdd(&g_vote_prof[cls][slot], (unsigned long long)(val)); } while (0)
#else
#define VP_T(v)
#define VP_ADD(cls, slot, val)
#endif
template <int CAP, int BLOCK, int LO>
__global__ void __launch_bounds__(BLOCK) __attribute__((amdgpu_waves_per_eu(CAP == 256 ? 7 : 5)))
k_vote_long(DevIndex ix, ReadGeom gm, ReadState st, const u64* __restrict__ count_ptr, const u32* __restrict__ list,
            u64* __restrict__ cand, bmbs_vote* __restrict__ votes, u32* __restrict__ slot_read, u32* __restrict__ big_list,
            unsigned long long* __restrict__ big_count, unsigned long long* __restrict__ counters)
{
    __shared__ u64 keys[CAP];
    __shared__ u16 endpos[CAP];
    __shared__ bmbs_vk items[CAP];
    __shared__ u32 sh_pref[BMBS_MAX_SEEDS + 1];
    __shared__ int sh_w[2 * (BLOCK / 64) + 1];
    __shared__ int sh_ctl[4];
    const long total_items = (long)*count_ptr;
    for (long item = blockIdx.x; item < total_items; item += gridDim.x) {
        const long r = list[item];
        const long nc = (long)st.n_cand[r];
        if (big_list && CAP != VL_CAP && nc > CAP) { if (threadIdx.x == 0) big_list[atomicAdd(big_count, 1ull)] = (u32)r; continue; }
        if (nc <= LO || (CAP != VL_CAP && nc > CAP)) continue;
        if (counters && threadIdx.x == 0) {
            atomicAdd(&SHARD(counters)[CAP == VM_CAP ? CNT_CAND_LONG : CNT_CAND_BIG], (unsigned long long)nc);
            atomicAdd(&SHARD(counters)[CNT_LISTS_LONG], 1ull);
        }
        const int k = gm.rk(gm.rl(r));
        const u64 off = st.cand_off[r];
        const SeedRec* my = st.seeds + (size_t)r * BMBS_MAX_SEEDS;
        const int ns = st.n_seeds[r];
        bmbs_vote* v = votes + off;
        if constexpr (CAP == VL_CAP) if (nc > CAP) {
            u64* c = cand + off;
            u64* tmp = reinterpret_cast<u64*>(v);
            u32* endidx = slot_read + off;
            vl_sort_huge<CAP, BLOCK>(ix, my, ns, nc, keys, sh_pref, tmp, c);
            int nvh = 0;
            for (long base = 0; base < nc; base += BLOCK) {
                const long i = base + (long)threadIdx.x;
                const bool flag = i < nc && (i == nc - 1 || c[i + 1] != c[i]);
                int tot;
                const int pre = vl_prefix(flag, sh_w, tot);
                if (flag) endidx[nvh + pre] = (u32)i;
                nvh += tot;
            }
            __syncthreads();
            for (long e = threadIdx.x; e < nvh; e += BLOCK) tmp[e] = c[endidx[e]];
            __syncthreads();
            if (nvh <= CAP) {
                for (int e = threadIdx.x; e < nvh; e += BLOCK) {
                    const u32 vote = endidx[e] - (e ? endidx[e - 1] : 0xffffffffu);
                    items[e].x = (vote << 24) | (u32)e;
                    c[e] = tmp[e];
                }
                __syncthreads();
                if (!vl_sort_votes<CAP, (CAP > 256 ? 128 : 32), (CAP + BLOCK - 1) / BLOCK>(items, nvh, keys, sh_w, sh_ctl)) {
                    for (int e = threadIdx.x; e < nvh; e += BLOCK) {
                        const u32 vote = endidx[e] - (e ? endidx[e - 1] : 0xffffffffu);
                        items[e].x = (vote << 24) | (u32)e;
                    }
                    __syncthreads();
                    if (threadIdx.x == 0) intro_sort_desc(items, (long)nvh);
                    __syncthreads();
                }
                for (int j = threadIdx.x; j < nvh; j += BLOCK) {
                    const u32 it = items[j].x;
                    const u64 site = c[it & 0xffffffu];
                    bmbs_vote o; o.site = site < (u64)k ? 0 : site - (u64)k; o.vote = it >> 24; o.pad = 0;
                    v[j] = o;
                }
            } else {
                if (threadIdx.x == 0) {
                    for (long e = nvh - 1; e >= 0; e--) {
                        const u64 site = tmp[e];
                        const u32 vote = endidx[e] - (e ? endidx[e - 1] : 0xffffffffu);
                        bmbs_vote o; o.site = site < (u64)k ? 0 : site - (u64)k; o.vote = vote; o.pad = 0;
                        v[e] = o;
                    }
                    intro_sort_desc(v, (long)nvh);
                }
            }
            __syncthreads();
            for (long i = threadIdx.x; i < nc; i += BLOCK) slot_read[off + i] = i < nvh ? (u32)r : 0xffffffffu;
            if (threadIdx.x == 0) st.n_votes[r] = (u32)nvh;
            __syncthreads();
            continue;
        }
        [[maybe_unused]] constexpr int VP_CLS = CAP == VM_CAP ? 0 : CAP == 1024 ? 1 : CAP == 2048 ? 2 : 3;
        VP_T(vp0);
        vl_locate_sort<(CAP + BLOCK - 1) / BLOCK>(ix, my, ns, (int)nc, keys, sh_pref);
        VP_T(vp1);
        const int nv = vl_run_ends(keys, (int)nc, endpos, sh_w);
        for (int e = threadIdx.x; e < nv; e += BLOCK) {
            const u32 vote = (u32)endpos[e] - (e ? (u32)endpos[e - 1] : 0xffffffffu);
            items[e].x = (vote << 24) | (u32)e;
        }
        u64* c = cand + off;
        for (int e = threadIdx.x; e < nv; e += BLOCK) c[e] = keys[endpos[e]];
        __syncthreads();
        VP_T(vp2);
        if (!vl_sort_votes<CAP, (CAP > 256 ? 128 : 32), (CAP + BLOCK - 1) / BLOCK>(items, nv, keys, sh_w, sh_ctl)) {
            for (int e = threadIdx.x; e < nv; e += BLOCK) {
                const u32 vote = (u32)endpos[e] - (e ? (u32)endpos[e - 1] : 0xffffffffu);
                items[e].x = (vote << 24) | (u32)e;
            }
            __syncthreads();
            if (threadIdx.x == 0) intro_sort_desc(items, (long)nv);
            __syncthreads();
            VP_ADD(VP_CLS, 7, 1);
        }
        VP_T(vp3);
        for (int j = threadIdx.x; j < nv; j += BLOCK) {
// ... 54 lines not shown
```

Before: 1467.

## Store first seed once in a packed per-read record instead of copying into seed list

Replaces the three separate first-seed arrays (sp0, hits0, ml0) with one SeedRec array per read. The decide kernels no longer copy the first seed into the per-read seed list; they mark it valid by setting its offset to zero. Consumers read seeds through a SeedView that stitches the first record and the rest of the list together. This removes the redundant seed_record writes and the skip_v1 special case, but adds a branch on every seed access and more complex indexing, which risks subtle bugs in the reseeding paths.

```diff
diff --git a/bitmapperbs_amd/csrc/bmbs_api.hip b/bitmapperbs_amd/csrc/bmbs_api.hip
--- a/bitmapperbs_amd/csrc/bmbs_api.hip
+++ b/bitmapperbs_amd/csrc/bmbs_api.hip
@@ -188,7 +188,7 @@
 int per_read_workspace(Lane* c, u64 n)
 {
     ENS(c, c->verdict, n); ENS(c, c->n_seeds, n); ENS(c, c->multi, n); ENS(c, c->mm_site, n * 2);
-    ENS(c, c->exit_site, n * 8); ENS(c, c->seeds, n * BMBS_MAX_SEEDS * sizeof(SeedRec));
+    ENS(c, c->exit_site, n * 8); ENS(c, c->seeds, n * BMBS_MAX_SEEDS * sizeof(SeedRec)); ENS(c, c->seed_first, n * sizeof(SeedRec));
     ENS(c, c->n_cand, n * 4); ENS(c, c->cand_off, (n + 1) * 8); ENS(c, c->n_votes, n * 4);
     ENS(c, c->best_site, n * 8); ENS(c, c->best_end, n * 4); ENS(c, c->best_err, n * 4); ENS(c, c->sbd, n * 4);
     ENS(c, c->red_status, n); ENS(c, c->job_flag, n * 4); ENS(c, c->job_off, (n + 1) * 8);
@@ -199,7 +199,7 @@
 {
     ReadState s;
     s.verdict = c->verdict.as<u8>(); s.n_seeds = c->n_seeds.as<u8>(); s.multi = c->multi.as<u8>();
-    s.mm_site = c->mm_site.as<u16>(); s.exit_site = c->exit_site.as<u64>(); s.seeds = c->seeds.as<SeedRec>();
+    s.mm_site = c->mm_site.as<u16>(); s.exit_site = c->exit_site.as<u64>(); s.seeds = c->seeds.as<SeedRec>(); s.first = c->seed_first.as<SeedRec>();
     s.n_cand = c->n_cand.as<u32>(); s.cand_off = c->cand_off.as<u64>(); s.n_votes = c->n_votes.as<u32>();
     s.best_site = c->best_site.as<u64>(); s.best_end = c->best_end.as<int32_t>(); s.best_err = c->best_err.as<u32>();
     s.sbd = c->sbd.as<u32>(); s.red_status = c->red_status.as<u8>(); s.job_flag = c->job_flag.as<u32>();
@@ -317,7 +317,7 @@
 SeedCarry seed_carry(Lane* c)
 {
     SeedCarry sc;
-    sc.sp0 = c->sd_sp0.as<u64>(); sc.hits0 = c->sd_hits0.as<u32>(); sc.ml0 = c->sd_ml0.as<u16>(); sc.tm = c->sd_tm.as<u16>();
+    sc.first = c->seed_first.as<SeedRec>(); sc.tm = c->sd_tm.as<u16>();
     sc.seed_id = c->sd_seed_id.as<u8>(); sc.clen = c->sd_clen.as<u32>(); sc.first_ml = c->sd_first_ml.as<u16>();
     sc.flag_c = c->sd_flag_c.as<u32>(); sc.flag_d = c->sd_flag_d.as<u32>(); sc.off_c = c->sd_off_c.as<u64>(); sc.off_d = c->sd_off_d.as<u64>();
     sc.list_c = c->sd_list_c.as<u32>(); sc.list_d = c->sd_list_d.as<u32>();
@@ -379,7 +379,7 @@
 
 int launch_seeding(Lane* c, const char* d_seq, const ReadGeom& gm, int stride, u64 n, int pe_mode, bool prepacked)
 {
-    ENS(c, c->sd_sp0, n * 8); ENS(c, c->sd_hits0, n * 4); ENS(c, c->sd_ml0, n * 2); ENS(c, c->sd_tm, n * 2); ENS(c, c->sd_seed_id, n);
+    ENS(c, c->sd_tm, n * 2); ENS(c, c->sd_seed_id, n);
     ENS(c, c->sd_clen, n * 4); ENS(c, c->sd_first_ml, n * 2); ENS(c, c->sd_flag_c, n * 4); ENS(c, c->sd_flag_d, n * 4);
     ENS(c, c->sd_off_c, (n + 1) * 8); ENS(c, c->sd_off_d, (n + 1) * 8); ENS(c, c->sd_list_c, n * 4); ENS(c, c->sd_list_d, n * 4);
     SeedCarry sc = seed_carry(c);
@@ -413,7 +413,7 @@
     const bool lds_ok = (size_t)64 * (stride + 8) <= 48 * 1024;
     if (packed)
         hipLaunchKernelGGL(k_seed_decide_p, dim3(nblk(n, 64)), dim3(64), (size_t)64 * (pr.pwords + 1) * 8, c->stream, c->ix, d_seq, pr, gm, stride,
-                           (long)n, c->prm.seed_len, pe_mode, (stage && !(pe_mode && c->prm.sensitive)) ? 1 : 0, st, sc, cnt);
+                           (long)n, c->prm.seed_len, pe_mode, st, sc, cnt);
     else if (lds_ok)
         hipLaunchKernelGGL((k_seed_decide<true, true>), dim3(nblk(n, 64)), dim3(64), (size_t)64 * (stride + 8), c->stream, c->ix, d_seq, gm,
                            stride, (long)n, c->prm.seed_len, pe_mode, st, sc, cnt);
@@ -623,13 +623,13 @@
         release(c->wavelog_buf); release(c->wavelog_count);
     }
     DevBuf* all[] = {&c->occ, &c->hash, &c->sa, &c->gen2, &c->gen2p, &c->chrom_start, &c->t20, &c->pen_lut, &c->mapq_lut, &c->verdict,
-                     &c->n_seeds, &c->multi, &c->mm_site, &c->exit_site, &c->seeds, &c->n_cand, &c->cand_off,
+                     &c->n_seeds, &c->multi, &c->mm_site, &c->exit_site, &c->seeds, &c->seed_first, &c->n_cand, &c->cand_off,
                      &c->n_votes, &c->best_site, &c->best_end, &c->best_err, &c->sbd, &c->red_status, &c->job_flag,
                      &c->job_off, &c->scan_tmp, &c->scan_ticket, &c->totals, &c->cand, &c->votes, &c->slot_read, &c->vote_off, &c->votes_dense, &c->dense_read, &c->ferr, &c->fend,
                      &c->job_read, &c->job_site, &c->job_end, &c->job_err, &c->need_sw, &c->sw_off, &c->sw_job, &c->trace, &c->a_start, &c->a_end, &c->a_nm, &c->a_score, &c->a_nops,
                      &c->in_seq, &c->in_qual, &c->out_res, &c->cig_pool, &c->in_a, &c->in_b, &c->in_c, &c->in_d,
                      &c->stats, &c->call_stats, &c->flags, &c->counters, &c->pe_seq, &c->pe_B, &c->pe_occ, &c->pe_len, &c->pe_cur,
-                     &c->sd_sp0, &c->sd_hits0, &c->sd_ml0, &c->sd_tm, &c->sd_seed_id, &c->sd_clen, &c->sd_first_ml, &c->sd_flag_c, &c->sd_flag_d,
+                     &c->sd_tm, &c->sd_seed_id, &c->sd_clen, &c->sd_first_ml, &c->sd_flag_c, &c->sd_flag_d,
                      &c->sd_off_c, &c->sd_off_d, &c->sd_list_c, &c->sd_list_d, &c->pe_vround, &c->pe_dead, &c->pe_both, &c->pe_npair, &c->pe_sbd, &c->in_seq2, &c->in_qual2,
                      &c->pe_first, &c->pe_full, &c->pe_R, &c->pe_roff, &c->pe_rflag, &c->pe_rscan, &c->pe_rlist, &c->pe_rcnt, &c->pe_ritem_off, &c->pe_rcand, &c->long_flag, &c->long_off, &c->long_list, &c->vote_list,
                      &c->mapq_off, &c->klut, &c->in_len, &c->fq_text1, &c->fq_text2, &c->fq_idx, &c->pk_in1, &c->pk_in2, &c->pq_in1, &c->pq_in2, &c->pk_ascii, &c->prow, &c->prow_dirty, &c->pe_mid_flag, &c->pe_mid_list};
@@ -981,7 +981,7 @@
     hipLaunchKernelGGL(k_finalize, dim3(nblk(n, 256)), dim3(256), 0, c->stream, c->ix, c->sp, c->pen_lut.as<int>(),
                        c->mapq_lut.as<u8>(), c->mapq_off.as<u32>(), c->mapq_unit, d_seq, d_qual, gm, P.stride, (long)n, st, c->a_start.as<int>(),
                        c->a_end.as<int>(), c->a_nm.as<u32>(), c->a_score.as<int>(), c->a_nops.as<int>(), max_ops, P.cigar_base,
-                       c->prm.ambiguous_out, c->sd_sp0.as<u64>(), c->sd_hits0.as<u32>(),
+                       c->prm.ambiguous_out,
                        reinterpret_cast<bmbs_result_dev*>(P.d_results), c->call_stats.as<unsigned long long>());
     prof_end(c);
     return call_end(c, P.slot);
diff --git a/bitmapperbs_amd/csrc/bmbs_dev.h b/bitmapperbs_amd/csrc/bmbs_dev.h
--- a/bitmapperbs_amd/csrc/bmbs_dev.h
+++ b/bitmapperbs_amd/csrc/bmbs_dev.h
@@ -37,6 +37,7 @@
     u8*   multi;
     u16*  mm_site;
     u64*  exit_site;
+    SeedRec* first;
     SeedRec* seeds;
     u32*  n_cand;
     u64*  cand_off;
@@ -49,6 +50,28 @@
     u32*  job_flag;
     u64*  job_off;
 };
+
+struct SeedView {
+    const SeedRec* first;
+    const SeedRec* rest;
+    __device__ __forceinline__ const SeedRec& operator[](int i) const { return *((i == 0 && first) ? first : rest + i); }
+};
+__device__ __forceinline__ SeedView seed_view(const ReadState& st, long r)
+{
+    const SeedRec* f = st.first + r;
+    const bool has = f->off == 0;
+    SeedView v;
+    v.first = has ? f : nullptr;
+    v.rest = st.seeds + (size_t)r * BMBS_MAX_SEEDS - (has ? 1 : 0);
+    return v;
+}
+__device__ __forceinline__ SeedView seed_view_reseeded(const ReadState& st, long r)
+{
+    SeedView v;
+    v.first = nullptr;
+    v.rest = st.seeds + (size_t)r * BMBS_MAX_SEEDS;
+    return v;
+}
 
 struct ReadGeom {
     const u16* len; const u8* klut; int L; int k;
diff --git a/bitmapperbs_amd/csrc/bmbs_host.h b/bitmapperbs_amd/csrc/bmbs_host.h
--- a/bitmapperbs_amd/csrc/bmbs_host.h
+++ b/bitmapperbs_amd/csrc/bmbs_host.h
@@ -139,7 +139,7 @@
     bool luts_ready = false;
     int mapq_unit = 0;
     DevBuf mapq_off, klut;
-    DevBuf verdict, n_seeds, multi, mm_site, exit_site, seeds, n_cand, cand_off, n_votes, best_site,
+    DevBuf verdict, n_seeds, multi, mm_site, exit_site, seeds, seed_first, n_cand, cand_off, n_votes, best_site,
         best_end, best_err, sbd, red_status, job_flag, job_off, scan_tmp, totals;
     DevBuf scan_ticket;
     u32 scan_ticket_base = 0, scan_epoch = 0;
@@ -178,7 +178,7 @@
     struct OpenText { bool valid = false, pe = false; u64 bytes1 = 0, bytes2 = 0; int64_t n = 0; } open_text;
     u32* h_info = nullptr;
     int n_refs = 0, max_ref_len = 0;
-    DevBuf sd_sp0, sd_hits0, sd_ml0, sd_tm, sd_seed_id, sd_clen, sd_first_ml, sd_flag_c, sd_flag_d, sd_off_c, sd_off_d, sd_list_c, sd_list_d;
+    DevBuf sd_tm, sd_seed_id, sd_clen, sd_first_ml, sd_flag_c, sd_flag_d, sd_off_c, sd_off_d, sd_list_c, sd_list_d;
     DevBuf pe_seq, pe_B, pe_occ, pe_len, pe_cur, pe_vround, pe_dead, pe_both, pe_npair, pe_sbd, in_seq2, in_qual2;
     DevBuf pe_first, pe_full, pe_R, pe_roff, pe_rflag, pe_rscan, pe_rlist, pe_rcnt, pe_ritem_off, pe_rcand;
     u64 last_reseeded = 0, last_reseed_cand = 0;
diff --git a/bitmapperbs_amd/csrc/k_finalize.hip b/bitmapperbs_amd/csrc/k_finalize.hip
--- a/bitmapperbs_amd/csrc/k_finalize.hip
+++ b/bitmapperbs_amd/csrc/k_finalize.hip
@@ -5,7 +5,7 @@
            const u32* __restrict__ mapq_off, int unit, const char* __restrict__ seq, const char* __restrict__ qual, ReadGeom gm,
            int stride, long n, ReadState st, const int* __restrict__ a_start, const int* __restrict__ a_end,
            const u32* __restrict__ a_nm, const int* __restrict__ a_score, const int* __restrict__ a_nops,
-           int max_ops, u32 cigar_base, int ambiguous_out, const u64* __restrict__ sp0, const u32* __restrict__ hits0,
+           int max_ops, u32 cigar_base, int ambiguous_out,
            bmbs_result_dev* __restrict__ res, unsigned long long* __restrict__ stats)
 {
     __shared__ unsigned long long sh[5];
@@ -35,8 +35,8 @@
         } else if (verdict == 4) {
             o.status = 2; o.path = 4;
             if (ambiguous_out) {
-                const u64 sp_ = sp0[r];
-                u32 nh = hits0[r]; if (nh > 1000u) nh = 1000u;
+                const u64 sp_ = st.first[r].sp;
+                u32 nh = st.first[r].hits; if (nh > 1000u) nh = 1000u;
                 o.status = 3;
                 for (u32 i = 0; i < nh; i++) {
                     const u64 s_ = ix.total - sa_at(ix, sp_ + i) - (u64)L;
diff --git a/bitmapperbs_amd/csrc/k_pe_fast.hip b/bitmapperbs_amd/csrc/k_pe_fast.hip
--- a/bitmapperbs_amd/csrc/k_pe_fast.hip
+++ b/bitmapperbs_amd/csrc/k_pe_fast.hip
@@ -192,7 +192,7 @@
     const int L = gm.rl(r), k = gm.rk(L);
     const int v = st.verdict[r];
     const long nc = (long)st.n_cand[r];
-    const SeedRec* my = st.seeds + (size_t)r * BMBS_MAX_SEEDS;
+    const SeedView my = seed_view(st, r);
     const int ns = st.n_seeds[r];
     PeCand* o = A + st.cand_off[r];
     if (nc <= VOTE_REG) {
@@ -288,7 +288,7 @@
     if (!act) return;
     const int L = gm.rl(r), k = gm.rk(L);
     const int v = st.verdict[r];
-    const SeedRec* my = st.seeds + (size_t)r * BMBS_MAX_SEEDS;
+    const SeedView my = seed_view(st, r);
     const int ns = st.n_seeds[r];
     PeCand* o = A + st.cand_off[r];
     u64 c[VOTE_MID];
@@ -421,7 +421,7 @@
             PeCand* o = A + st.cand_off[r];
             if (nc > CAP) {
                 u64* c = cand + st.cand_off[r];
-                vl_sort_huge<CAP, BLOCK>(ix, st.seeds + (size_t)r * BMBS_MAX_SEEDS, st.n_seeds[r], nc, keys, sh_pref, reinterpret_cast<u64*>(o), c);
+                vl_sort_huge<CAP, BLOCK>(ix, seed_view(st, r), st.n_seeds[r], nc, keys, sh_pref, reinterpret_cast<u64*>(o), c);
                 if (v == 4) {
                     for (long i = threadIdx.x; i < nc; i += BLOCK) { PeCand e; e.site = c[i]; e.err = 0; e.end = L - 1; o[i] = e; }
                     if (threadIdx.x == 0) { ps.occ[r] = (int)nc; ps.len[r] = (u32)nc; }
@@ -443,7 +443,7 @@
                 __syncthreads();
                 continue;
             }
-            vl_locate_range(ix, st.seeds + (size_t)r * BMBS_MAX_SEEDS, st.n_seeds[r], 0, (int)nc, keys, sh_pref, true);
+            vl_locate_range(ix, seed_view(st, r), st.n_seeds[r], 0, (int)nc, keys, sh_pref, true);
             int cnt = (int)nc;
             if (prefilter && v == 3) {
                 const bool earlier = !listed(m) || (long)st.n_cand[m] <= LO;
diff --git a/bitmapperbs_amd/csrc/k_pe_sensitive.hip b/bitmapperbs_amd/csrc/k_pe_sensitive.hip
--- a/bitmapperbs_amd/csrc/k_pe_sensitive.hip
+++ b/bitmapperbs_amd/csrc/k_pe_sensitive.hip
@@ -26,8 +26,8 @@
     for (int m = 0; m < 2; m++) {
         const long r = p + m * n;
         const int v = st.verdict[r], ns = st.n_seeds[r];
-        const SeedRec* my = st.seeds + (size_t)r * BMBS_MAX_SEEDS;
-        c[m] = (v == 1 || v == 4) ? 0u : (ns >= 1 && my[0].off == 0 ? my[0].hits : 0u);
+        const SeedRec f0 = st.first[r];
+        c[m] = (v == 1 || v == 4) ? 0u : (f0.off == 0 ? f0.hits : 0u);
         ps.full[r] = (u8)((sc.flag_c[r] && !sc.flag_d[r]) ? 1 : ns);
         ps.roff[r] = 0;
     }
@@ -146,22 +146,24 @@
         const u64* prow = PACKED ? pr.base + (size_t)r * pr.pwords : nullptr;
         const bool dirty = PACKED ? pr.dirty[r] != 0 : false;
         const int L = gm.rl(r);
+        const SeedView old = seed_view(st, r);
         SeedRec* my = st.seeds + (size_t)r * BMBS_MAX_SEEDS;
         const int full = ps.full[r];
         int rs[3], rl[3], rn = 0;
         int s0 = 0, s1 = 0;
-        if (full >= 1) s0 = my[0].off;
+        if (full >= 1) s0 = old[0].off;
         if (full >= 2) {
-            s1 = my[1].off;
+            s1 = old[1].off;
             rn = 2;
             rs[0] = s0; rl[0] = s1 - s0;
-            rs[1] = (int)my[full - 2].off + (int)my[full - 2].len; rl[1] = L - rs[1];
+            rs[1] = (int)old[full - 2].off + (int)old[full - 2].len; rl[1] = L - rs[1];
         } else if (full == 1) {
             rn = 2;
             rs[0] = s0; rl[0] = L / 2;
             rs[1] = rs[0] + rl[0]; rl[1] = L - rs[1];
         }
-        const int last = full >= 1 ? (int)my[full - 1].off + (int)my[full - 1].len : 0;
+        const int last = full >= 1 ? (int)old[full - 1].off + (int)old[full - 1].len : 0;
+        if (old.first) st.first[r].off = 0xffff;
         if (last < L) { rs[rn] = last; rl[rn] = L - last; rn++; }
         const int max_seed = L / 10 == 0 ? 25 : (L / 10 - 1 > 25 ? 25 : L / 10 - 1);
         const u64 max_hits = 1000, avail = 20;
@@ -225,7 +227,7 @@
     const long nc = (long)(o1 - o0);
     if (nc == 0) { ps.len[r] = 0; ps.vround[r] = 0; return; }
     if (long_flag && nc > PESV_LONG) { long_flag[it] = 1; return; }
-    const SeedRec* my = st.seeds + (size_t)r * BMBS_MAX_SEEDS;
+    const SeedView my = seed_view_reseeded(st, r);
     const int ns = st.n_seeds[r];
     u64* c = rcand + o0;
     long o = 0;
@@ -271,7 +273,7 @@
         const int k = gm.rk(gm.rl(r));
         long long maxd, mind; int large_k;
         pe_bounds(gm, pi, p, n, maxd, mind, large_k);
-        const SeedRec* my = st.seeds + (size_t)r * BMBS_MAX_SEEDS;
+        const SeedView my = seed_view_reseeded(st, r);
         const int ns = st.n_seeds[r];
         const PeCand* a = pe_list(ps, st, A, B, rF);
         const int occF = ps.occ[rF];
diff --git a/bitmapperbs_amd/csrc/k_seed.hip b/bitmapperbs_amd/csrc/k_seed.hip
--- a/bitmapperbs_amd/csrc/k_seed.hip
+++ b/bitmapperbs_amd/csrc/k_seed.hip
@@ -316,7 +316,7 @@
 }
 
 struct SeedCarry {
-    u64* sp0; u32* hits0; u16* ml0;
+    SeedRec* first;
     u16* tm; u8* seed_id; u32* clen; u16* first_ml;
     u32* flag_c; u32* flag_d;
     u64* off_c; u64* off_d;
@@ -379,9 +379,7 @@
              unsigned long long* __restrict__ counters)
 {
     __shared__ u64 s_c3[KG ? 27 : 1];
-    __shared__ u64 s_sp0[STAGE ? SEED_CHUNK : 1];
-    __shared__ u32 s_hits0[STAGE ? SEED_CHUNK : 1];
-    __shared__ u16 s_ml0[STAGE ? SEED_CHUNK : 1];
+    __shared__ SeedRec s_first[STAGE ? SEED_CHUNK : 1];
     th_tab_fill(ix);
     const u64* c3 = KG ? kgram_c3(ix, s_c3) : nullptr;
     const WaveLogT wl_t = wavelog_begin();
@@ -404,8 +402,8 @@
             next += __popcll(pm);
             if (pending) {
                 if (have) {
-                    if (STAGE) { const int q = (int)(r - chunk_begin); s_sp0[q] = h.sp; s_hits0[q] = (u32)h.hits; s_ml0[q] = (u16)h.ml; }
-                    else { sc.sp0[r] = h.sp; sc.hits0[r] = (u32)h.hits; sc.ml0[r] = (u16)h.ml; }
+                    SeedRec f; f.sp = h.sp; f.hits = (u32)h.hits; f.len = (u16)h.ml; f.off = 0xffff;
+                    if (STAGE) s_first[(int)(r - chunk_begin)] = f; else sc.first[r] = f;
                     have = false;
                 }
                 if (it < chunk_end) {
@@ -432,7 +430,7 @@
     if (STAGE) {
         __syncthreads();
         const int cnt = (int)(chunk_end - chunk_begin);
-        for (int q = threadIdx.x & 63; q < cnt; q += 64) { sc.sp0[chunk_begin + q] = s_sp0[q]; sc.hits0[chunk_begin + q] = s_hits0[q]; sc.ml0[chunk_begin + q] = s_ml0[q]; }
+        for (int q = threadIdx.x & 63; q < cnt; q += 64) sc.first[chunk_begin + q] = s_first[q];
     }
     flush_counters(counters, lc, 0);
     wavelog_end(wl_t, 3);
@@ -477,9 +475,9 @@
             const u64 z = (x - 0x0101010101010101ull) & ~x & 0x8080808080808080ull;
             if (z) { const int j = i + (__ffsll((long long)z) - 1) / 8; if (j < L) firstC = j; break; }
         }
-        SeedRec* my = st.seeds + (size_t)r * BMBS_MAX_SEEDS;
         int ns = 0;
         u64 ncand = 0, clen = 0;
+        auto book_first = [&](u64 h_) { ns = 1; ncand = h_; };
         const int max_seed = L / 10 == 0 ? 25 : (L / 10 - 1 > 25 ? 25 : L / 10 - 1);
         int verdict = 0, multi = 0, get_error = -1, tm = 0, seed_id = 0;
         u64 mm_site = 0, c0 = 0, first_ml = 0;
@@ -487,15 +485,16 @@
         bool done = false;
         u32 fc = 0, fd = 0;
         if (seed_id < max_seed && tm < L) {
-            const u64 hits = sc.hits0[r], sp = sc.sp0[r];
-            u64 ml = sc.ml0[r];
+            const SeedRec f0 = sc.first[r];
+            const u64 hits = f0.hits, sp = f0.sp;
+            u64 ml = f0.len;
             first_ml = ml;
             if (hits == 1) {
                 u64 p;
                 if (sp >> 63) p = sp & ~(1ull << 63);
                 else { p = sa_at(ix, sp); n_sa++; }
                 const u64 loc = ix.total - p - ml;
-                seed_record(my, ns, ncand, sp, 1, ml, 0);
+                book_first(1);
                 c0 = loc; clen = 1;
                 int error = 0;
                 if (ml > (u64)firstC) ml = (u64)firstC;
@@ -564,16 +563,17 @@
                     }
                 } else if (ml == (u64)L && hits > 1 && hits <= 10000) {
                     multi = 1;
-                    if (firstC == L) { seed_record(my, ns, ncand, sp, hits, ml, 0); verdict = 4; done = true; }
+                    if (firstC == L) { book_first(hits); verdict = 4; done = true; }
                 }
             }
             if (!done) {
                 if (hits == 1) {  }
-                else if (ml >= (u64)seed_len && hits <= max_hits) { if (hits != 0) { seed_record(my, ns, ncand, sp, hits, ml, (u64)tm); clen += hits; } }
+                else if (ml >= (u64)seed_len && hits <= max_hits) { if (hits != 0) { book_first(hits); clen += hits; } }
                 if (ml == 0) tm = seed_offset_unmatch(L, tm, rd, 8); else tm = tm + (int)(ml / 2);
                 seed_id++;
             }
         }
+        if (ns) sc.first[r].off = 0;
         st.multi[r] = (u8)multi;
         st.mm_site[r] = (u16)(mm_site | ((mm_site < (u64)L && rd[mm_site] == 'N') ? 0x8000u : 0u));
         if (done) seed_finish(st, r, verdict, ns, ncand, pe_mode);
@@ -594,7 +594,7 @@
 
 __global__ void __launch_bounds__(64)
 k_seed_decide_p(DevIndex ix, const char* __restrict__ seq, PackedRows pr, ReadGeom gm, int stride, long n, int seed_len, int pe_mode,
-                int skip_v1, ReadState st, SeedCarry sc, unsigned long long* __restrict__ counters)
+                ReadState st, SeedCarry sc, unsigned long long* __restrict__ counters)
 {
     __shared__ unsigned int shc[2];
     if (threadIdx.x < 2) shc[threadIdx.x] = 0;
@@ -622,9 +622,9 @@
             const u64 z = x & ~(x >> 1) & PK_EVEN;
             if (z) { const int j = w * 32 + (__ffsll((long long)z) - 1) / 2; if (j < L) firstC = j; break; }
         }
-        SeedRec* my = st.seeds + (size_t)r * BMBS_MAX_SEEDS;
         int ns = 0;
         u64 ncand = 0, clen = 0;
+        auto book_first = [&](u64 h_) { ns = 1; ncand = h_; };
         const int max_seed = L / 10 == 0 ? 25 : (L / 10 - 1 > 25 ? 25 : L / 10 - 1);
         int verdict = 0, multi = 0, get_error = -1, tm = 0, seed_id = 0;
         u64 mm_site = 0, c0 = 0, first_ml = 0;
@@ -632,15 +632,16 @@
         bool done = false;
         u32 fc = 0, fd = 0;
         if (seed_id < max_seed && tm < L) {
-            const u64 hits = sc.hits0[r], sp = sc.sp0[r];
-            u64 ml = sc.ml0[r];
+            const SeedRec f0 = sc.first[r];
+            const u64 hits = f0.hits, sp = f0.sp;
+            u64 ml = f0.len;
             first_ml = ml;
             if (hits == 1) {
                 u64 p;
                 if (sp >> 63) p = sp & ~(1ull << 63);
                 else { p = sa_at(ix, sp); n_sa++; }
                 const u64 loc = ix.total - p - ml;
-                if (!skip_v1) seed_record(my, ns, ncand, sp, 1, ml, 0);
+                book_first(1);
                 c0 = loc; clen = 1;
                 int error = 0;
                 if (ml > (u64)firstC) ml = (u64)firstC;
@@ -666,7 +667,6 @@
                 }
                 get_error = error;
                 if (error == 0) { verdict = 1; st.exit_site[r] = loc; done = true; }
-                if (skip_v1) { if (error == 0) { ns = 1; ncand = 1; } else seed_record(my, ns, ncand, sp, 1, first_ml, 0); }
             }
             if (!done) {
                 mm_site = ml;
@@ -677,12 +677,12 @@
                     }
                 } else if (ml == (u64)L && hits > 1 && hits <= 10000) {
                     multi = 1;
-                    if (firstC == L) { seed_record(my, ns, ncand, sp, hits, ml, 0); verdict = 4; done = true; }
+                    if (firstC == L) { book_first(hits); verdict = 4; done = true; }
                 }
             }
             if (!done) {
                 if (hits == 1) {  }
-                else if (ml >= (u64)seed_len && hits <= max_hits) { if (hits != 0) { seed_record(my, ns, ncand, sp, hits, ml, (u64)tm); clen += hits; } }
+                else if (ml >= (u64)seed_len && hits <= max_hits) { if (hits != 0) { book_first(hits); clen += hits; } }
                 if (ml == 0) {
                     if (!dirty) tm = (L - tm < 18) ? L : tm + 8;
                     else tm = seed_offset_unmatch_p(L, tm, seq + (size_t)r * stride, 8, row + W);
@@ -690,6 +690,7 @@
                 seed_id++;
             }
         }
+        if (ns) sc.first[r].off = 0;
         st.multi[r] = (u8)multi;
         bool isN = false;
         if (dirty && mm_site < (u64)L && ((row[W + (mm_site >> 6)] >> (mm_site & 63)) & 1)) isN = seq[(size_t)r * stride + mm_site] == 'N';
@@ -736,8 +737,8 @@
     const u64 max_hits = 1000;
     bool verify = false;
     auto finish = [&]() {
-        SeedRec* my = st.seeds + (size_t)r * BMBS_MAX_SEEDS;
         int ns = st.n_seeds[r];
+        SeedRec* my = st.seeds + (size_t)r * BMBS_MAX_SEEDS - ns;
         u64 ncand = st.n_cand[r], clen = sc.clen[r];
         const u64 first_ml = sc.first_ml[r];
         const u64 second_len = (u64)L - first_ml;
@@ -945,8 +946,7 @@
                     r = sc.list_d[it]; L = gm.rl(r);
                     if (!ROWS_LDS) rd = seq + (size_t)r * stride;
                     if constexpr (PACKED) { if constexpr (!PLDS) prow = pr.base + (size_t)r * pr.pwords; dirty = pr.dirty[r] != 0; }
-                    my = st.seeds + (size_t)r * BMBS_MAX_SEEDS;
-                    ns = st.n_seeds[r]; ncand = st.n_cand[r]; clen = sc.clen[r]; tm = sc.tm[r]; seed_id = sc.seed_id[r];
+                    ns = st.n_seeds[r]; my = st.seeds + (size_t)r * BMBS_MAX_SEEDS - ns; ncand = st.n_cand[r]; clen = sc.clen[r]; tm = sc.tm[r]; seed_id = sc.seed_id[r];
                     max_seed = L / 10 == 0 ? 25 : (L / 10 - 1 > 25 ? 25 : L / 10 - 1);
                     have = true;
                     if (!(seed_id < max_seed && tm < L)) { seed_finish(st, r, clen != 0 ? 3 : 0, ns, ncand, pe_mode); have = false; }
diff --git a/bitmapperbs_amd/csrc/k_vote.hip b/bitmapperbs_amd/csrc/k_vote.hip
--- a/bitmapperbs_amd/csrc/k_vote.hip
+++ b/bitmapperbs_amd/csrc/k_vote.hip
@@ -16,7 +16,7 @@
     const int k = gm.rk(gm.rl(r));
     const u64 off = st.cand_off[r];
     const long nc = (long)st.n_cand[r];
-    const SeedRec* my = st.seeds + (size_t)r * BMBS_MAX_SEEDS;
+    const SeedView my = seed_view(st, r);
     const int ns = st.n_seeds[r];
     bmbs_vote* v = votes + off;
     if (nc <= VOTE_REG) {
@@ -108,7 +108,7 @@
     if (!act) return;
     const int k = gm.rk(gm.rl(r));
     const u64 off = st.cand_off[r];
-    const SeedRec* my = st.seeds + (size_t)r * BMBS_MAX_SEEDS;
+    const SeedView my = seed_view(st, r);
     const int ns = st.n_seeds[r];
     bmbs_vote* v = votes + off;
     u64 c[VOTE_MID];
@@ -247,7 +247,7 @@
         __syncthreads();
     }
 }
-DEVI void vl_locate_range(const DevIndex& ix, const SeedRec* my, int ns, long j0, int cnt, u64* keys, u32* sh_pref, bool build_pref)
+DEVI void vl_locate_range(const DevIndex& ix, const SeedView& my, int ns, long j0, int cnt, u64* keys, u32* sh_pref, bool build_pref)
 {
     if (build_pref && threadIdx.x == 0) { u32 a = 0; for (int s2 = 0; s2 < ns; s2++) { sh_pref[s2] = a; a += my[s2].hits; } sh_pref[ns] = a; }
     __syncthreads();
@@ -281,18 +281,18 @@
     return np2;
 }
 template <int EMAX>
-DEVI int vl_locate_sort_range(const DevIndex& ix, const SeedRec* my, int ns, long j0, int cnt, u64* keys, u32* sh_pref, bool build_pref)
+DEVI int vl_locate_sort_range(const DevIndex& ix, const SeedView& my, int ns, long j0, int cnt, u64* keys, u32* sh_pref, bool build_pref)
 {
     vl_locate_range(ix, my, ns, j0, cnt, keys, sh_pref, build_pref);
     return vl_sort_keys<EMAX>(keys, cnt);
 }
 template <int EMAX>
-DEVI int vl_locate_sort(const DevIndex& ix, const SeedRec* my, int ns, int nc, u64* keys, u32* sh_pref)
+DEVI int vl_locate_sort(const DevIndex& ix, const SeedView& my, int ns, int nc, u64* keys, u32* sh_pref)
 {
     return vl_locate_sort_range<EMAX>(ix, my, ns, 0, nc, keys, sh_pref, true);
 }
 template <int CAP, int BLOCK>
-DEVI void vl_sort_huge(const DevIndex& ix, const SeedRec* my, int ns, long nc, u64* keys, u32* sh_pref, u64* tmp, u64* c)
+DEVI void vl_sort_huge(const DevIndex& ix, const SeedView& my, int ns, long nc, u64* keys, u32* sh_pref, u64* tmp, u64* c)
 {
     const int T = (int)((nc + CAP - 1) / CAP);
     for (int t = 0; t < T; t++) {
@@ -536,7 +536,7 @@
         }
         const int k = gm.rk(gm.rl(r));
         const u64 off = st.cand_off[r];
-        const SeedRec* my = st.seeds + (size_t)r * BMBS_MAX_SEEDS;
+        const SeedView my = seed_view(st, r);
         const int ns = st.n_seeds[r];
         bmbs_vote* v = votes + off;
         if constexpr (CAP == VL_CAP) if (nc > CAP) {
```

New measurement: 1477 (median of 6 runs). Within noise of the previous version (+0.7%).
